# jdwhite48/groth-sahai-rs

Measured on AMD Instinct MI355X. Metric: GS proofs+verifies/sec (BLS12-381 PPE batch), higher is better.
Workload: dtype u32 limbs (381-bit Montgomery); 1 GPU; 2^16 independent PPE equations per GPU, m=4 n=4, BLS12-381, commit_and_prove+verify(exact); curve=BLS12-381, equations_per_gpu=65536, total_equations=65536, rccl_ranks=0, distinct_devices=1, parallelism=equation-sharded x1

## Files before the change

groth_sahai_rs_amd/csrc/gen_params.py:

```python
#!/usr/bin/env python3
import os
import sys


def limbs32(v, n):
    return [(v >> (32 * i)) & 0xFFFFFFFF for i in range(n)]


def carr(v, n):
    return "{" + ",".join("0x%08xu" % x for x in limbs32(v, n)) + "}"


class F2:

    def __init__(self, p):
        self.p = p

    def mul(self, a, b):
        p = self.p
        return ((a[0] * b[0] - a[1] * b[1]) % p, (a[0] * b[1] + a[1] * b[0]) % p)

    def pow(self, a, e):
        r = (1, 0)
        while e:
            if e & 1:
                r = self.mul(r, a)
            a = self.mul(a, a)
            e >>= 1
        return r

    def inv(self, a):
        p = self.p
        n = pow(a[0] * a[0] + a[1] * a[1], -1, p)
        return (a[0] * n % p, (-a[1]) * n % p)


def naf(k):
    d = []
    while k:
        if k & 1:
            z = 2 - (k % 4)
            k -= z
        else:
            z = 0
        d.append(z)
        k >>= 1
    return d


def emit(name, S, p, r, x, b, xi, twist, loop_count, loop_neg, bn, g1, g2):
    n = (p.bit_length() + 31) // 32
    nr = (r.bit_length() + 31) // 32
    Rp = 1 << (32 * n)
    Rr = 1 << (32 * nr)
    f2 = F2(p)

    def m(v):
        return v * Rp % p

    def m2(a):
        return "{%s,%s}" % (carr(m(a[0]), n), carr(m(a[1]), n))

    L = (p.bit_length() + 27) // 28
    if L * 28 - p.bit_length() < 8:
        L += 1
    R28 = 1 << (28 * L)
    Rb = 1 << (32 * n)

    def l28(v):
        ls = []
        for i in range(L - 1):
            ls.append(v & 0xFFFFFFF)
            v >>= 28
        ls.append(v)
        return "{" + ",".join(str(x) for x in ls) + "}"

    def i28(v):
        return l28(v * R28 % p)

    def i28_2(a):
        return "{%s,%s}" % (i28(a[0]), i28(a[1]))

    out = []
    w = out.append
    w("// GENERATED by gen_params.py -- do not edit.")
    w("#pragma once")
    w("#include <stdint.h>")
    w("#ifndef GS_DEVCONST")
    w("#if defined(__HIPCC__)")
    w("#define GS_DEVCONST __device__")
    w("#else")
    w("#define GS_DEVCONST")
    w("#endif")
    w("#endif")
    w("namespace gs {")
    w("struct %s {" % S)
    w("  static constexpr int N = %d;      // u32 limbs of Fq" % n)
    w("  static constexpr int NR = %d;     // u32 limbs of Fr" % nr)
    w("  static constexpr int CURVE_ID = %d;" % (0 if name == "bls12_381" else 1))
    w("  static constexpr bool TWIST_M = %s;" % ("true" if twist == "M" else "false"))
    w("  static constexpr bool IS_BN = %s;" % ("true" if bn else "false"))
    w("  static constexpr int XI_A = %d;   // xi = XI_A + u" % xi[0])
    w("  GS_DEVCONST static constexpr uint32_t P[%d] = %s;" % (n, carr(p, n)))
    w("  GS_DEVCONST static constexpr uint32_t P_INV = 0x%08xu;   // -p^-1 mod 2^32" % ((-pow(p, -1, 1 << 32)) % (1 << 32)))
    w("  GS_DEVCONST static constexpr uint32_t P_ONE[%d] = %s;   // R mod p" % (n, carr(Rp % p, n)))
    w("  GS_DEVCONST static constexpr uint32_t P_R2[%d] = %s;    // R^2 mod p" % (n, carr(Rp * Rp % p, n)))
    w("  GS_DEVCONST static constexpr uint32_t P_M2[%d] = %s;    // p - 2 (inversion exponent)" % (n, carr(p - 2, n)))
    w("  static constexpr int P_BITS = %d;" % p.bit_length())
    w("  GS_DEVCONST static constexpr uint32_t Q[%d] = %s;   // scalar field modulus r" % (nr, carr(r, nr)))
    w("  GS_DEVCONST static constexpr uint32_t Q_INV = 0x%08xu;" % ((-pow(r, -1, 1 << 32)) % (1 << 32)))
    w("  GS_DEVCONST static constexpr uint32_t Q_ONE[%d] = %s;" % (nr, carr(Rr % r, nr)))
    w("  GS_DEVCONST static constexpr uint32_t Q_R2[%d] = %s;" % (nr, carr(Rr * Rr % r, nr)))
    w("  static constexpr int Q_BITS = %d;" % r.bit_length())
    w("  GS_DEVCONST static constexpr uint32_t TWO_INV[%d] = %s;" % (n, carr(m(pow(2, -1, p)), n)))
    w("  GS_DEVCONST static constexpr uint32_t B1[%d] = %s;       // G1: y^2 = x^3 + b" % (n, carr(m(b), n)))
    b2 = f2.mul((b, 0), xi) if twist == "M" else f2.mul((b, 0), f2.inv(xi))
    w("  GS_DEVCONST static constexpr uint32_t B2[2][%d] = %s;   // twist coefficient b'" % (n, m2(b2)))
    b2x3 = ((3 * b2[0]) % p, (3 * b2[1]) % p)
    w("  GS_DEVCONST static constexpr uint32_t B2X3[2][%d] = %s;" % (n, m2(b2x3)))
    k = 3 * b if twist == "M" and 3 * b < 16 else 0
    assert k == 0 or b2x3 == f2.mul((k, 0), xi)
    w("  static constexpr int B2X3_XI_K = %d;   // 3 b' = B2X3_XI_K * xi when non-zero" % k)
    for j in (1, 2, 3):
        e = (p**j - 1) // 6
        assert (p**j - 1) % 6 == 0
        g = [f2.pow(xi, k * e) for k in range(6)]
        w("  GS_DEVCONST static constexpr uint32_t FROB%d[6][2][%d] = {%s};" % (j, n, ",".join(m2(v) for v in g)))
    ax = abs(x)
    w("  static constexpr uint64_t X_ABS = 0x%xull;" % ax)
    w("  static constexpr bool X_NEG = %s;" % ("true" if x < 0 else "false"))
    d = naf(loop_count) if bn else [(loop_count >> i) & 1 for i in range(loop_count.bit_length())]
    w("  static constexpr int LOOP_LEN = %d;   // digits of the Miller loop count, LSB first" % len(d))
    w("  GS_DEVCONST static constexpr int8_t LOOP[%d] = {%s};" % (len(d), ",".join(str(v) for v in d)))
    w("  static constexpr bool LOOP_NEG = %s;" % ("true" if loop_neg else "false"))
    w("  GS_DEVCONST static constexpr uint32_t G1_GEN[2][%d] = {%s,%s};" % (n, carr(m(g1[0]), n), carr(m(g1[1]), n)))
    w("  GS_DEVCONST static constexpr uint32_t G2_GEN[2][2][%d] = {%s,%s};" % (n, m2(g2[0]), m2(g2[1])))
    w("  static constexpr int L = %d;      // 28-bit limbs of Fq (internal form a*2^(28L) mod p, lazily reduced)" % L)
    w("  GS_DEVCONST static constexpr int32_t P28[%d] = %s;" % (L, l28(p)))
    w("  static constexpr uint32_t P28_INV = %du;   // -p^-1 mod 2^28" % ((-pow(p, -1, 1 << 28)) % (1 << 28)))
    w("  static constexpr float INV_PTOP2 = %.9ef;   // 2^(28(L-2)) / p  (value-reduction quotient estimate)" % ((1 << (28 * (L - 2))) / p))
    w("  GS_DEVCONST static constexpr int32_t ONE28[%d] = %s;" % (L, i28(1)))
    w("  GS_DEVCONST static constexpr int32_t K_IN28[%d] = %s;   // boundary -> internal: R28^2/Rb mod p" % (L, l28(R28 * R28 * pow(Rb, -1, p) % p)))
    w("  GS_DEVCONST static constexpr int32_t K_OUT28[%d] = %s;  // internal -> boundary: Rb mod p" % (L, l28(Rb % p)))
    assert p % 4 == 3
    w("  GS_DEVCONST static constexpr int32_t RR28[%d] = %s;    // canonical -> internal: R28^2 mod p" % (L, l28(R28 * R28 % p)))
    w("  GS_DEVCONST static constexpr int32_t RRR28[%d] = %s;   // R28^3 mod p: plain inverse of an internal value -> internal inverse" % (L, l28(pow(R28, 3, p))))
    w("  static constexpr int INV_DIVSTEPS = %d;" % ((45907 * p.bit_length() + 26313) // 19929))
    w("  GS_DEVCONST static constexpr uint32_t SQRT_EXP[%d] = %s;  // (p+1)/4" % (n, carr((p + 1) // 4, n)))
    w("  GS_DEVCONST static constexpr uint32_t HALF_P[%d] = %s;    // (p-1)/2" % (n, carr((p - 1) // 2, n)))
    w("  GS_DEVCONST static constexpr uint32_t P_WORDS[%d] = %s;" % (n, carr(p, n)))
    w("  GS_DEVCONST static constexpr uint32_t R_WORDS[%d] = %s;" % (nr, carr(r, nr)))
    w("  GS_DEVCONST static constexpr int32_t B2_28[2][%d] = %s;   // b of the twist" % (L, i28_2(b2)))
    w("  GS_DEVCONST static constexpr int32_t B1_28[%d] = %s;" % (L, i28(b)))
    w("  GS_DEVCONST static constexpr int32_t B2X3_28[2][%d] = %s;" % (L, i28_2(b2x3)))
    for j in (1, 2, 3):
        e = (p**j - 1) // 6
        g = [f2.pow(xi, k * e) for k in range(6)]
        w("  GS_DEVCONST static constexpr int32_t FROB%d_28[6][2][%d] = {%s};" % (j, L, ",".join(i28_2(v) for v in g)))
    if not bn:
        lam = x * x - 1
        assert (lam * lam + lam + 1) % r == 0 and lam.bit_length() <= 128
        def f2add(a, b2_): return ((a[0] + b2_[0]) % p, (a[1] + b2_[1]) % p)
        def f2sub(a, b2_): return ((a[0] - b2_[0]) % p, (a[1] - b2_[1]) % p)
        def ec_add(P1, P2, mul_, sub_, add_, inv_, zero):
            if P1 is None: return P2
            if P2 is None: return P1
            (x1, y1), (x2, y2) = P1, P2
            if x1 == x2:
                if y1 != y2 or y1 == zero: return None
                l_ = mul_(mul_(add_(add_(x1, x1), x1), x1), inv_(add_(y1, y1)))
            else:
                l_ = mul_(sub_(y2, y1), inv_(sub_(x2, x1)))
            x3 = sub_(sub_(mul_(l_, l_), x1), x2)
            return (x3, sub_(mul_(l_, sub_(x1, x3)), y1))
        def ec_mul(k, P_, *ops):
            acc = None
            for bit in bin(k)[2:]:
                acc = ec_add(acc, acc, *ops)
                if bit == "1": acc = ec_add(acc, P_, *ops)
            return acc
        ops1 = (lambda a, b_: a * b_ % p, lambda a, b_: (a - b_) % p, lambda a, b_: (a + b_) % p, lambda a: pow(a, -1, p), 0)
        ops2 = (f2.mul, f2sub, f2add, f2.inv, (0, 0))
        lamG = ec_mul(lam, g1, *ops1)
        beta = None
        for cand in range(2, 50):
            bcand = pow(cand, (p - 1) // 3, p)
            if bcand != 1 and (bcand * g1[0]) % p == lamG[0]:
                beta = bcand
                break
        assert beta is not None and lamG[1] == g1[1]
        G2 = ((g2[0][0], g2[0][1]), (g2[1][0], g2[1][1]))
        xG2 = ec_mul(abs(x), G2, *ops2)
        xG2 = (xG2[0], ((-xG2[1][0]) % p, (-xG2[1][1]) % p))
        conj_ = lambda a: (a[0], (-a[1]) % p)
        e3, e2 = (p - 1) // 3, (p - 1) // 2
        found = None
        for sx in (1, -1):
            for sy in (1, -1):
                cx = f2.pow(xi, e3) if sx == 1 else f2.inv(f2.pow(xi, e3))
                cy = f2.pow(xi, e2) if sy == 1 else f2.inv(f2.pow(xi, e2))
                if (f2.mul(conj_(G2[0]), cx), f2.mul(conj_(G2[1]), cy)) == xG2:
                    found = (cx, cy)
        assert found, "psi constants"
        cx, cy = found
        nx, ny = f2.mul(cx, conj_(cx)), f2.mul(cy, conj_(cy))
        assert nx[1] == 0 and ny[1] == 0
        c3x, c3y = f2.mul(cx, nx), f2.mul(cy, ny)
        out.insert(out.index("};"), "") if False else None
        w2 = lambda line: out.insert(len(out), line)
        endo = []
        endo.append("  static constexpr bool HAS_ENDO = true;")
        endo.append("  GS_DEVCONST static constexpr uint32_t LAMBDA[4] = %s;   // x^2 - 1: phi(P) = (beta x, y) = lambda P" % carr(lam, 4))
        endo.append("  GS_DEVCONST static constexpr int32_t BETA_28[%d] = %s;" % (L, i28(beta)))
        endo.append("  GS_DEVCONST static constexpr uint32_t XABS_LIMBS[2] = %s;" % carr(abs(x), 2))
        endo.append("  GS_DEVCONST static constexpr int32_t PSI_X_28[2][%d] = %s;   // psi(x,y) = (conj(x) cx, conj(y) cy) = [x]Q" % (L, i28_2(cx)))
        endo.append("  GS_DEVCONST static constexpr int32_t PSI_Y_28[2][%d] = %s;" % (L, i28_2(cy)))
        endo.append("  GS_DEVCONST static constexpr int32_t PSI2_X_28[%d] = %s;     // psi^2(x,y) = (x nx, y ny)" % (L, i28(nx[0])))
        endo.append("  GS_DEVCONST static constexpr int32_t PSI2_Y_28[%d] = %s;" % (L, i28(ny[0])))
        endo.append("  GS_DEVCONST static constexpr int32_t PSI3_X_28[2][%d] = %s;" % (L, i28_2(c3x)))
        endo.append("  GS_DEVCONST static constexpr int32_t PSI3_Y_28[2][%d] = %s;" % (L, i28_2(c3y)))
    else:
        from fractions import Fraction
        def ec_add1(P1, P2):
            if P1 is None: return P2
            if P2 is None: return P1
            (x1, y1), (x2, y2) = P1, P2
            if x1 == x2:
                if (y1 + y2) % p == 0: return None
                l_ = 3 * x1 * x1 * pow(2 * y1, -1, p) % p
            else:
                l_ = (y2 - y1) * pow(x2 - x1, -1, p) % p
            x3 = (l_ * l_ - x1 - x2) % p
            return (x3, (l_ * (x1 - x3) - y1) % p)
        def ec_mul1(k, P_):
            acc = None
            for bit in bin(k)[2:]:
                acc = ec_add1(acc, acc)
                if bit == "1": acc = ec_add1(acc, P_)
            return acc
        lam = beta = None
        for gcand in range(2, 12):
            z = pow(gcand, (r - 1) // 3, r)
            if z == 1: continue
            for zz in (z, (-z - 1) % r):
                lg = ec_mul1(zz, g1)
                for cand in range(2, 50):
                    bc = pow(cand, (p - 1) // 3, p)
                    if bc != 1 and bc * g1[0] % p == lg[0] and lg[1] == g1[1]:
                        lam, beta = zz, bc
            if lam: break
        assert lam and (lam * lam + lam + 1) % r == 0
        def lagrange(u, v):
            dot = lambda a, b_: a[0] * b_[0] + a[1] * b_[1]
            if dot(u, u) < dot(v, v): u, v = v, u
            while True:
                q = round(Fraction(dot(u, v), dot(v, v)))
                u = (u[0] - q * v[0], u[1] - q * v[1])
                if dot(u, u) >= dot(v, v): return [list(v), list(u)]
                u, v = v, u
        def lll(B_):
            n_ = len(B_)
            B_ = [list(map(Fraction, b_)) for b_ in B_]
            def gso():
                Bs, m_ = [], [[Fraction(0)] * n_ for _ in range(n_)]
                for i in range(n_):
                    v = B_[i][:]
                    for j in range(i):
                        m_[i][j] = sum(a * b_ for a, b_ in zip(B_[i], Bs[j])) / sum(a * a for a in Bs[j])
                        v = [a - m_[i][j] * b_ for a, b_ in zip(v, Bs[j])]
                    Bs.append(v)
                return Bs, m_
            k_ = 1
            while k_ < n_:
                Bs, m_ = gso()
                for j in range(k_ - 1, -1, -1):
                    q = round(m_[k_][j])
                    if q:
                        B_[k_] = [a - q * b_ for a, b_ in zip(B_[k_], B_[j])]
                        Bs, m_ = gso()
                if sum(a * a for a in Bs[k_]) >= (Fraction(3, 4) - m_[k_][k_ - 1] ** 2) * sum(a * a for a in Bs[k_ - 1]):
                    k_ += 1
                else:
                    B_[k_], B_[k_ - 1] = B_[k_ - 1], B_[k_]
                    k_ = max(k_ - 1, 1)
            return [[int(a) for a in b_] for b_ in B_]
        def inv_first_row(B_):
            n_ = len(B_)
            A_ = [list(map(Fraction, row)) + [Fraction(int(i == j)) for j in range(n_)] for i, row in enumerate(B_)]
            for i in range(n_):
                piv = next(j for j in range(i, n_) if A_[j][i] != 0)
                A_[i], A_[piv] = A_[piv], A_[i]
                f_ = A_[i][i]
                A_[i] = [a / f_ for a in A_[i]]
                for j in range(n_):
                    if j != i:
                        f_ = A_[j][i]
                        A_[j] = [a - f_ * b_ for a, b_ in zip(A_[j], A_[i])]
            return [A_[0][n_ + i] for i in range(n_)]
        def lattice_consts(tag, B_, eig, gw, bw):
            n_ = len(B_)
            for b_ in B_:
                assert sum(b_[j] * eig ** j for j in range(n_)) % r == 0
            row = inv_first_row(B_)
            G_ = [abs(int(v * (1 << 256))) for v in row]
            sg = [1 if v < 0 else 0 for v in row]
            import random as _rnd
            rr_ = _rnd.Random(7)
            worst = 0
            for _ in range(4000):
                k_ = rr_.randrange(r)
                cs = [(k_ * G_[i] >> 256) * (-1 if sg[i] else 1) for i in range(n_)]
                ks = [(k_ if j == 0 else 0) - sum(cs[i] * B_[i][j] for i in range(n_)) for j in range(n_)]
                assert (sum(ks[j] * eig ** j for j in range(n_)) - k_) % r == 0
                worst = max(worst, max(abs(v).bit_length() for v in ks))
            lines = ["  static constexpr int %s_SUBBITS = %d;   // measured bound on the sub-scalars (4000 samples) + slack below" % (tag, worst),
                     "  GS_DEVCONST static constexpr uint32_t %s_G[%d][%d] = {%s};" % (tag, n_, gw, ",".join(carr(v, gw) for v in G_)),
                     "  GS_DEVCONST static constexpr uint8_t %s_GS[%d] = {%s};" % (tag, n_, ",".join(str(v) for v in sg)),
                     "  GS_DEVCONST static constexpr uint32_t %s_B[%d][%d][%d] = {%s};" % (tag, n_, n_, bw, ",".join("{" + ",".join(carr(abs(v), bw) for v in b_) + "}" for b_ in B_)),
                     "  GS_DEVCONST static constexpr uint8_t %s_BS[%d][%d] = {%s};" % (tag, n_, n_, ",".join("{" + ",".join("1" if v < 0 else "0" for v in b_) + "}" for b_ in B_))]
            for v in G_: assert v.bit_length() <= 32 * gw
            for b_ in B_:
                for v in b_: assert abs(v).bit_length() <= 32 * bw
            return lines, worst
        B1 = lagrange((r, 0), (-lam, 1))
        mu = p % r
        B2l = lll([[r, 0, 0, 0], [-mu, 1, 0, 0], [-(mu * mu) % r, 0, 1, 0], [-(mu ** 3) % r, 0, 0, 1]])
        l1, w1 = lattice_consts("GLV1", B1, lam, 5, 4)
        l2, w2 = lattice_consts("GLS2", B2l, mu, 7, 2)
        assert w1 <= 130 and w2 <= 68
        f2add = lambda a, b2_: ((a[0] + b2_[0]) % p, (a[1] + b2_[1]) % p)
        f2sub = lambda a, b2_: ((a[0] - b2_[0]) % p, (a[1] - b2_[1]) % p)
        def ec_add2(P1, P2):
            if P1 is None: return P2
            if P2 is None: return P1
            (x1, y1), (x2, y2) = P1, P2
            if x1 == x2:
                if f2add(y1, y2) == (0, 0): return None
                l_ = f2.mul(f2.mul((3, 0), f2.mul(x1, x1)), f2.inv(f2add(y1, y1)))
            else:
                l_ = f2.mul(f2sub(y2, y1), f2.inv(f2sub(x2, x1)))
            x3 = f2sub(f2sub(f2.mul(l_, l_), x1), x2)
            return (x3, f2sub(f2.mul(l_, f2sub(x1, x3)), y1))
        def ec_mul2(k, P_):
            acc = None
            for bit in bin(k)[2:]:
                acc = ec_add2(acc, acc)
                if bit == "1": acc = ec_add2(acc, P_)
            return acc
        G2p = ((g2[0][0], g2[0][1]), (g2[1][0], g2[1][1]))
        cxp, cyp = f2.pow(xi, 2 * (p - 1) // 6), f2.pow(xi, 3 * (p - 1) // 6)
        psiQ = (f2.mul((G2p[0][0], (-G2p[0][1]) % p), cxp), f2.mul((G2p[1][0], (-G2p[1][1]) % p), cyp))
        assert psiQ == ec_mul2(mu, G2p), "psi eigenvalue"
        endo = ["  static constexpr bool HAS_ENDO = true;",
                "  GS_DEVCONST static constexpr int32_t BETA_28[%d] = %s;   // phi(x,y) = (beta x, y) = [lambda](x,y)" % (L, i28(beta))]
        endo += l1 + l2
    for line in endo:
        w(line)
    w("};")
    w("}  // namespace gs")
    return "\n".join(out) + "\n"


def main():
    here = os.path.dirname(os.path.abspath(__file__))
    p = 0x1A0111EA397FE69A4B1BA7B6434BACD764774B84F38512BF6730D2A0F6B0F6241EABFFFEB153FFFFB9FEFFFFFFFFAAAB
    r = 0x73EDA753299D7D483339D80809A1D80553BDA402FFFE5BFEFFFFFFFF00000001
    x = -0xD201000000010000
    g1 = (
        0x17F1D3A73197D7942695638C4FA9AC0FC3688C4F9774B905A14E3A3F171BAC586C55E83FF97A1AEFFB3AF00ADB22C6BB,
        0x08B3F481E3AAA0F1A09E30ED741D8AE4FCF5E095D5D00AF600DB18CB2C04B3EDD03CC744A2888AE40CAA232946C5E7E1,
    )
    g2 = (
        (
# ... 32 lines not shown
```

groth_sahai_rs_amd/csrc/gs_amd.hip:

```cpp
#include "../../include/gs_amd.h"

#include <hip/hip_runtime.h>
#include <stdio.h>
#include <stdlib.h>
#include <string.h>

#include <dlfcn.h>
#include <sys/mman.h>

#include <algorithm>
#include <atomic>
#include <chrono>
#include <condition_variable>
#include <deque>
#include <map>
#include <memory>
#include <mutex>
#include <queue>
#include <string>
#include <thread>
#include <type_traits>
#include <unordered_map>
#include <vector>

// ... 318 lines not shown
    hipError_t e = hipHostMalloc(&c->pin, bytes, hipHostMallocDefault);
    if (e != hipSuccess) return fail(c, GS_ERR_ALLOC, "hipHostMalloc (pinned staging)", e);
    c->pin_cap = bytes;
    return GS_OK;
  }
  int begin(const int* order, int norder, size_t base = 0, bool reserve = true) {
    begun = true;
    t0 = std::chrono::steady_clock::now();
    trace = getenv("GS_PIPE_TRACE") != nullptr;
    if (const char* e = getenv("GS_COPY_SPLIT")) split = std::max(1, std::min(2, atoi(e)));
    int prio_least = 0, prio_greatest = 0;
    (void)hipDeviceGetStreamPriorityRange(&prio_least, &prio_greatest);
    for (hipStream_t* st : {&c->copy_stream, &c->copy_stream2, &c->copy_out_stream, &c->copy_out_stream2})
      if (!*st && hipStreamCreateWithPriority(st, hipStreamNonBlocking, prio_greatest) != hipSuccess) {
        (void)hipGetLastError();
        *st = nullptr;
        HIPCHK(c, hipStreamCreateWithFlags(st, hipStreamNonBlocking));
      }
    if (!c->pev_ready) HIPCHK(c, hipEventCreateWithFlags(&c->pev_ready, hipEventDisableTiming));
    if (!c->pool) {
      int nt = 4;
      if (const char* e = getenv("GS_COPY_THREADS")) nt = std::max(1, std::min(32, atoi(e)));
      c->pool = new CopyPool(nt);
    }
    const size_t total = layout();
    if (reserve) RC(pin_reserve(c, base + total));
    for (int i = 0; i < n; i++) {
      if (!arr[i].bytes) continue;
      char name[32];
      snprintf(name, sizeof name, "stage.%d", i);
      RC(scratch(c, name, arr[i].bytes, &arr[i].d));
      arr[i].off += base;
      for (hipEvent_t* ev : {&ev1[i], &ev2[i]}) HIPCHK(c, hipEventCreateWithFlags(ev, hipEventDisableTiming));
    }
    for (int k = 0; k < norder; k++) {
      Arr& a = arr[order[k]];
      if (a.hin && !a.direct) c->pool->submit((uint8_t*)c->pin + a.off, a.hin, a.bytes, &a.left);
    }
    for (int k = 0; k < norder; k++) {
      Arr& a = arr[order[k]];
      if (!a.hin || !a.direct || a.enq) continue;
      RC(xfer(a.d, a.hin, a.bytes, hipMemcpyHostToDevice, c->copy_stream, c->copy_stream2, ev1[order[k]], ev2[order[k]]));
      a.enq = true;
    }
    c->pipe = this;
    if (trace) fprintf(stderr, "[pipe] %7.2f ms begin done (%zu bytes of staging)\n", ms(), total);
    return GS_OK;
  }
  int xfer(void* dst, const void* src, size_t bytes, hipMemcpyKind kind, hipStream_t s0, hipStream_t s1, hipEvent_t ev,
           hipEvent_t ev_b) {
    if (split < 2 || bytes < ((size_t)4 << 20)) {
      HIPCHK(c, hipMemcpyAsync(dst, src, bytes, kind, s0));
    } else {
      size_t h = (bytes / 2 + 255) & ~(size_t)255;
      HIPCHK(c, hipMemcpyAsync(dst, src, h, kind, s0));
      HIPCHK(c, hipMemcpyAsync((uint8_t*)dst + h, (const uint8_t*)src + h, bytes - h, kind, s1));
      HIPCHK(c, hipEventRecord(ev_b, s1));
      HIPCHK(c, hipStreamWaitEvent(s0, ev_b, 0));
    }
    HIPCHK(c, hipEventRecord(ev, s0));
    return GS_OK;
  }
  int need(unsigned mask) {
    hipStream_t tgt = c->cur ? c->cur : c->stream;
    for (int i = 0; i < n; i++) {
      Arr& a = arr[i];
      if (!((mask >> i) & 1) || !a.hin) continue;
      if (!a.enq) {
        double w0 = trace ? ms() : 0;
        CopyPool::wait(&a.left);
        double w1 = trace ? ms() : 0;
        RC(xfer(a.d, a.direct ? a.hin : (uint8_t*)c->pin + a.off, a.bytes, hipMemcpyHostToDevice, c->copy_stream, c->copy_stream2, ev1[i],
                ev2[i]));
        a.enq = true;
        if (trace)
          fprintf(stderr, "[pipe] %7.2f ms H2D of array %d enqueued (%.1f MB, waited %.2f ms for its staging, %.2f ms in the enqueue)\n",
                  ms(), i, a.bytes / 1e6, w1 - w0, ms() - w1);
      }
      HIPCHK(c, hipStreamWaitEvent(tgt, ev1[i], 0));
    }
    return GS_OK;
  }
  int out_ready(unsigned mask) {
    if (c->rec) return GS_OK;
    hipStream_t src = c->cur ? c->cur : c->stream;
    bool first = true;
    for (int i = 0; i < n; i++) {
      Arr& a = arr[i];
      if (!((mask >> i) & 1) || !a.hout || a.enq) continue;
      if (first) {
        HIPCHK(c, hipEventRecord(c->pev_ready, src));
        HIPCHK(c, hipStreamWaitEvent(c->copy_out_stream, c->pev_ready, 0));
        HIPCHK(c, hipStreamWaitEvent(c->copy_out_stream2, c->pev_ready, 0));
        first = false;
      }
      RC(xfer(a.direct ? a.hout : (uint8_t*)c->pin + a.off, a.d, a.bytes, hipMemcpyDeviceToHost, c->copy_out_stream, c->copy_out_stream2,
              ev1[i], ev2[i]));
      a.enq = true;
      out_order[n_out++] = i;
      if (trace) fprintf(stderr, "[pipe] %7.2f ms D2H of array %d enqueued (%.1f MB)\n", ms(), i, a.bytes / 1e6);
    }
    return GS_OK;
  }
  int finish() {
    c->pipe = nullptr;
    if (trace) fprintf(stderr, "[pipe] %7.2f ms kernels enqueued\n", ms());
    hipStream_t keep = c->cur;
    c->cur = nullptr;
    int rc = out_ready(0xFFFFu);
    c->cur = keep;
    RC(rc);
    for (int k = 0; k < n_out; k++) {
      const int i = out_order[k];
      Arr& a = arr[i];
      HIPCHK(c, hipEventSynchronize(ev1[i]));
      if (trace) fprintf(stderr, "[pipe] %7.2f ms array %d arrived\n", ms(), i);
      if (!a.direct) c->pool->submit(a.hout, (uint8_t*)c->pin + a.off, a.bytes, &a.left);
    }
    HIPCHK(c, hipStreamSynchronize(c->stream));
    for (int i = 0; i < n; i++) CopyPool::wait(&arr[i].left);
    finished = true;
    if (trace) fprintf(stderr, "[pipe] %7.2f ms done\n", ms());
    return GS_OK;
  }
};
bool HostPipe::host_pinned(const void* p, size_t bytes) {
  static const bool off = getenv("GS_PIPE_NO_DIRECT") != nullptr;
  if (off || !p || !bytes) return false;
  std::lock_guard<std::mutex> lk(g_reg_mu);
  auto it = g_reg.upper_bound((const uint8_t*)p);
  if (it == g_reg.begin()) return false;
  --it;
  return (const uint8_t*)p + bytes <= it->first + it->second;
}
static inline int need(gs_ctx* c, unsigned mask) { return c->pipe ? c->pipe->need(mask) : GS_OK; }
static inline int out_ready(gs_ctx* c, unsigned mask) { return c->pipe ? c->pipe->out_ready(mask) : GS_OK; }
enum { PI_X = 0, PI_Y, PI_A, PI_B, PI_G, PI_R, PI_S, PI_T, PO_XC, PO_YC, PO_PI, PO_TH };
enum { VI_A = 0, VI_B, VI_G, VI_TG, VI_XC, VI_YC, VI_PI, VI_TH, VO_OK };
enum { RI_A = 0, RI_B, RI_G, RI_R, RI_S, RI_T, RI_XC, RI_YC, RI_PI, RI_TH, RO_XC, RO_YC, RO_PI, RO_TH };
#define BIT(i) (1u << (i))

static inline size_t fillN(const gs_ctx* c, size_t N) { return c->fill_n > N ? c->fill_n : N; }

struct MCost {
  double base, var, fix;
};
#ifndef GS_PLAN_PAIR
#define GS_PLAN_PAIR 1
#endif
static inline MCost mcost(int curve, bool twin) {
#if defined(GS_LINES_GENERAL)
  if (curve == 0) return twin ? MCost{4536.0, 7764.0, 6256.0} : MCost{2268.0, 4636.0, 3128.0};
  return twin ? MCost{4680.0, 10519.0, 8096.0} : MCost{2340.0, 6471.0, 4048.0};
#else
  if (curve == 0) return twin ? MCost{4536.0, 7356.0, 5304.0} : MCost{2268.0, 4636.0, 2652.0};
  return twin ? MCost{4680.0, 9991.0, 6864.0} : MCost{2340.0, 6471.0, 3432.0};
#endif
}
static inline bool pair_fixed(bool lt, const PairRef& r) { return lt && r.q_arr == 2; }
static void chunk_tasks(std::vector<MillerTask>& mt, const std::vector<PairRef>& pr, double budget, int b, bool single,
                        const MCost& mc, bool lt) {
  size_t P = pr.size();
  if (P == 0) return;
  std::vector<size_t> order;
  double total = 0;
  for (size_t i = 0; i < P; i++)
    if (!pair_fixed(lt, pr[i])) order.push_back(i);
  for (size_t i = 0; i < P; i++)
    if (pair_fixed(lt, pr[i])) order.push_back(i);
  for (size_t i = 0; i < P; i++) total += pair_fixed(lt, pr[i]) ? mc.fix : mc.var;
  size_t nt0 = (P + MILLER_CH - 1) / MILLER_CH;
  if (budget > 0) nt0 = std::max(nt0, (size_t)(total / budget));
  nt0 = std::min(std::max(nt0, (size_t)1), P);
  for (size_t nt = nt0; nt <= P; nt++) {
    std::vector<double> load(nt, 0.0);
    std::vector<std::vector<size_t>> members(nt);
    typedef std::pair<double, size_t> Slot;
    std::priority_queue<Slot, std::vector<Slot>, std::greater<Slot>> heap;
    for (size_t t = 0; t < nt; t++) heap.push(Slot(0.0, t));
    for (size_t idx : order) {
      Slot sl = heap.top();
      heap.pop();
      size_t best = sl.second;
      members[best].push_back(idx);
      load[best] += pair_fixed(lt, pr[idx]) ? mc.fix : mc.var;
      if (members[best].size() < (size_t)MILLER_CH) heap.push(Slot(load[best], best));
    }
    double mx = 0;
    for (double l : load) mx = l > mx ? l : mx;
    if (mx > budget && nt < P) continue;
    for (size_t t = 0; t < nt; t++) {
      MillerTask mtk;
      memset(&mtk, 0, sizeof mtk);
      mtk.b = (uint8_t)b;
      mtk.single = single ? 1 : 0;
      mtk.np = (uint8_t)members[t].size();
      for (int q = 0; q < mtk.np; q++) mtk.pr[q] = pr[members[t][q]];
      mt.push_back(mtk);
    }
    return;
  }
}
static double fold_cost(double n, double unit) {
  double c = 0;
  while (n > 16.0) {
    c += 8.0 * unit;
    n = (double)(size_t)((n + 7.0) / 8.0);
  }
  return c + n * unit;
}
static inline double pair_lane_cost(const gs_ctx* c, const MillerTask& t) {
  const MCost mc = mcost(c->curve, true);
  int nv = 0, nf = 0;
  for (int q = 0; q < t.np; q++) (pair_fixed(c->line_tables, t.pr[q]) ? nf : nv)++;
  return mc.base / 2 + ((nv + 1) / 2) * (mc.var - mc.fix) + (nv + nf) * mc.fix / 2;
}
static double miller_cost(const gs_ctx* c, size_t N, const std::vector<MillerTask>& mt, bool twin, bool pair = false) {
  MCost mc = mcost(c->curve, twin);
  double longest = 0, all = 0;
  const size_t NL = pair ? 2 * N : N;
  const double wpt = NL >= 64 ? (double)(size_t)((NL + 63) / 64) : (double)NL / 64.0;
  for (const MillerTask& t : mt) {
    double l = mc.base;
    for (int q = 0; q < t.np; q++) l += pair_fixed(c->line_tables, t.pr[q]) ? mc.fix : mc.var;
    if (pair) l = pair_lane_cost(c, t);
    longest = l > longest ? l : longest;
    all += l * wpt;
  }
  double rounds = (double)mt.size() * wpt / (double)c->simd_slots;
  double fill = all / (double)c->simd_slots;
  if (rounds > 1.0 && rounds < 4.0) fill *= (double)(size_t)(rounds + 0.999) / rounds;
  double lane = rounds <= 1.0 ? longest : (fill > longest ? fill : longest);
  double per_cell = (double)mt.size() * (twin ? 2.0 : 1.0) / 4.0;
  return lane + fold_cost(per_cell, 54.0);
}
static std::vector<double> miller_budgets(const gs_ctx* c, bool twin) {
  const MCost mc = mcost(c->curve, twin);
  std::vector<double> out;
  for (int a = 1; a <= MILLER_CH; a++)
    for (int f = 0; f <= 2 && a + f <= MILLER_CH; f++) {
      if (c->miller_ch > 0 && a + f != c->miller_ch) continue;
      out.push_back(a * mc.var + f * mc.fix);
    }
  return out;
}
static std::vector<MillerTask> plan_miller_single(const gs_ctx* c, size_t N, const std::vector<PairRef>& pr) {
  std::vector<MillerTask> mt;
  double best = -1;
  for (double cand : miller_budgets(c, false)) {
    std::vector<MillerTask> tmp;
    chunk_tasks(tmp, pr, cand, 0, true, mcost(c->curve, false), c->line_tables);
    double cost = miller_cost(c, N, tmp, false);
    if (best < 0 || cost < best) {
      best = cost;
      mt = tmp;
    }
  }
  return mt;
}
static void miller_work_hint(gs_ctx* c, size_t N, const std::vector<MillerTask>& mt, bool twin) {
  const MCost mc = mcost(c->curve, twin);
  double pairs = 0;
  for (const MillerTask& t : mt)
    for (int q = 0; q < t.np; q++) pairs += pair_fixed(c->line_tables, t.pr[q]) ? mc.fix / mc.var : 1.0;
  c->work_hint = (uint64_t)((double)N * pairs);
}

static inline size_t var_ws_default(const gs_ctx* c) { return 2 * c->simd_slots * 64; }
static size_t var_ws_auto(const gs_ctx* c, size_t tot, size_t bytes_per_lane) {
  const size_t round = c->simd_slots * 64, base = var_ws_default(c);
  if (tot <= base) return tot;
  size_t free_b = 0, total_b = 0;
  if (hipMemGetInfo(&free_b, &total_b) != hipSuccess) {
    (void)hipGetLastError();
    return base;
  }
  size_t budget = std::min(free_b / 4, (size_t)32 << 30);
  size_t lanes = budget / std::max(bytes_per_lane, (size_t)1) / round * round;
  return std::min(tot, std::max(lanes, base));
}
template <class K, class... Args>
static int launch(gs_ctx* c, const char* name, K kern, size_t total, int block, Args... args) {
  if (c->rec) return fail(c, GS_ERR_ARG, "internal: this kernel cannot be part of a merged launch");
  if (total == 0) return GS_OK;
  unsigned grid = (unsigned)((total + block - 1) / block);
  hipStream_t st = c->cur ? c->cur : c->stream;
  if (c->prof) hipEventRecord(c->ev0, st);
  hipLaunchKernelGGL(kern, dim3(grid), dim3(block), 0, st, args...);
  hipError_t e = hipGetLastError();
  if (e != hipSuccess) return fail(c, GS_ERR_DEVICE, name, e);
  if (c->prof) {
    hipEventRecord(c->ev1, st);
    hipEventSynchronize(c->ev1);
    float ms = 0;
    hipEventElapsedTime(&ms, c->ev0, c->ev1);
    if (!c->prof_map.count(name)) c->prof_order.push_back(name);
    ProfEntry& p = c->prof_map[name];
    p.ms += ms;
    p.n += 1;
    p.lanes += total;
    p.work += c->work_hint ? c->work_hint : total;
  }
  c->work_hint = 0;
  return GS_OK;
}

// ... 169 lines not shown
      if (e.host.size() != nb || (nb && memcmp(e.host.data(), b, nb) != 0)) continue;
      if (!e.dev.p) {
        c->plans.erase(it);
        continue;
      }
      e.last_use = ++c->plan_clock;
      *out = (const T*)e.dev.p;
      return GS_OK;
    }
    RC(plan_evict(c));
    PlanEntry e;
    RC(ensure(c, e.dev, nb + 16));
    if (nb) {
      hipError_t ce = hipMemcpy(e.dev.p, b, nb, hipMemcpyHostToDevice);
      if (ce != hipSuccess) {
        hipFree(e.dev.p);
        return fail(c, GS_ERR_DEVICE, "task table upload", ce);
      }
    }
    e.host.assign(b, b + nb);
    e.last_use = ++c->plan_clock;
    *out = (const T*)e.dev.p;
    c->plans.emplace(key, std::move(e));
    return GS_OK;
  }
}

struct SidePlan {
  std::vector<GrpTask> grp;
  int tm = 1;
  int mo = 1, w = 4;
  bool shared_done = false;
  std::vector<VarTask> var;
  std::vector<FixTask> fix;
  std::vector<RedTask> red;
  int nslots = 0;
  int ncom = 0;
  int tab_bases = 0;
};

static FixTask mkfix(int s0, int t0, int s1, int t1, int a_arr, int a_idx, int slot, int a_neg = 0) {
  FixTask f;
  f.s0 = (uint32_t)s0;
  f.s1 = (uint32_t)s1;
  f.t0 = (uint8_t)t0;
  f.t1 = (uint8_t)t1;
  f.a_arr = (uint8_t)a_arr;
  f.a_idx = (uint32_t)a_idx;
  f.a_neg = (uint8_t)a_neg;
  f.slot = (uint32_t)slot;
  return f;
}
static VarTask mkvar(int s, int arr, int idx, int slot) {
  VarTask v;
  v.s_idx = (uint32_t)s;
  v.p_arr = (uint8_t)arr;
  v.p_idx = (uint32_t)idx;
  v.slot = (uint32_t)slot;
  v.neg = 0;
  v.pad0 = v.pad1 = 0;
  return v;
}
static RedTask mkred(int b0, int e0, int b1, int e1, int out_arr, int out_idx) {
  RedTask r;
  r.b0 = (uint32_t)b0;
  r.e0 = (uint32_t)e0;
  r.b1 = (uint32_t)b1;
  r.e1 = (uint32_t)e1;
  r.out_arr = (uint8_t)out_arr;
  r.out_idx = (uint32_t)out_idx;
  r.pad = r.pad1 = r.pad2 = 0;
  return r;
}
static void add_pair(std::vector<PairRef>& v, int p_arr, int p_idx, int neg, int q_arr, int q_idx) {
  PairRef r;
  r.p_arr = (uint8_t)p_arr;
  r.p_idx = (uint32_t)p_idx;
  r.neg = (uint8_t)neg;
  r.q_arr = (uint8_t)q_arr;
  r.q_idx = (uint32_t)q_idx;
  r.pad = 0;
  v.push_back(r);
}
struct ArrEnt {
  int i;
  const void* base;
  uint32_t stride;
  bool present = true;
};
static ArrTab arr_tab(std::initializer_list<ArrEnt> ents) {
  ArrTab t;
  memset(&t, 0, sizeof t);
  for (const ArrEnt& e : ents)
    if (e.present) {
      t.base[e.i] = (const uint8_t*)e.base;
      t.stride[e.i] = e.stride;
    }
  return t;
}
static OutTab out_tab(void* base0, uint32_t stride0, void* base1 = nullptr, uint32_t stride1 = 0) {
  OutTab t;
  memset(&t, 0, sizeof t);
  t.base[0] = (uint8_t*)base0;
  t.stride[0] = stride0;
  t.base[1] = (uint8_t*)base1;
  t.stride[1] = stride1;
  return t;
}

static void add_var_terms(SidePlan& sp, const std::vector<VarTask>& terms, int& slot) {
  size_t T = terms.size();
  if (T == 0) return;
  size_t tm = sp.tm < 1 ? 1 : (size_t)sp.tm, ng = (T + tm - 1) / tm, base = T / ng, rem = T % ng, s0 = 0;
  for (size_t k = 0; k < ng; k++) {
    size_t n = base + (k < rem ? 1 : 0);
    GrpTask g;
    memset(&g, 0, sizeof g);
    g.first[0] = (uint32_t)sp.var.size();
    g.nt = (uint32_t)n;
    g.no = 1;
    g.slot[0] = (uint32_t)slot;
    for (size_t i = 0; i < n; i++) {
      VarTask v = terms[s0 + i];
      v.slot = (uint32_t)slot;
      sp.var.push_back(v);
    }
    s0 += n;
    sp.grp.push_back(g);
    slot++;
  }
}
struct ComOutputs {
  SidePlan& sp;
  int slot = 0;
  void fix(int s0, int t0, int s1, int t1, int a_arr, int a_idx, int a_neg = 0) {
    sp.fix.push_back(mkfix(s0, t0, s1, t1, a_arr, a_idx, slot, a_neg));
    slot++;
  }
  void terms(const std::vector<VarTask>& t) { add_var_terms(sp, t, slot); }
  template <class Emit> void add(int count, int out_arr, int out0, Emit emit) {
    for (int q = 0; q < count; q++) {
      int b[2], e[2];
      for (int comp = 0; comp < 2; comp++) {
        b[comp] = slot;
        emit(q, comp, *this);
        e[comp] = slot;
      }
      sp.red.push_back(mkred(b[0], e[0], b[1], e[1], out_arr, out0 + q));
    }
    sp.nslots = slot;
  }
};
static double straus_lane_cost(bool g2, bool bn, int nt, int no, int w) {
  const double madd = g2 ? 29.0 : 11.0, dbl = g2 ? 16.0 : 8.0, gz = g2 ? 21.0 : 7.0, endo = g2 ? 4.0 : 0.5;
  const int ns = g2 ? 4 : 2, nl = g2 ? (bn ? 3 : 2) : (bn ? 5 : 4), nd = (32 * nl + w - 1) / w + 1, ne = 1 << (w - 1);
  double build = nt * (ne / 2 * dbl + (ne / 2 - 1) * madd + ne * gz);
  double run = (nd - 1) * w * dbl + (double)nt * ns * (nd - 0.5) * (1.0 - 1.0 / (2 * ne)) * (madd + endo);
  return build + no * run;
}
static double wave_rounds(const gs_ctx* c, double waves, bool g2) {
  double r = waves / (double)c->simd_slots;
  if (g2 || c->curve != 1) {
    if (r <= 1.0) return 1.0;
    return r < 4.0 ? (double)(size_t)(r + 0.999) : r;
  }
  const double gain = 1.55;
  return r <= gain ? 1.0 : r / gain;
}
static int pick_tm(const gs_ctx* c, size_t N, int T, int outputs, bool g2, int share) {
  if (T < 2 || !c->endo) return 1;
  if (c->var_tm > 0) {
    int ng = (T + c->var_tm - 1) / c->var_tm;
    return (T + ng - 1) / ng;
  }
  int best_tm = 1;
  double best = -1;
  for (int tm = 1; tm <= 8; tm++) {
    int ng = (T + tm - 1) / tm, eff = (T + ng - 1) / ng;
    if (eff != tm) continue;
    for (int mo : {1, 2, 4}) {
      if (mo > 1 && (eff < 2 || mo > share)) continue;
      if (c->var_mo > 0 && mo != c->var_mo && !(eff < 2 && mo == 1)) continue;
      for (int w : {4, 5}) {
        if (w == 5 && eff < 2) continue;
        if (c->var_w > 0 && w != c->var_w && eff >= 2) continue;
        double lanes = (double)N * ((double)outputs / mo) * ng;
        double rounds = wave_rounds(c, lanes / 64.0, g2);
        double cost = rounds * straus_lane_cost(g2, c->curve == 1, eff, mo, w) +
                      fold_cost((double)ng, g2 ? 29.0 + 14.0 : 16.0);
        if (best < 0 || cost < best) {
          best = cost;
          best_tm = eff;
        }
      }
    }
  }
  return best_tm;
}

static void share_tables(const gs_ctx* c, size_t N, SidePlan& sp, bool g2) {
  if (sp.shared_done) return;
  sp.shared_done = true;
  sp.mo = 1;
  sp.w = 4;
  if (sp.tab_bases > 0) return;
  if (sp.tm <= 1 || sp.grp.empty()) return;
  auto same = [&](const GrpTask& a, const GrpTask& b) {
    if (a.nt != b.nt) return false;
    for (uint32_t i = 0; i < a.nt; i++) {
      const VarTask &x = sp.var[a.first[0] + i], &y = sp.var[b.first[0] + i];
      if (x.p_idx != y.p_idx || x.p_arr != y.p_arr || x.neg != y.neg) return false;
    }
    return true;
  };
  std::vector<std::vector<size_t>> fam;
  std::unordered_map<uint64_t, std::vector<size_t>> by_hash;
  int ntmax = 1;
  for (size_t i = 0; i < sp.grp.size(); i++) {
    const GrpTask& g = sp.grp[i];
    uint64_t h = 1469598103934665603ull ^ g.nt;
    for (uint32_t k = 0; k < g.nt; k++) {
      const VarTask& v = sp.var[g.first[0] + k];
      h = (h ^ (((uint64_t)v.p_idx << 16) | ((uint64_t)v.p_arr << 8) | v.neg)) * 1099511628211ull;
    }
    std::vector<size_t>& cand = by_hash[h];
    size_t f = (size_t)-1;
    for (size_t c2 : cand)
      if (same(sp.grp[fam[c2][0]], g)) {
        f = c2;
        break;
      }
    if (f == (size_t)-1) {
      f = fam.size();
      fam.emplace_back();
      cand.push_back(f);
    }
    fam[f].push_back(i);
    ntmax = std::max(ntmax, (int)g.nt);
  }
  size_t share = 1;
  for (auto& f : fam) share = std::max(share, f.size());
  int best_mo = 1, best_w = 4;
  double best = -1;
  for (int mo : {1, 2, 4}) {
    if (c->var_mo > 0 && mo != c->var_mo) continue;
    if (c->var_mo <= 0 && (size_t)mo > share) continue;
    size_t lanes = 0;
    for (auto& f : fam) lanes += (f.size() + mo - 1) / mo;
    for (int w : {4, 5}) {
      if (c->var_w > 0 && w != c->var_w) continue;
      if (c->var_w <= 0 && c->rec && w != 4) continue;
      double rounds = wave_rounds(c, (double)N * lanes / 64.0, g2);
      int eff_mo = (int)std::min((size_t)mo, share);
      double cost = rounds * straus_lane_cost(g2, c->curve == 1, ntmax, eff_mo, w);
      if (best < 0 || cost < best) {
        best = cost;
        best_mo = mo;
        best_w = w;
      }
    }
  }
  sp.mo = best_mo;
  sp.w = best_w;
  if (getenv("GS_PLAN_TRACE")) {
    size_t lanes = 0;
    for (auto& f : fam) lanes += (f.size() + best_mo - 1) / best_mo;
    fprintf(stderr, "[plan] straus %s fill %zu: %zu groups in %zu families (largest %zu), <= %d terms; outputs per build %d, window %d, "
            "%zu lanes per equation\n", g2 ? "G2" : "G1", N, sp.grp.size(), fam.size(), share, ntmax, best_mo, best_w, lanes);
  }
  if (best_mo == 1) return;
  std::vector<GrpTask> merged;
  for (const std::vector<size_t>& f : fam) {
    for (size_t b = 0; b < f.size(); b += best_mo) {
      GrpTask g = sp.grp[f[b]];
      g.no = (uint32_t)std::min((size_t)best_mo, f.size() - b);
      for (uint32_t o = 1; o < g.no; o++) {
        g.first[o] = sp.grp[f[b + o]].first[0];
        g.slot[o] = sp.grp[f[b + o]].slot[0];
      }
      merged.push_back(g);
    }
  }
  sp.grp.swap(merged);
}

static void build_side(SidePlan& sp, bool want_coms, int nv, int nc, bool group, int kc, int npf, int rc, int vc,
                       int cs, int ph, int f0, int sg) {
  ComOutputs out{sp};
  if (want_coms) {
    out.add(nv, 0, 0, [&](int i, int c, ComOutputs& o) {
      if (group)
        o.fix(rc + 2 * i, tb_u(0, c), rc + 2 * i + 1, tb_u(1, c), c ? 0 : 0xFF, i);
      else
        o.fix(vc + i, tb_w(c), rc + i, tb_u(0, c), 0xFF, 0);
    });
    sp.ncom = nv;
  }
  out.add(npf, 1, 0, [&](int l, int c, ComOutputs& o) {
    if (!group) return o.fix(sg + l, tb_w(c), f0 + l, tb_u(0, c), 0xFF, 0);
    o.fix(f0 + l * 2, tb_u(0, c), f0 + l * 2 + 1, tb_u(1, c), 0xFF, 0);
    if (c == 0) return;
    std::vector<VarTask> terms;
    for (int j = 0; j < nc; j++) terms.push_back(mkvar(cs + j * npf + l, 1, j, 0));
    for (int i = 0; i < nv; i++) terms.push_back(mkvar(ph + l * nv + i, 0, i, 0));
    o.terms(terms);
  });
}
// ... 2594 lines not shown
```

groth_sahai_rs_amd/csrc/gs_curve.cuh:

```cuda
#pragma once
#include "gs_tower.cuh"

#if defined(GS_JAC_INLINE)
#define GS_JAC GS_HD
#else
#define GS_JAC GS_HD_NOINLINE
#endif

namespace gs {

template <class F> struct Aff {
  F x, y;
};
template <class F> struct Jac {
  F x, y, z;
};

template <class F> GS_HD bool aff_is_inf(const Aff<F>& p) { return is_zero_limbs(p.x) && is_zero_limbs(p.y); }
template <class F> GS_HD void jac_set_inf(Jac<F>& r) {
  r.x = one_of<F>();
  r.y = one_of<F>();
  r.z = zero_of<F>();
}
template <class F> GS_HD void jac_from_aff(Jac<F>& r, const Aff<F>& p) {
// ... 434 lines not shown
    v += carry;
    if (v >= (1u << (W - 1))) {
      dg[i] = (int8_t)((int)v - (1 << W));
      carry = 1;
    } else {
      dg[i] = (int8_t)v;
      carry = 0;
    }
  }
}
template <class F> GS_HD_NOINLINE void smul_build_table_n(Jac<F>* tab, const Aff<F>& p, int ne) {
  Jac<F> cur;
  jac_from_aff(cur, p);
  tab[0] = cur;
#pragma unroll 1
  for (int k = 2; k <= ne; k++) {
    if (k & 1) {
      jac_madd_ip(cur, p);
    } else {
      Jac<F> t = tab[k / 2 - 1];
      cur = t;
      jac_dbl_ip(cur);
    }
    tab[k - 1] = cur;
  }
}

template <class F> GS_HD_NOINLINE void smul_affine_table(Aff<F>* out, Jac<F>* stage, const Aff<F>& p, int ne) {
  if (aff_is_inf(p)) {
    for (int i = 0; i < ne; i++) out[i].x = zero_of<F>(), out[i].y = zero_of<F>();
    return;
  }
  smul_build_table_n(stage, p, ne);
  F acc = one_of<F>();
  for (int i = 0; i < ne; i++) {
    out[i].x = acc;
    if (!is_zero_limbs(stage[i].z)) acc = mul(acc, stage[i].z);
  }
  F iv = inv(acc);
  for (int i = ne - 1; i >= 0; i--) {
    if (is_zero_limbs(stage[i].z)) {
      out[i].x = zero_of<F>();
      out[i].y = zero_of<F>();
      continue;
    }
    F zi = mul(out[i].x, iv);
    iv = mul(iv, stage[i].z);
    F z2 = sqr(zi);
    out[i].x = mul(stage[i].x, z2);
    out[i].y = mul(stage[i].y, mul(z2, zi));
  }
}

template <int NA, int NB> GS_HD void mp_mul(uint32_t* out, const uint32_t* a, const uint32_t* b) {
  for (int i = 0; i < NA + NB; i++) out[i] = 0;
  for (int i = 0; i < NA; i++) {
    uint64_t carry = 0;
    for (int j = 0; j < NB; j++) {
      uint64_t t = (uint64_t)a[i] * b[j] + out[i + j] + carry;
      out[i + j] = (uint32_t)t;
      carry = t >> 32;
    }
    out[i + NB] = (uint32_t)carry;
  }
}
template <int W, int NA> GS_HD void mp_acc(uint32_t* acc, const uint32_t* a, bool add) {
  uint64_t c = add ? 0 : 1;
  for (int i = 0; i < W; i++) {
    uint32_t w = i < NA ? a[i] : 0u;
    if (!add) w = ~w;
    uint64_t t = (uint64_t)acc[i] + w + c;
    acc[i] = (uint32_t)t;
    c = t >> 32;
  }
}
template <int D, int GW, int BW, int NL>
GS_HD void endo_lattice(uint32_t (*mag)[NL], uint8_t* sgn, const uint32_t* k, const uint32_t (*G)[GW], const uint8_t* GS,
                        const uint32_t (*B)[D][BW], const uint8_t (*BS)[D]) {
  constexpr int W = 10;
  static_assert(GW + BW < W && NL <= W, "decomposition width");
  uint32_t c[D][GW];
  for (int i = 0; i < D; i++) {
    uint32_t t[8 + GW], g[GW];
    for (int w = 0; w < GW; w++) g[w] = G[i][w];
    mp_mul<8, GW>(t, k, g);
    for (int w = 0; w < GW; w++) c[i][w] = t[8 + w];
  }
  for (int j = 0; j < D; j++) {
    uint32_t acc[W];
    for (int w = 0; w < W; w++) acc[w] = (j == 0 && w < 8) ? k[w] : 0u;
    for (int i = 0; i < D; i++) {
      uint32_t t[GW + BW], b[BW];
      for (int w = 0; w < BW; w++) b[w] = B[i][j][w];
      mp_mul<GW, BW>(t, c[i], b);
      bool neg_prod = (GS[i] != 0) != (BS[i][j] != 0);
      mp_acc<W, GW + BW>(acc, t, neg_prod);
    }
    bool negative = (acc[W - 1] >> 31) != 0;
    if (negative) {
      uint64_t cy = 1;
      for (int w = 0; w < W; w++) {
        uint64_t t = (uint64_t)(~acc[w]) + cy;
        acc[w] = (uint32_t)t;
        cy = t >> 32;
      }
    }
    sgn[j] = negative ? 1 : 0;
    for (int w = 0; w < NL; w++) mag[j][w] = acc[w];
  }
}

template <class C> GS_HD_NOINLINE void jac_smul_endo(Jac<Fq<C>>& rout, const Aff<Fq<C>>& p, const Fr<C>& k) {
  Jac<Fq<C>> r;
  uint32_t kk[8], q[8], k1[4], k2[4], lam[4];
  for (int i = 0; i < 8; i++) kk[i] = k.v[i];
  for (int i = 0; i < 4; i++) lam[i] = C::LAMBDA[i];
  limb_divmod_const<8, 4, DivLambda<C>>(q, k1, kk);
  (void)lam;
  for (int i = 0; i < 4; i++) k2[i] = q[i];
  Jac<Fq<C>> tab[8];
  Aff<Fq<C>> at[8];
  Fq<C> zback;
  int8_t d1[33], d2[33];
  smul_build_table(tab, p);
  table_global_z<C>(at, tab, 8, zback);
  recode_w4_limbs<4>(d1, k1);
  recode_w4_limbs<4>(d2, k2);
  Fq<C> beta;
  for (int i = 0; i < C::L; i++) beta.v[i] = C::BETA_28[i];
  jac_set_inf(r);
  for (int i = 32; i >= 0; i--) {
    if (i != 32) {
#pragma unroll 1
      for (int d4 = 0; d4 < 4; d4++) jac_dbl(r, r);
    }
    int a = d1[i];
    if (a != 0) {
      Aff<Fq<C>> t = at[(a < 0 ? -a : a) - 1];
      if (a < 0) t.y = neg(t.y);
      jac_madd(r, r, t);
    }
    int b = d2[i];
    if (b != 0) {
      Aff<Fq<C>> t = at[(b < 0 ? -b : b) - 1];
      t.x = mul(t.x, beta);
      if (b < 0) t.y = neg(t.y);
      jac_madd(r, r, t);
    }
  }
  r.z = mul(r.z, zback);
  rout = r;
}

template <class C> GS_HD Fp2<C> fp2_const28(const int32_t (*c)[C::L]) {
  Fp2<C> r;
  for (int i = 0; i < C::L; i++) {
    r.c0.v[i] = c[0][i];
    r.c1.v[i] = c[1][i];
  }
  return r;
}
template <class C> GS_HD void endo_apply(Aff<Fq<C>>& t, int s) {
  if (s == 1) {
    Fq<C> beta;
    for (int i = 0; i < C::L; i++) beta.v[i] = C::BETA_28[i];
    t.x = mul(t.x, beta);
  }
}
template <class C> GS_HD void endo_apply(Aff<Fp2<C>>& t, int s) {
  if (aff_is_inf(t)) return;
  if constexpr (C::IS_BN) {
    if (s == 0) return;
    Fp2<C> x = (s & 1) ? conj(t.x) : t.x, y = (s & 1) ? conj(t.y) : t.y;
    t.x = mul(x, frob_coeff<C>(s, 2));
    t.y = mul(y, frob_coeff<C>(s, 3));
    return;
  } else if (s == 1) {
    t.x = mul(conj(t.x), fp2_const28<C>(C::PSI_X_28));
    t.y = mul(conj(t.y), fp2_const28<C>(C::PSI_Y_28));
  } else if (s == 2) {
    Fq<C> nx, ny;
    for (int l = 0; l < C::L; l++) {
      nx.v[l] = C::PSI2_X_28[l];
      ny.v[l] = C::PSI2_Y_28[l];
    }
    t.x = mul_fp(t.x, nx);
    t.y = mul_fp(t.y, ny);
  } else if (s == 3) {
    t.x = mul(conj(t.x), fp2_const28<C>(C::PSI3_X_28));
    t.y = mul(conj(t.y), fp2_const28<C>(C::PSI3_Y_28));
  }
}
template <class C> GS_HD_NOINLINE void jac_smul_endo(Jac<Fp2<C>>& rout, const Aff<Fp2<C>>& p, const Fr<C>& k) {
  Jac<Fp2<C>> r;
  uint32_t n[8], q[8], xa[2], d[4][2];
  for (int i = 0; i < 8; i++) n[i] = k.v[i];
  xa[0] = C::XABS_LIMBS[0];
  xa[1] = C::XABS_LIMBS[1];
  for (int j = 0; j < 3; j++) {
    limb_divmod_const<8, 2, DivXabs<C>>(q, d[j], n);
    for (int i = 0; i < 8; i++) n[i] = q[i];
  }
  (void)xa;
  d[3][0] = n[0];
  d[3][1] = n[1];
  Jac<Fp2<C>> tab[8];
  Aff<Fp2<C>> at[8];
  Fp2<C> zback;
  int8_t dg[4][17];
  smul_build_table(tab, p);
  table_global_z<C>(at, tab, 8, zback);
  for (int j = 0; j < 4; j++) recode_w4_limbs<2>(dg[j], d[j]);
  jac_set_inf(r);
  for (int i = 16; i >= 0; i--) {
    if (i != 16) {
#pragma unroll 1
      for (int d4 = 0; d4 < 4; d4++) jac_dbl_ip(r);
    }
    for (int j = 0; j < 4; j++) {
      int a = dg[j][i];
      if (a == 0) continue;
      Aff<Fp2<C>> t = at[(a < 0 ? -a : a) - 1];
      bool negate = (a < 0) != ((j & 1) != 0);
      endo_apply<C>(t, j);
      if (negate) t.y = neg(t.y);
      jac_madd_ip(r, t);
    }
  }
  r.z = mul(r.z, zback);
  rout = r;
}

template <class C, class F, int TMAX>
GS_HD void jac_msm_straus_at(Jac<F>& r, const Aff<F>* ps, const Fr<C>* ks, int nt, Aff<F>* at);
template <class C, class F, int TMAX> GS_HD void jac_msm_straus(Jac<F>& r, const Aff<F>* ps, const Fr<C>* ks, int nt) {
  Aff<F> at[TMAX * 8];
  jac_msm_straus_at<C, F, TMAX>(r, ps, ks, nt, at);
}
template <class C, class F, bool ENDO = true> GS_HD void jac_smul_any(Jac<F>& r, const Aff<F>& p, const Fr<C>& k) {
  if constexpr (!ENDO)
    jac_smul(r, p, k);
  else if constexpr (C::HAS_ENDO && C::IS_BN)
    jac_msm_straus<C, F, 1>(r, &p, &k, 1);
  else if constexpr (C::HAS_ENDO)
    jac_smul_endo<C>(r, p, k);
  else
    jac_smul(r, p, k);
}

template <class C, class F> struct EndoShape;
template <class C> struct EndoShape<C, Fq<C>> {
  static constexpr int NS = 2, NL = C::IS_BN ? 5 : 4, ND = 8 * NL + 1;
  static constexpr int nd(int w) { return (32 * NL + w - 1) / w + 1; }
};
template <class C> struct EndoShape<C, Fp2<C>> {
  static constexpr int NS = 4, NL = C::IS_BN ? 3 : 2, ND = 8 * NL + 1;
  static constexpr int nd(int w) { return (32 * NL + w - 1) / w + 1; }
};
template <class C, int W = 4> GS_HD void endo_digits(int8_t* dg, uint8_t* sgn, const Fr<C>& k, const Jac<Fq<C>>*) {
  typedef EndoShape<C, Fq<C>> E;
  constexpr int ND = E::nd(W);
  uint32_t kk[8];
  for (int i = 0; i < 8; i++) kk[i] = k.v[i];
  if constexpr (C::IS_BN) {
    uint32_t mag[2][E::NL];
    endo_lattice<2, 5, 4, E::NL>(mag, sgn, kk, C::GLV1_G, C::GLV1_GS, C::GLV1_B, C::GLV1_BS);
    for (int s = 0; s < 2; s++) recode_w_limbs<E::NL, W>(dg + ND * s, mag[s]);
  } else {
    uint32_t q[8], k1[4], k2[4], lam[4];
    for (int i = 0; i < 4; i++) lam[i] = C::LAMBDA[i];
    limb_divmod_const<8, 4, DivLambda<C>>(q, k1, kk);
    (void)lam;
    for (int i = 0; i < 4; i++) k2[i] = q[i];
    recode_w_limbs<4, W>(dg, k1);
    recode_w_limbs<4, W>(dg + ND, k2);
    sgn[0] = sgn[1] = 0;
  }
}
template <class C, int W = 4> GS_HD void endo_digits(int8_t* dg, uint8_t* sgn, const Fr<C>& k, const Jac<Fp2<C>>*) {
  typedef EndoShape<C, Fp2<C>> E;
  constexpr int ND = E::nd(W);
  uint32_t n[8];
  for (int i = 0; i < 8; i++) n[i] = k.v[i];
  if constexpr (C::IS_BN) {
    uint32_t mag[4][E::NL];
    endo_lattice<4, 7, 2, E::NL>(mag, sgn, n, C::GLS2_G, C::GLS2_GS, C::GLS2_B, C::GLS2_BS);
    for (int s = 0; s < 4; s++) recode_w_limbs<E::NL, W>(dg + ND * s, mag[s]);
  } else {
    uint32_t q[8], xa[2], d[4][2];
    xa[0] = C::XABS_LIMBS[0];
    xa[1] = C::XABS_LIMBS[1];
    for (int j = 0; j < 3; j++) {
      limb_divmod_const<8, 2, DivXabs<C>>(q, d[j], n);
      for (int i = 0; i < 8; i++) n[i] = q[i];
    }
    (void)xa;
    d[3][0] = n[0];
    d[3][1] = n[1];
    for (int j = 0; j < 4; j++) {
      recode_w_limbs<2, W>(dg + ND * j, d[j]);
      sgn[j] = (uint8_t)(j & 1);
    }
  }
}

#if defined(GS_DEBUG_STAMPS) && defined(__HIPCC__)
__device__ unsigned long long gs_dbg[16];
#endif
#if defined(GS_DEBUG_STAMPS) && defined(__HIP_DEVICE_COMPILE__)
#define GS_STAMP_T() __builtin_amdgcn_s_memtime()
#define GS_STAMP_ADD(i, t) do { if ((threadIdx.x & 63) == 0) atomicAdd(&gs_dbg[i], (unsigned long long)(t)); } while (0)
#else
#define GS_STAMP_T() 0ull
#define GS_STAMP_ADD(i, t) do { } while (0)
#endif
#if defined(GS_STRAUS_INLINE)
#define GS_STRAUS GS_HD
#else
#define GS_STRAUS GS_HD_NOINLINE
#endif
template <class C, class F, int TMAX, int W>
GS_STRAUS void jac_straus_build(Aff<F>* at, F& zback, const Aff<F>* ps, int nt, Jac<F>* tab) {
  constexpr int NE = 1 << (W - 1);
  for (int t = 0; t < nt; t++) smul_build_table_n(tab + t * NE, ps[t], NE);
  table_global_z<C>(at, tab, NE * nt, zback);
}
template <class C, class F, int TMAX, int W, bool GTAB = false, int LDSKB = 36>
GS_STRAUS void jac_straus_run(Jac<F>& rout, const Fr<C>* ks, int nt, const Aff<F>* at, const F& zback,
                                   const Aff<F>* const* tabs = nullptr, uint32_t negm = 0) {
  constexpr int NE = 1 << (W - 1);
  Jac<F> r;
  if constexpr (C::HAS_ENDO) {
    typedef EndoShape<C, F> E;
    constexpr int ND = E::nd(W);
#if defined(__HIP_DEVICE_COMPILE__) && !defined(GS_STRAUS_OLD_LOOP)
    unsigned long long st0 = GS_STAMP_T(), st_dbl = 0, st_add = 0;
    constexpr int NSL = E::NS * ND;
    constexpr int ROWB = ((TMAX * NSL + 3) / 4 * 4);
    constexpr int ROW = ((ROWB / 4) % 2 == 0) ? ROWB + 4 : ROWB;
    constexpr bool LDS_DG = (size_t)ROW * 64 <= (size_t)LDSKB * 1024;
    __shared__ int8_t sdg[LDS_DG ? ROW * 64 : 4];
    int8_t ldg[LDS_DG ? 1 : TMAX * NSL];
    int8_t* const dgp = LDS_DG ? &sdg[(threadIdx.x & 63) * ROW] : ldg;
    uint32_t sgm = 0;
    for (int t = 0; t < nt; t++) {
      uint8_t sg1[E::NS];
      endo_digits<C, W>(dgp + t * NSL, sg1, ks[t], (const Jac<F>*)nullptr);
      for (int s2 = 0; s2 < E::NS; s2++) sgm |= (uint32_t)(sg1[s2] != 0) << (t * E::NS + s2);
    }
    auto digit = [&](int i, int k) -> int {
      const int idx = (k / E::NS) * NSL + (k % E::NS) * ND + i;
      if constexpr (LDS_DG) return (int)sdg[(threadIdx.x & 63) * ROW + idx];
      return (int)ldg[idx];
    };
    jac_set_inf(r);
    const int nk = nt * E::NS;
    int top = 0;
    for (int k = 0; k < nk; k++)
      for (int i = ND - 1; i > top; i--)
        if (digit(i, k) != 0) top = i;
    auto entry = [&](int i, int k) -> const Aff<F>* {
      int a = digit(i, k);
      a = a < 0 ? -a : a;
      const int idx = a ? a - 1 : 0, t = k / E::NS;
      return tabs ? tabs[t] + idx : at + t * NE + idx;
    };
    auto ldaff = [](const Aff<F>* p) -> Aff<F> {
      Aff<F> v;
      constexpr int NWD = (int)(sizeof(Aff<F>) / sizeof(limb_t));
      if constexpr (GTAB) {
        typedef const __attribute__((address_space(1))) limb_t* gptr;
        gptr w = (gptr) reinterpret_cast<const limb_t*>(p);
#pragma unroll
        for (int q = 0; q < NWD; q++) reinterpret_cast<limb_t*>(&v)[q] = w[q];
      } else {
        const limb_t* w = reinterpret_cast<const limb_t*>(p);
#pragma unroll
        for (int q = 0; q < NWD; q++) reinterpret_cast<limb_t*>(&v)[q] = w[q];
      }
      return v;
    };
    Aff<F> e = ldaff(entry(top, 0));
    unsigned long long st1 = GS_STAMP_T();
    for (int i = top; i >= 0; i--) {
      if (i != top) {
        unsigned long long sa = GS_STAMP_T();
#pragma unroll 1
        for (int d4 = 0; d4 < W; d4++) jac_dbl_ip(r);
        st_dbl += GS_STAMP_T() - sa;
      }
#pragma unroll 1
      for (int k = 0; k < nk; k++) {
        Aff<F> en = e;
        {
          int ni = i, k2 = k + 1;
          if (k2 == nk) ni = i - 1, k2 = 0;
          if (ni >= 0) en = ldaff(entry(ni, k2));
        }
        const int a = digit(i, k);
        unsigned long long sb = GS_STAMP_T();
        if (a != 0) {
          const int t = k / E::NS, s2 = k % E::NS;
          Aff<F> u = e;
          endo_apply<C>(u, s2);
          if (((a < 0) != (((sgm >> k) & 1) != 0)) != (((negm >> t) & 1) != 0)) u.y = neg(u.y);
          jac_madd_ip(r, u);
        }
        st_add += GS_STAMP_T() - sb;
        e = en;
      }
    }
    {
      unsigned long long st2 = GS_STAMP_T();
      GS_STAMP_ADD(0, st1 - st0);
      GS_STAMP_ADD(1, st2 - st1);
      GS_STAMP_ADD(2, st_dbl);
      GS_STAMP_ADD(3, st_add);
      GS_STAMP_ADD(4, 1);
    }
#else
    int8_t dg[TMAX][E::NS * ND];
    uint8_t sg[TMAX][E::NS];
    for (int t = 0; t < nt; t++) endo_digits<C, W>(dg[t], sg[t], ks[t], (const Jac<F>*)nullptr);
    jac_set_inf(r);
    int top = 0;
    for (int t = 0; t < nt; t++)
      for (int s = 0; s < E::NS; s++)
        for (int i = ND - 1; i > top; i--)
          if (dg[t][s * ND + i] != 0) top = i;
    for (int i = top; i >= 0; i--) {
      if (i != top) {
#pragma unroll 1
        for (int d4 = 0; d4 < W; d4++) jac_dbl_ip(r);
      }
      for (int t = 0; t < nt; t++)
        for (int s = 0; s < E::NS; s++) {
          int a = dg[t][s * ND + i];
          if (a == 0) continue;
          Aff<F> e = tabs ? tabs[t][(a < 0 ? -a : a) - 1] : at[t * NE + (a < 0 ? -a : a) - 1];
          endo_apply<C>(e, s);
          if (((a < 0) != (sg[t][s] != 0)) != (((negm >> t) & 1) != 0)) e.y = neg(e.y);
          jac_madd_ip(r, e);
        }
    }
#endif
  } else {
    static_assert(C::HAS_ENDO || W == 4, "plain curves: width 4 only");
    constexpr int ND = (FrM<C>::BITS + 3) / 4 + 1;
    int8_t dg[TMAX][ND];
    for (int t = 0; t < nt; t++) recode_w4<FrM<C>>(dg[t], ND, ks[t]);
    jac_set_inf(r);
    int top = 0;
    for (int t = 0; t < nt; t++)
      for (int i = ND - 1; i > top; i--)
        if (dg[t][i] != 0) top = i;
    for (int i = top; i >= 0; i--) {
      if (i != top) {
#pragma unroll 1
        for (int d4 = 0; d4 < 4; d4++) jac_dbl(r, r);
      }
      for (int t = 0; t < nt; t++) {
        int a = dg[t][i];
        if (a == 0) continue;
        Aff<F> e = at[t * NE + (a < 0 ? -a : a) - 1];
        if (a < 0) e.y = neg(e.y);
        jac_madd(r, r, e);
      }
    }
  }
  r.z = mul(r.z, zback);
  rout = r;
}
template <class C, class F, int TMAX>
GS_HD void jac_msm_straus_at(Jac<F>& rout, const Aff<F>* ps, const Fr<C>* ks, int nt, Aff<F>* at) {
  F zback;
  Jac<F> tab[TMAX * 8];
  jac_straus_build<C, F, TMAX, 4>(at, zback, ps, nt, tab);
  jac_straus_run<C, F, TMAX, 4>(rout, ks, nt, at, zback);
}

constexpr int SHARED_MAXD = 104;
struct SharedDigits {
  int32_t top;
  uint32_t sgm;
  int8_t d[SHARED_MAXD];
};
template <class C, class F, bool ENDO> struct SharedShape {
  static constexpr bool E = ENDO && C::HAS_ENDO;
  static constexpr int NS = E ? EndoShape<C, F>::NS : 1;
  static constexpr int ND = E ? EndoShape<C, F>::nd(4) : (FrM<C>::BITS + 3) / 4 + 1;
  static_assert(NS * ND <= SHARED_MAXD, "digit streams of a launch-wide scalar");
};
template <class C, class F, bool ENDO> GS_HD void shared_digits(SharedDigits& o, const Fr<C>& k) {
  typedef SharedShape<C, F, ENDO> S;
  for (int i = 0; i < SHARED_MAXD; i++) o.d[i] = 0;
  o.sgm = 0;
  if constexpr (S::E) {
    uint8_t sg[S::NS];
    endo_digits<C, 4>(o.d, sg, k, (const Jac<F>*)nullptr);
    for (int s = 0; s < S::NS; s++) o.sgm |= (uint32_t)(sg[s] != 0) << s;
  } else {
    recode_w4<FrM<C>>(o.d, S::ND, k);
  }
  int top = 0;
  for (int s = 0; s < S::NS; s++)
    for (int i = S::ND - 1; i > top; i--)
      if (o.d[s * S::ND + i] != 0) top = i;
  o.top = top;
}
GS_HD int wave_uniform(int v) {
#if defined(__HIP_DEVICE_COMPILE__)
  return __builtin_amdgcn_readfirstlane(v);
#else
  return v;
#endif
}
template <class C, class F, bool ENDO>
GS_HD_NOINLINE void jac_smul_shared(Jac<F>& rout, const Aff<F>& p, const SharedDigits* sd) {
  typedef SharedShape<C, F, ENDO> S;
  constexpr bool IP = S::E && (C::IS_BN || sizeof(F) != sizeof(Fq<C>));
  Jac<F> r;
  Jac<F> tab[8];
  Aff<F> at[8];
  F zback;
  smul_build_table(tab, p);
  table_global_z<C>(at, tab, 8, zback);
  const int top = wave_uniform(sd->top);
  const uint32_t sgm = (uint32_t)wave_uniform((int)sd->sgm);
  jac_set_inf(r);
  for (int i = top; i >= 0; i--) {
    if (i != top) {
#pragma unroll 1
      for (int d4 = 0; d4 < 4; d4++) {
        if constexpr (IP)
          jac_dbl_ip(r);
        else
          jac_dbl(r, r);
      }
    }
#pragma unroll 1
    for (int s = 0; s < S::NS; s++) {
      const int a = wave_uniform((int)sd->d[s * S::ND + i]);
      if (a == 0) continue;
      Aff<F> t = at[(a < 0 ? -a : a) - 1];
      if constexpr (S::E) endo_apply<C>(t, s);
      if ((a < 0) != (((sgm >> s) & 1u) != 0)) t.y = neg(t.y);
      if constexpr (IP)
        jac_madd_ip(r, t);
      else
        jac_madd(r, r, t);
    }
  }
  r.z = mul(r.z, zback);
  rout = r;
}

}
```

groth_sahai_rs_amd/csrc/gs_pairing.cuh:

```cuda
#pragma once
#include "gs_curve.cuh"

namespace gs {

template <class C> struct Proj2 {
  Fp2<C> x, y, z;
};
template <class C> struct GLine {
  Fp2<C> l0, lx, ly;
};
#if defined(GS_LINES_GENERAL)
template <class C> using Line = GLine<C>;
template <class C> GS_HD Line<C> line_real(const GLine<C>& l) { return l; }
template <class C> GS_HD Line<C> line_unit(const GLine<C>& l) { return l; }
#else
template <class C> struct Line {
  Fp2<C> l0, lx;
  Fq<C> ly;
};
template <class C> GS_HD Line<C> line_real(const GLine<C>& l) {
  const bool z = is_zero(l.ly);
  const Fp2<C> cj = conj(l.ly);
  Line<C> r;
  r.l0 = select(z, l.l0, mul(l.l0, cj));
  r.lx = select(z, l.lx, mul(l.lx, cj));
  r.ly = add(sqr(l.ly.c0), sqr(l.ly.c1));
  return r;
}
template <class C> GS_HD Line<C> line_unit(const GLine<C>& l) {
  Line<C> r;
  if (is_zero(l.ly)) {
    r.l0 = l.l0;
    r.lx = l.lx;
    r.ly = fq_zero<C>();
    return r;
  }
  const Fp2<C> i = inv(l.ly);
  r.l0 = mul(l.l0, i);
  r.lx = mul(l.lx, i);
  r.ly = fq_one<C>();
  return r;
}
#endif

template <class C> GS_HD Fp2<C> twist_b3() {
  Fp2<C> r;
#pragma unroll
  for (int i = 0; i < C::L; i++) {
    r.c0.v[i] = C::B2X3_28[0][i];
    r.c1.v[i] = C::B2X3_28[1][i];
  }
  return r;
}

template <class C> GS_ML void miller_dbl(Proj2<C>& t, GLine<C>& l) {
  Fp2<C> xy = mul(t.x, t.y);
  Fp2<C> b = sqr(t.y);
  Fp2<C> c = sqr(t.z);
  Fp2<C> e;
  if constexpr (C::B2X3_XI_K != 0) {
    static_assert(C::B2X3_XI_K % 4 == 0 && C::B2X3_XI_K <= 12, "limb growth below: 2 x 3, then x 4");
    Fp2<C> x = norm(mul_small(norm(mul_small(mul_xi(c), C::B2X3_XI_K / 4)), 4));
    e.c0 = vreduce(x.c0);
    e.c1 = vreduce(x.c1);
  } else {
    e = mul(twist_b3<C>(), c);
  }
  Fp2<C> f = norm(add(dbl(e), e));
  Fp2<C> h = norm(sub(sub(sqr_l2(add(t.y, t.z)), b), c));
  Fp2<C> j = sqr(t.x);
  Fp2<C> e2 = sqr(e);
  l.l0 = norm(sub(b, e));
  l.lx = norm(neg(add(dbl(j), j)));
  l.ly = h;
  Fp2<C> e2x4 = norm(dbl(dbl(e2)));
  t.x = mul(norm(dbl(xy)), norm(sub(b, f)));
  t.y = norm(sub(sqr(norm(add(b, f))), add(dbl(e2x4), e2x4)));
  t.z = mul(b, norm(dbl(dbl(h))));
}

template <class C> GS_ML void miller_add(Proj2<C>& t, GLine<C>& l, const Aff<Fp2<C>>& q) {
  Fp2<C> theta = norm(sub(t.y, mul(q.y, t.z)));
  Fp2<C> lambda = norm(sub(t.x, mul(q.x, t.z)));
  Fp2<C> c = sqr(theta);
  Fp2<C> d = sqr(lambda);
  Fp2<C> e = mul(lambda, d);
  Fp2<C> f = mul(t.z, c);
  Fp2<C> g = mul(t.x, d);
  Fp2<C> h = norm(sub(add(e, f), dbl(g)));
  l.l0 = norm(sub(mul(theta, q.x), mul(lambda, q.y)));
  l.lx = neg(theta);
  l.ly = lambda;
  t.x = mul(lambda, h);
  t.y = norm(sub(mul(theta, norm(sub(g, h))), mul(e, t.y)));
  t.z = mul(t.z, e);
}

template <class C> struct LineAcc {
  ELine<C> pend;
  bool has = false;
#if !defined(GS_LINES_GENERAL)
  GS_HD void add(Fp12<C>& f, const Line<C>& l, const Aff<Fq<C>>& p) {
    const Fp2<C> cx = mul_fp(l.lx, p.x);
    const Fq<C> cy = mul(l.ly, p.y);
#if defined(GS_LINES2_ALL)
    GLine<C> g;
    g.l0 = l.l0, g.lx = cx, g.ly = Fp2<C>{cy, fq_zero<C>()};
    add_evaluated(f, g);
#else
    if (C::TWIST_M)
      f12_mul_by_014r(f, l.l0, cx, cy);
    else
      f12_mul_by_034r(f, cy, cx, l.l0);
#endif
  }
#endif
  GS_HD void add(Fp12<C>& f, const GLine<C>& l, const Aff<Fq<C>>& p) {
    GLine<C> g;
    g.l0 = l.l0, g.lx = mul_fp(l.lx, p.x), g.ly = mul_fp(l.ly, p.y);
    add_evaluated(f, g);
  }
  GS_HD void add_evaluated(Fp12<C>& f, const GLine<C>& l) {
    const Fp2<C>&cx = l.lx, &cy = l.ly;
#if defined(GS_LINES2_ALL)
    constexpr bool pair_lines = true;
#elif defined(GS_LINES2_NONE)
    constexpr bool pair_lines = false;
#else
    constexpr bool pair_lines = false;
#endif
    if (!pair_lines) {
      if (C::TWIST_M)
        f12_mul_by_014(f, l.l0, cx, cy);
      else
        f12_mul_by_034(f, cy, cx, l.l0);
      return;
    }
    ELine<C> e;
    if (C::TWIST_M) {
      e.a = l.l0;
      e.b = cx;
      e.c = cy;
    } else {
      e.a = cy;
      e.b = cx;
      e.c = l.l0;
    }
    if (has) {
      f12_mul_by_lines2(f, pend, e);
      has = false;
    } else {
      pend = e;
      has = true;
    }
  }
  GS_HD void flush(Fp12<C>& f) {
    if (has) {
      f12_mul_by_line(f, pend);
      has = false;
    }
  }
};

template <class C> constexpr int miller_line_count() {
  int n = 0;
  for (int i = C::LOOP_LEN - 2; i >= 0; i--) n += 1 + (C::LOOP[i] != 0 ? 1 : 0);
  return n + (C::IS_BN ? 2 : 0);
}
template <class C> GS_HD_NOINLINE void miller_line_table(Line<C>* out, const Aff<Fp2<C>>& q) {
  Proj2<C> t;
  t.x = q.x;
  t.y = q.y;
  t.z = one_of<Fp2<C>>();
  int n = 0;
  GLine<C> l;
  for (int i = C::LOOP_LEN - 2; i >= 0; i--) {
    miller_dbl(t, l);
    out[n++] = line_unit(l);
    int d = C::LOOP[i];
    if (d != 0) {
      Aff<Fp2<C>> qq = q;
      if (d < 0) qq.y = neg(qq.y);
      miller_add(t, l, qq);
      out[n++] = line_unit(l);
    }
  }
  if (C::IS_BN) {
    Aff<Fp2<C>> q1, q2;
    q1.x = mul(conj(q.x), frob_coeff<C>(1, 2));
    q1.y = mul(conj(q.y), frob_coeff<C>(1, 3));
    q2.x = mul(q.x, frob_coeff<C>(2, 2));
    q2.y = neg(mul(q.y, frob_coeff<C>(2, 3)));
    miller_add(t, l, q1);
    out[n++] = line_unit(l);
    miller_add(t, l, q2);
    out[n++] = line_unit(l);
  }
}

template <class C>
GS_HD_NOINLINE void multi_miller(Fp12<C>& fout, const Aff<Fq<C>>* ps, const Aff<Fp2<C>>* qs, int np, Proj2<C>* ts,
                                 bool* live, const Line<C>* const* fixed = nullptr) {
  Fp12<C> f;
  f12_one(f);
  bool any = false;
  for (int k = 0; k < np; k++) {
    live[k] = !(aff_is_inf(ps[k]) || aff_is_inf(qs[k]));
    any |= live[k];
    ts[k].x = qs[k].x;
    ts[k].y = qs[k].y;
    ts[k].z = one_of<Fp2<C>>();
  }
  if (!any) {
    fout = f;
    return;
  }
  GLine<C> l;
  LineAcc<C> acc;
  int li = 0;
  for (int i = C::LOOP_LEN - 2; i >= 0; i--) {
    acc.flush(f);
    f12_sqr(f, f);
    for (int k = 0; k < np; k++) {
      if (!live[k]) continue;
      if (fixed && fixed[k]) {
        acc.add(f, fixed[k][li], ps[k]);
        continue;
      }
      miller_dbl(ts[k], l);
      acc.add(f, l, ps[k]);
    }
    li++;
    int d = C::LOOP[i];
    if (d != 0) {
      for (int k = 0; k < np; k++) {
        if (!live[k]) continue;
        if (fixed && fixed[k]) {
          acc.add(f, fixed[k][li], ps[k]);
          continue;
        }
        Aff<Fp2<C>> q = qs[k];
        if (d < 0) q.y = neg(q.y);
        miller_add(ts[k], l, q);
        acc.add(f, l, ps[k]);
      }
      li++;
    }
  }
  if (C::IS_BN) {
    for (int k = 0; k < np; k++) {
      if (!live[k]) continue;
      if (fixed && fixed[k]) {
        acc.add(f, fixed[k][li], ps[k]);
        acc.add(f, fixed[k][li + 1], ps[k]);
        continue;
      }
      Aff<Fp2<C>> q1, q2;
      q1.x = mul(conj(qs[k].x), frob_coeff<C>(1, 2));
      q1.y = mul(conj(qs[k].y), frob_coeff<C>(1, 3));
      q2.x = mul(qs[k].x, frob_coeff<C>(2, 2));
      q2.y = neg(mul(qs[k].y, frob_coeff<C>(2, 3)));
      miller_add(ts[k], l, q1);
      acc.add(f, l, ps[k]);
      miller_add(ts[k], l, q2);
      acc.add(f, l, ps[k]);
    }
  }
  acc.flush(f);
  if (C::LOOP_NEG) f12_conj(f, f);
  fout = f;
}

template <class C>
GS_HD_NOINLINE void multi_miller2(Fp12<C>& f0out, Fp12<C>& f1out, const Aff<Fq<C>>* p0, const Aff<Fq<C>>* p1,
                                  const Aff<Fp2<C>>* qs, int np, Proj2<C>* ts, uint8_t* live,
                                  const Line<C>* const* fixed = nullptr) {
  Fp12<C>&f0 = f0out, &f1 = f1out;
  f12_one(f0);
  f12_one(f1);
  bool any = false;
  for (int k = 0; k < np; k++) {
    bool q_ok = !aff_is_inf(qs[k]);
    uint8_t l = 0;
    if (q_ok && !aff_is_inf(p0[k])) l |= 1;
    if (q_ok && !aff_is_inf(p1[k])) l |= 2;
    live[k] = l;
    any |= (l != 0);
    ts[k].x = qs[k].x;
    ts[k].y = qs[k].y;
    ts[k].z = one_of<Fp2<C>>();
  }
  if (!any) return;
  GLine<C> g;
  Line<C> l;
  LineAcc<C> acc0, acc1;
  int li = 0;
  for (int i = C::LOOP_LEN - 2; i >= 0; i--) {
    acc0.flush(f0);
    acc1.flush(f1);
    f12_sqr(f0, f0);
    f12_sqr(f1, f1);
    for (int k = 0; k < np; k++) {
      if (!live[k]) continue;
      const Line<C>* lp = &l;
      if (fixed && fixed[k])
        lp = &fixed[k][li];
      else {
        miller_dbl(ts[k], g);
        l = line_real(g);
      }
      if (live[k] & 1) acc0.add(f0, *lp, p0[k]);
      if (live[k] & 2) acc1.add(f1, *lp, p1[k]);
    }
    li++;
    int d = C::LOOP[i];
    if (d != 0) {
      for (int k = 0; k < np; k++) {
        if (!live[k]) continue;
        const Line<C>* lp = &l;
        if (fixed && fixed[k]) {
          lp = &fixed[k][li];
        } else {
          Aff<Fp2<C>> q = qs[k];
          if (d < 0) q.y = neg(q.y);
          miller_add(ts[k], g, q);
          l = line_real(g);
        }
        if (live[k] & 1) acc0.add(f0, *lp, p0[k]);
        if (live[k] & 2) acc1.add(f1, *lp, p1[k]);
      }
      li++;
    }
  }
  if (C::IS_BN) {
    for (int k = 0; k < np; k++) {
      if (!live[k]) continue;
      if (fixed && fixed[k]) {
        for (int e = 0; e < 2; e++) {
          if (live[k] & 1) acc0.add(f0, fixed[k][li + e], p0[k]);
          if (live[k] & 2) acc1.add(f1, fixed[k][li + e], p1[k]);
        }
        continue;
      }
      Aff<Fp2<C>> q1, q2;
      q1.x = mul(conj(qs[k].x), frob_coeff<C>(1, 2));
      q1.y = mul(conj(qs[k].y), frob_coeff<C>(1, 3));
      q2.x = mul(qs[k].x, frob_coeff<C>(2, 2));
      q2.y = neg(mul(qs[k].y, frob_coeff<C>(2, 3)));
      miller_add(ts[k], g, q1);
      l = line_real(g);
      if (live[k] & 1) acc0.add(f0, l, p0[k]);
      if (live[k] & 2) acc1.add(f1, l, p1[k]);
      miller_add(ts[k], g, q2);
      l = line_real(g);
      if (live[k] & 1) acc0.add(f0, l, p0[k]);
      if (live[k] & 2) acc1.add(f1, l, p1[k]);
    }
  }
  acc0.flush(f0);
  acc1.flush(f1);
  if (C::LOOP_NEG) {
    f12_conj(f0, f0);
    f12_conj(f1, f1);
  }
}

template <class C, class X>
GS_HD void multi_miller_pair(Fp12<C>& fout, int a, const Aff<Fq<C>>* ps, const Aff<Fp2<C>>* qown, uint32_t qok,
                                      int nstep, int np, Proj2<C>* ts, const Line<C>* const* fixed, X& xch) {
  Fp12<C> f;
  f12_one(f);
  uint32_t live = 0;
  for (int k = 0; k < np; k++)
    if (((qok >> k) & 1) && !aff_is_inf(ps[k])) live |= 1u << k;
  const int rounds = (nstep + 1) / 2;
  for (int r = 0; r < rounds; r++) {
    const Aff<Fp2<C>>& q = qown[r];
    ts[r].x = q.x;
    ts[r].y = q.y;
    ts[r].z = one_of<Fp2<C>>();
  }
  GLine<C> l;
  Line<C> lp;
  LineAcc<C> acc;
  int li = 0;
  auto products = [&](const GLine<C>& stepped, int ko, int kp) {
    const Line<C> mine = line_real(stepped);
    const bool own_ok = ko < nstep && ((live >> ko) & 1), par_ok = kp < nstep && ((live >> kp) & 1);
    xch.put(mine);
    if (own_ok && par_ok) {
      acc.add(f, mine, ps[ko]);
      lp = xch.get();
      acc.add(f, lp, ps[kp]);
    } else {
      lp = xch.get();
      if (own_ok || par_ok) {
        Line<C> use;
        use.l0 = select(own_ok, mine.l0, lp.l0);
        use.lx = select(own_ok, mine.lx, lp.lx);
        use.ly = select(own_ok, mine.ly, lp.ly);
        acc.add(f, use, ps[own_ok ? ko : kp]);
      }
    }
  };
  for (int i = C::LOOP_LEN - 2; i >= 0; i--) {
    acc.flush(f);
    f12_sqr(f, f);
    for (int r = 0; r < rounds; r++) {
      const int ko = 2 * r + a, kp = 2 * r + 1 - a;
      miller_dbl(ts[r], l);
      products(l, ko, kp);
    }
    for (int k = nstep; k < np; k++)
      if ((live >> k) & 1) acc.add(f, fixed[k][li], ps[k]);
    li++;
    int d = C::LOOP[i];
    if (d != 0) {
      for (int r = 0; r < rounds; r++) {
        const int ko = 2 * r + a, kp = 2 * r + 1 - a;
        Aff<Fp2<C>> q = qown[r];
        if (d < 0) q.y = neg(q.y);
        miller_add(ts[r], l, q);
        products(l, ko, kp);
      }
      for (int k = nstep; k < np; k++)
        if ((live >> k) & 1) acc.add(f, fixed[k][li], ps[k]);
      li++;
    }
  }
  if (C::IS_BN) {
    for (int e = 0; e < 2; e++) {
      for (int r = 0; r < rounds; r++) {
        const int ko = 2 * r + a, kp = 2 * r + 1 - a;
        const Aff<Fp2<C>>& q = qown[r];
        Aff<Fp2<C>> qf;
        if (e == 0) {
          qf.x = mul(conj(q.x), frob_coeff<C>(1, 2));
          qf.y = mul(conj(q.y), frob_coeff<C>(1, 3));
        } else {
          qf.x = mul(q.x, frob_coeff<C>(2, 2));
          qf.y = neg(mul(q.y, frob_coeff<C>(2, 3)));
        }
        miller_add(ts[r], l, qf);
        products(l, ko, kp);
      }
      for (int k = nstep; k < np; k++)
        if ((live >> k) & 1) acc.add(f, fixed[k][li + e], ps[k]);
    }
  }
  acc.flush(f);
  if (C::LOOP_NEG) f12_conj(f, f);
  fout = f;
}

template <class C> GS_HD_NOINLINE void f12_exp_by_x_gs(Fp12<C>& r, const Fp12<C>& f) {
  Fp12<C> acc = f;
  int top = 63;
  while (!((C::X_ABS >> top) & 1)) top--;
  int since = 0;
  for (int i = top - 1; i >= 0; i--) {
#if defined(GS_FE_INLINE)
    f12_cyclo_sqr_inl(acc, acc);
#else
    f12_cyclo_sqr(acc, acc);
#endif
    if ((C::X_ABS >> i) & 1) {
      Fp12<C> t = acc;
      f12_mul(t, t, f);
      acc = t;
      since = 0;
    } else if (++since == 3) {
      f12_vreduce_inl(acc);
      since = 0;
    }
  }
  if (C::X_NEG) f12_conj(acc, acc);
  r = acc;
}

template <class C> GS_HD void cyclo_sqr_compressed(Fp2<C>& g2, Fp2<C>& g3, Fp2<C>& g4, Fp2<C>& g5) {
  Fp2<C> t2, t3, t4, t5;
  fp4_sqr(t2, t3, g2, g3);
  fp4_sqr(t4, t5, g4, g5);
  Fp2<C> x5 = norm(mul_xi(t5));
  Fp2<C> z = add(x5, g2);
  g2 = norm(add(dbl(z), x5));
  z = sub(t4, g3);
  g3 = norm(add(dbl(z), t4));
  z = sub(t2, g4);
  g4 = norm(add(dbl(z), t2));
  z = add(t3, g5);
  g5 = norm(add(dbl(z), t3));
}
template <class C> constexpr int x_popcount() {
  int n = 0;
  for (int i = 0; i < 64; i++) n += (int)((C::X_ABS >> i) & 1);
  return n;
}
template <class C> GS_HD_NOINLINE void f12_exp_by_x_karabina(Fp12<C>& r, const Fp12<C>& f) {
  constexpr int NS = x_popcount<C>() - (int)(C::X_ABS & 1);
  Fp2<C> sv[NS][4];
  Fp2<C> g2 = f.c1.c0, g3 = f.c0.c2, g4 = f.c0.c1, g5 = f.c1.c2;
  int top = 63;
  while (!((C::X_ABS >> top) & 1)) top--;
  int ns = 0, since = 0;
  unsigned long long sk0 = GS_STAMP_T();
#pragma unroll 1
  for (int i = 1; i <= top; i++) {
    cyclo_sqr_compressed<C>(g2, g3, g4, g5);
    if (++since == 3) {
#define GS_VR2(x) x.c0 = vreduce(x.c0), x.c1 = vreduce(x.c1)
      GS_VR2(g2);
      GS_VR2(g3);
      GS_VR2(g4);
      GS_VR2(g5);
#undef GS_VR2
      since = 0;
    }
    if ((C::X_ABS >> i) & 1) {
      sv[ns][0] = g2, sv[ns][1] = g3, sv[ns][2] = g4, sv[ns][3] = g5;
      ns++;
    }
  }
  unsigned long long sk1 = GS_STAMP_T();
  GS_STAMP_ADD(10, sk1 - sk0);
  Fp2<C> den[NS], pre[NS];
  Fp2<C> acc = one_of<Fp2<C>>();
  bool degenerate = false;
  for (int k = 0; k < NS; k++) {
    den[k] = norm(dbl(dbl(sv[k][0])));
    degenerate |= is_zero(den[k]);
    pre[k] = acc;
    acc = mul(acc, den[k]);
  }
  if (degenerate) {
    f12_exp_by_x_gs(r, f);
    return;
  }
  Fp2<C> suf = inv(acc);
  GS_STAMP_ADD(11, GS_STAMP_T() - sk1);
  Fp12<C> out;
  bool have = false;
  if (C::X_ABS & 1) {
    out = f;
    have = true;
  }
  for (int k = NS - 1; k >= 0; k--) {
    Fp2<C> i4z2 = mul(suf, pre[k]);
    suf = mul(suf, den[k]);
    const Fp2<C>&z2 = sv[k][0], &z3 = sv[k][1], &z4 = sv[k][2], &z5 = sv[k][3];
    Fp2<C> s4 = sqr(z4);
    Fp2<C> num = norm(sub(add(mul_xi(sqr(z5)), add(dbl(s4), s4)), dbl(z3)));
    Fp2<C> z1 = mul(num, i4z2);
    Fp2<C> b = mul(z3, z4);
    Fp2<C> t = norm(sub(add(dbl(sqr(z1)), mul(z2, z5)), add(dbl(b), b)));
    Fp2<C> z0 = norm(add(mul_xi(t), one_of<Fp2<C>>()));
    Fp12<C> v;
    v.c0.c0 = z0, v.c1.c1 = z1, v.c1.c0 = z2, v.c0.c2 = z3, v.c0.c1 = z4, v.c1.c2 = z5;
    if (have) {
      f12_mul_inl(out, out, v);
    } else {
      out = v;
      have = true;
    }
  }
  if (C::X_NEG) f12_conj(out, out);
  r = out;
  GS_STAMP_ADD(12, GS_STAMP_T() - sk0);
}
template <class C> GS_HD void f12_exp_by_x(Fp12<C>& r, const Fp12<C>& f) {
#if !defined(GS_NO_KARABINA)
  if constexpr (x_popcount<C>() <= 8) {
    f12_exp_by_x_karabina(r, f);
    return;
  }
#endif
  f12_exp_by_x_gs(r, f);
}

template <class C> struct ExpXLane {
  GS_HD void operator()(Fp12<C>& r, const Fp12<C>& f) const { f12_exp_by_x(r, f); }
};
template <class C, class EX> GS_HD_NOINLINE void final_exp_with(Fp12<C>& out, const Fp12<C>& f, EX& ex) {
  Fp12<C> r, t, y0, y1, y2;
  unsigned long long se0 = GS_STAMP_T();
  if (!C::IS_BN) {
#pragma unroll 1
    for (int step = 0; step < 9; step++) {
      Fp12<C>*pd, *pb;
      const Fp12<C>* pa;
      switch (step) {
        case 0:
          f12_inv(t, f);
          f12_conj(r, f);
          pd = &r, pa = &r, pb = &t;
          break;
        case 1:
          f12_frob(t, r, 2);
          pd = &r, pa = &r, pb = &t;
          break;
// ... 78 lines not shown
```

groth_sahai_rs_amd/csrc/gs_params_bls12_381.h:

```cpp
#pragma once
#include <stdint.h>
#ifndef GS_DEVCONST
#if defined(__HIPCC__)
#define GS_DEVCONST __device__
#else
#define GS_DEVCONST
#endif
#endif
namespace gs {
struct Bls12_381 {
  static constexpr int N = 12;
  static constexpr int NR = 8;
  static constexpr int CURVE_ID = 0;
  static constexpr bool TWIST_M = true;
  static constexpr bool IS_BN = false;
  static constexpr int XI_A = 1;
  GS_DEVCONST static constexpr uint32_t P[12] = {0xffffaaabu,0xb9feffffu,0xb153ffffu,0x1eabfffeu,0xf6b0f624u,0x6730d2a0u,0xf38512bfu,0x64774b84u,0x434bacd7u,0x4b1ba7b6u,0x397fe69au,0x1a0111eau};
  GS_DEVCONST static constexpr uint32_t P_INV = 0xfffcfffdu;
  GS_DEVCONST static constexpr uint32_t P_ONE[12] = {0x0002fffdu,0x76090000u,0xc40c0002u,0xebf4000bu,0x53c758bau,0x5f489857u,0x70525745u,0x77ce5853u,0xa256ec6du,0x5c071a97u,0xfa80e493u,0x15f65ec3u};
  GS_DEVCONST static constexpr uint32_t P_R2[12] = {0x1c341746u,0xf4df1f34u,0x09d104f1u,0x0a76e6a6u,0x4c95b6d5u,0x8de5476cu,0x939d83c0u,0x67eb88a9u,0xb519952du,0x9a793e85u,0x92cae3aau,0x11988fe5u};
  GS_DEVCONST static constexpr uint32_t P_M2[12] = {0xffffaaa9u,0xb9feffffu,0xb153ffffu,0x1eabfffeu,0xf6b0f624u,0x6730d2a0u,0xf38512bfu,0x64774b84u,0x434bacd7u,0x4b1ba7b6u,0x397fe69au,0x1a0111eau};
  static constexpr int P_BITS = 381;
  GS_DEVCONST static constexpr uint32_t Q[8] = {0x00000001u,0xffffffffu,0xfffe5bfeu,0x53bda402u,0x09a1d805u,0x3339d808u,0x299d7d48u,0x73eda753u};
  GS_DEVCONST static constexpr uint32_t Q_INV = 0xffffffffu;
  GS_DEVCONST static constexpr uint32_t Q_ONE[8] = {0xfffffffeu,0x00000001u,0x00034802u,0x5884b7fau,0xecbc4ff5u,0x998c4fefu,0xacc5056fu,0x1824b159u};
  GS_DEVCONST static constexpr uint32_t Q_R2[8] = {0xf3f29c6du,0xc999e990u,0x87925c23u,0x2b6cedcbu,0x7254398fu,0x05d31496u,0x9f59ff11u,0x0748d9d9u};
  static constexpr int Q_BITS = 255;
  GS_DEVCONST static constexpr uint32_t TWO_INV[12] = {0x00015554u,0x18040000u,0x3ab00001u,0x85500005u,0x253c276fu,0x633cb57cu,0x31ebb502u,0x6e22d1ecu,0xf2d14ca2u,0xd3916126u,0x1a006596u,0x17fbb857u};
  GS_DEVCONST static constexpr uint32_t B1[12] = {0x000cfff3u,0xaa270000u,0xfc34000au,0x53cc0032u,0x6b0a807fu,0x478fe97au,0xe6ba24d7u,0xb1d37ebeu,0xbf78ab2fu,0x8ec9733bu,0x3d83de7eu,0x09d64551u};
  GS_DEVCONST static constexpr uint32_t B2[2][12] = {{0x000cfff3u,0xaa270000u,0xfc34000au,0x53cc0032u,0x6b0a807fu,0x478fe97au,0xe6ba24d7u,0xb1d37ebeu,0xbf78ab2fu,0x8ec9733bu,0x3d83de7eu,0x09d64551u},{0x000cfff3u,0xaa270000u,0xfc34000au,0x53cc0032u,0x6b0a807fu,0x478fe97au,0xe6ba24d7u,0xb1d37ebeu,0xbf78ab2fu,0x8ec9733bu,0x3d83de7eu,0x09d64551u}};
  GS_DEVCONST static constexpr uint32_t B2X3[2][12] = {{0x0027552eu,0x44760000u,0x43480020u,0xdcb8009au,0x4a6e8b59u,0x6f7ee9ceu,0xc0a95bc6u,0xb10330b7u,0xfb1e54b7u,0x6140b1fcu,0x7f0bb4e1u,0x0381be09u},{0x0027552eu,0x44760000u,0x43480020u,0xdcb8009au,0x4a6e8b59u,0x6f7ee9ceu,0xc0a95bc6u,0xb10330b7u,0xfb1e54b7u,0x6140b1fcu,0x7f0bb4e1u,0x0381be09u}};
  static constexpr int B2X3_XI_K = 12;
  GS_DEVCONST static constexpr uint32_t FROB1[6][2][12] = {{{0x0002fffdu,0x76090000u,0xc40c0002u,0xebf4000bu,0x53c758bau,0x5f489857u,0x70525745u,0x77ce5853u,0xa256ec6du,0x5c071a97u,0xfa80e493u,0x15f65ec3u},{0x00000000u,0x00000000u,0x00000000u,0x00000000u,0x00000000u,0x00000000u,0x00000000u,0x00000000u,0x00000000u,0x00000000u,0x00000000u,0x00000000u}},{{0xb319d465u,0x07089552u,0xb50a8313u,0xc6695f92u,0xd117228fu,0x97e83cccu,0xb2dc29eeu,0xa35baecau,0x5daace4du,0x1ce393eau,0xb0fb66ebu,0x08f2220fu},{0x4ce5d646u,0xb2f66aadu,0xfc497cecu,0x5842a06bu,0x2599d394u,0xcf4895d4u,0x40a8e8d0u,0xc11b9cbau,0xe5a0de89u,0x2e3813cbu,0x88847fafu,0x110eefdau}},{{0x00000000u,0x00000000u,0x00000000u,0x00000000u,0x00000000u,0x00000000u,0x00000000u,0x00000000u,0x00000000u,0x00000000u,0x00000000u,0x00000000u},{0x8671f071u,0xcd03c9e4u,0x1fcda5d2u,0x5dab2246u,0xd3851b95u,0x587042afu,0x01bacb9eu,0x8eb60ebeu,0x83d050d2u,0x03f97d6eu,0x54638741u,0x18f02065u}},{{0x5aa30fdau,0x7bcfa7a2u,0x2a927e7cu,0xdc17dec1u,0x6b4ebef1u,0x2f088dd8u,0xda74d4a7u,0xd1ca2087u,0x96cebc1du,0x2da25966u,0xbbfd87d2u,0x0e2b7eedu},{0x5aa30fdau,0x7bcfa7a2u,0x2a927e7cu,0xdc17dec1u,0x6b4ebef1u,0x2f088dd8u,0xda74d4a7u,0xd1ca2087u,0x96cebc1du,0x2da25966u,0xbbfd87d2u,0x0e2b7eedu}},{{0x867545c3u,0x890dc9e4u,0x3285a5d5u,0x2af32253u,0x309b7e2cu,0x50880866u,0x7e881024u,0xa20d1b8cu,0xe2db9068u,0x14e4f04fu,0x1564853au,0x14e56d3fu},{0x00000000u,0x00000000u,0x00000000u,0x00000000u,0x00000000u,0x00000000u,0x00000000u,0x00000000u,0x00000000u,0x00000000u,0x00000000u,0x00000000u}},{{0x0dbce43fu,0x82d83cf5u,0xdf9d018fu,0xa2813e53u,0x3c65e181u,0xc6f0caa5u,0x8d50fe95u,0x7525cf52u,0xf4798a6bu,0x4a85ed50u,0x6cf8eebdu,0x171da0fdu},{0xf242c66cu,0x3726c30au,0xd1b6fe70u,0x7c2ac1aau,0xba4b14a2u,0xa04007fbu,0x66341429u,0xef517c32u,0x4ed2226bu,0x0095ba65u,0xcc86f7ddu,0x02e370ecu}}};
  GS_DEVCONST static constexpr uint32_t FROB2[6][2][12] = {{{0x0002fffdu,0x76090000u,0xc40c0002u,0xebf4000bu,0x53c758bau,0x5f489857u,0x70525745u,0x77ce5853u,0xa256ec6du,0x5c071a97u,0xfa80e493u,0x15f65ec3u},{0x00000000u,0x00000000u,0x00000000u,0x00000000u,0x00000000u,0x00000000u,0x00000000u,0x00000000u,0x00000000u,0x00000000u,0x00000000u,0x00000000u}},{{0x798dba3au,0xecfb361bu,0x91865a2cu,0xc100ddb8u,0x232bda8eu,0x0ec08ff1u,0xf1ca4721u,0xd5c13cc6u,0xbf7b5c04u,0x47222a47u,0xe51c5f59u,0x0110f184u},{0x00000000u,0x00000000u,0x00000000u,0x00000000u,0x00000000u,0x00000000u,0x00000000u,0x00000000u,0x00000000u,0x00000000u,0x00000000u,0x00000000u}},{{0x798a64e8u,0x30f1361bu,0x7ece5a2au,0xf3b8ddabu,0xc61577f7u,0x16a8ca3au,0x74fd029bu,0xc26a2ff8u,0x60701c6eu,0x3636b766u,0x241b6160u,0x051ba4abu},{0x00000000u,0x00000000u,0x00000000u,0x00000000u,0x00000000u,0x00000000u,0x00000000u,0x00000000u,0x00000000u,0x00000000u,0x00000000u,0x00000000u}},{{0xfffcaaaeu,0x43f5ffffu,0xed47fffdu,0x32b7fff2u,0xa2e99d69u,0x07e83a49u,0x8332bb7au,0xeca8f331u,0xa0f4c069u,0xef148d1eu,0x3eff0206u,0x040ab326u},{0x00000000u,0x00000000u,0x00000000u,0x00000000u,0x00000000u,0x00000000u,0x00000000u,0x00000000u,0x00000000u,0x00000000u,0x00000000u,0x00000000u}},{{0x8671f071u,0xcd03c9e4u,0x1fcda5d2u,0x5dab2246u,0xd3851b95u,0x587042afu,0x01bacb9eu,0x8eb60ebeu,0x83d050d2u,0x03f97d6eu,0x54638741u,0x18f02065u},{0x00000000u,0x00000000u,0x00000000u,0x00000000u,0x00000000u,0x00000000u,0x00000000u,0x00000000u,0x00000000u,0x00000000u,0x00000000u,0x00000000u}},{{0x867545c3u,0x890dc9e4u,0x3285a5d5u,0x2af32253u,0x309b7e2cu,0x50880866u,0x7e881024u,0xa20d1b8cu,0xe2db9068u,0x14e4f04fu,0x1564853au,0x14e56d3fu},{0x00000000u,0x00000000u,0x00000000u,0x00000000u,0x00000000u,0x00000000u,0x00000000u,0x00000000u,0x00000000u,0x00000000u,0x00000000u,0x00000000u}}};
  GS_DEVCONST static constexpr uint32_t FROB3[6][2][12] = {{{0x0002fffdu,0x76090000u,0xc40c0002u,0xebf4000bu,0x53c758bau,0x5f489857u,0x70525745u,0x77ce5853u,0xa256ec6du,0x5c071a97u,0xfa80e493u,0x15f65ec3u},{0x00000000u,0x00000000u,0x00000000u,0x00000000u,0x00000000u,0x00000000u,0x00000000u,0x00000000u,0x00000000u,0x00000000u,0x00000000u,0x00000000u}},{{0xa55c9ad1u,0x3e2f585du,0x86c18183u,0x4294213du,0x8b623732u,0x382844c8u,0x19103e18u,0x92ad2afdu,0xac7cf0b9u,0x1d794e4fu,0x7d825ec8u,0x0bd592fcu},{0x5aa30fdau,0x7bcfa7a2u,0x2a927e7cu,0xdc17dec1u,0x6b4ebef1u,0x2f088dd8u,0xda74d4a7u,0xd1ca2087u,0x96cebc1du,0x2da25966u,0xbbfd87d2u,0x0e2b7eedu}},{{0x00000000u,0x00000000u,0x00000000u,0x00000000u,0x00000000u,0x00000000u,0x00000000u,0x00000000u,0x00000000u,0x00000000u,0x00000000u,0x00000000u},{0x0002fffdu,0x76090000u,0xc40c0002u,0xebf4000bu,0x53c758bau,0x5f489857u,0x70525745u,0x77ce5853u,0xa256ec6du,0x5c071a97u,0xfa80e493u,0x15f65ec3u}},{{0xa55c9ad1u,0x3e2f585du,0x86c18183u,0x4294213du,0x8b623732u,0x382844c8u,0x19103e18u,0x92ad2afdu,0xac7cf0b9u,0x1d794e4fu,0x7d825ec8u,0x0bd592fcu},{0xa55c9ad1u,0x3e2f585du,0x86c18183u,0x4294213du,0x8b623732u,0x382844c8u,0x19103e18u,0x92ad2afdu,0xac7cf0b9u,0x1d794e4fu,0x7d825ec8u,0x0bd592fcu}},{{0xfffcaaaeu,0x43f5ffffu,0xed47fffdu,0x32b7fff2u,0xa2e99d69u,0x07e83a49u,0x8332bb7au,0xeca8f331u,0xa0f4c069u,0xef148d1eu,0x3eff0206u,0x040ab326u},{0x00000000u,0x00000000u,0x00000000u,0x00000000u,0x00000000u,0x00000000u,0x00000000u,0x00000000u,0x00000000u,0x00000000u,0x00000000u,0x00000000u}},{{0x5aa30fdau,0x7bcfa7a2u,0x2a927e7cu,0xdc17dec1u,0x6b4ebef1u,0x2f088dd8u,0xda74d4a7u,0xd1ca2087u,0x96cebc1du,0x2da25966u,0xbbfd87d2u,0x0e2b7eedu},{0xa55c9ad1u,0x3e2f585du,0x86c18183u,0x4294213du,0x8b623732u,0x382844c8u,0x19103e18u,0x92ad2afdu,0xac7cf0b9u,0x1d794e4fu,0x7d825ec8u,0x0bd592fcu}}};
  static constexpr uint64_t X_ABS = 0xd201000000010000ull;
  static constexpr bool X_NEG = true;
  static constexpr int LOOP_LEN = 64;
  GS_DEVCONST static constexpr int8_t LOOP[64] = {0,0,0,0,0,0,0,0,0,0,0,0,0,0,0,0,1,0,0,0,0,0,0,0,0,0,0,0,0,0,0,0,0,0,0,0,0,0,0,0,0,0,0,0,0,0,0,0,1,0,0,0,0,0,0,0,0,1,0,0,1,0,1,1};
  static constexpr bool LOOP_NEG = true;
  GS_DEVCONST static constexpr uint32_t G1_GEN[2][12] = {{0xfd530c16u,0x5cb38790u,0x9976fff5u,0x7817fc67u,0x143ba1c1u,0x154f95c7u,0xf3d0e747u,0xf0ae6acdu,0x21dbf440u,0xedce6eccu,0x9e0bfb75u,0x12017741u},{0x0ce72271u,0xbaac93d5u,0x7918fd8eu,0x8c22631au,0x570725ceu,0xdd595f13u,0x50405194u,0x51ac5829u,0xad0059c0u,0x0e1c8c3fu,0x5008a26au,0x0bbc3efcu}};
  GS_DEVCONST static constexpr uint32_t G2_GEN[2][2][12] = {{{0x02940a10u,0xf5f28fa2u,0x87b4961au,0xb3f5fb26u,0x3e2ae580u,0xa1a893b5u,0x1a3caee9u,0x9894999du,0x1863366bu,0x6f67b763u,0x4350bcd7u,0x05819192u},{0x9e23f606u,0xa5a9c075u,0xbccd60c3u,0xaaa0c59du,0xe2867806u,0x3bb17e18u,0x8541b367u,0x1b1ab6ccu,0xf2158547u,0xc2b6ed0eu,0x7360edf3u,0x11922a09u}},{{0x60494c4au,0x4c730af8u,0x5e369c5au,0x597cfa1fu,0xaa0a635au,0xe7e6856cu,0x6e0d495fu,0xbbefb5e9u,0xf0ef25a2u,0x07d3a975u,0x7e80dae5u,0x0083fd8eu},{0xdf64b05du,0xadc0fc92u,0x2b1461dcu,0x18aa270au,0x3be4eba0u,0x86adac6au,0xc93da33au,0x79495c4eu,0xa43ccaedu,0xe7175850u,0x63de1bf2u,0x0b2bc2a1u}}};
  static constexpr int L = 14;
  GS_DEVCONST static constexpr int32_t P28[14] = {268413611,267386879,67108793,268430101,103030443,168782607,258420946,255349035,74926980,79351158,195540547,241804465,32127359,106513};
  static constexpr uint32_t P28_INV = 268238845u;
  static constexpr float INV_PTOP2 = 3.497494308e-14f;
  GS_DEVCONST static constexpr int32_t ONE28[14] = {55049400,226492416,176409,13493970,208802528,138027152,3630751,228652862,162569026,19495856,85318031,1231484,106560762,22394};
  GS_DEVCONST static constexpr int32_t K_IN28[14] = {135160473,55574580,246491222,233514649,211322480,82798231,118064104,172912617,65577043,248456990,203477795,116089733,75436678,87770};
  GS_DEVCONST static constexpr int32_t K_OUT28[14] = {196605,9437184,201327222,48192,146467828,91569269,90130584,117777780,130963539,91145943,119183266,239678912,247724672,89957};
  GS_DEVCONST static constexpr int32_t RR28[14] = {17002733,114410309,237256034,247749715,61986394,9646461,189740704,97992840,202435186,140890392,120719989,265669968,214476633,51412};
  GS_DEVCONST static constexpr int32_t RRR28[14] = {33011856,43306061,166965026,190555500,213237964,202217308,210348229,113862836,36074218,152955081,55988902,139032520,69516217,82347};
  static constexpr int INV_DIVSTEPS = 878;
  GS_DEVCONST static constexpr uint32_t SQRT_EXP[12] = {0xffffeaabu,0xee7fbfffu,0xac54ffffu,0x07aaffffu,0x3dac3d89u,0xd9cc34a8u,0x3ce144afu,0xd91dd2e1u,0x90d2eb35u,0x92c6e9edu,0x8e5ff9a6u,0x0680447au};
  GS_DEVCONST static constexpr uint32_t HALF_P[12] = {0xffffd555u,0xdcff7fffu,0x58a9ffffu,0x0f55ffffu,0x7b587b12u,0xb3986950u,0x79c2895fu,0xb23ba5c2u,0x21a5d66bu,0x258dd3dbu,0x1cbff34du,0x0d0088f5u};
  GS_DEVCONST static constexpr uint32_t P_WORDS[12] = {0xffffaaabu,0xb9feffffu,0xb153ffffu,0x1eabfffeu,0xf6b0f624u,0x6730d2a0u,0xf38512bfu,0x64774b84u,0x434bacd7u,0x4b1ba7b6u,0x397fe69au,0x1a0111eau};
  GS_DEVCONST static constexpr uint32_t R_WORDS[8] = {0x00000001u,0xffffffffu,0xfffe5bfeu,0x53bda402u,0x09a1d805u,0x3339d808u,0x299d7d48u,0x73eda753u};
  GS_DEVCONST static constexpr int32_t B2_28[2][14] = {{220197600,100663296,705639,53975880,29903744,15237699,14523006,109305080,113405195,77983426,72836668,4925937,157807592,89577},{220197600,100663296,705639,53975880,29903744,15237699,14523006,109305080,113405195,77983426,72836668,4925937,157807592,89577}};
  GS_DEVCONST static constexpr int32_t B1_28[14] = {220197600,100663296,705639,53975880,29903744,15237699,14523006,109305080,113405195,77983426,72836668,4925937,157807592,89577};
  GS_DEVCONST static constexpr int32_t B2X3_28[2][14] = {{123765578,35651586,136334786,161938349,152085800,245018794,63598036,85652624,190361624,75247962,95864366,68039792,140732600,55706},{123765578,35651586,136334786,161938349,152085800,245018794,63598036,85652624,190361624,75247962,95864366,68039792,140732600,55706}};
  GS_DEVCONST static constexpr int32_t FROB1_28[6][2][14] = {{{55049400,226492416,176409,13493970,208802528,138027152,3630751,228652862,162569026,19495856,85318031,1231484,106560762,22394},{0,0,0,0,0,0,0,0,0,0,0,0,0,0}},{{166836792,248851249,51584792,154304858,56352319,130327775,208630885,40286156,44881151,212744589,37992072,174141729,120403823,7230},{101576819,18535630,15524001,114125243,46678124,38454832,49790061,215062879,30045829,135042025,157548474,67662736,180158992,99282}},{{0,0,0,0,0,0,0,0,0,0,0,0,0,0},{37886809,200165479,30609410,74842500,80498822,209116160,179210523,180816594,266565572,239503032,99423592,150315392,2841631,53668}},{{54406951,53093802,41722322,203293854,205484154,5622420,33622907,62470036,224036522,173297123,89563204,163999141,59688213,52899},{54406951,53093802,41722322,203293854,205484154,5622420,33622907,62470036,224036522,173297123,89563204,163999141,59688213,52899}},{{92936209,158222439,30785820,88336470,20865894,78707857,182841275,141034000,160699143,258998889,184741623,151546876,109402393,76062},{0,0,0,0,0,0,0,0,0,0,0,0,0,0}},{{221243743,33509595,93307115,89163256,261836474,135950195,242253792,102756192,482217,117606257,127555277,69705414,180092037,60129},{47169868,233877284,242237134,179266844,109629425,32832411,16167154,152592843,74444763,230180357,67985269,172099051,120470778,46383}}};
  GS_DEVCONST static constexpr int32_t FROB2_28[6][2][14] = {{{55049400,226492416,176409,13493970,208802528,138027152,3630751,228652862,162569026,19495856,85318031,1231484,106560762,22394},{0,0,0,0,0,0,0,0,0,0,0,0,0,0}},{{230526802,67221400,36499383,193587601,22531621,228101903,79210422,74532441,76796864,108283581,96116954,91489073,29285728,52845},{0,0,0,0,0,0,0,0,0,0,0,0,0,0}},{{175477402,109164440,36322973,180093631,82164549,90074750,75579671,114315035,182663293,88787724,10798923,90257589,191160422,30450},{0,0,0,0,0,0,0,0,0,0,0,0,0,0}},{{213364211,40894463,66932384,254936131,162663371,30755454,254790195,26696173,180793410,59855301,110222516,240572981,194002053,84118},{0,0,0,0,0,0,0,0,0,0,0,0,0,0}},{{37886809,200165479,30609410,74842500,80498822,209116160,179210523,180816594,266565572,239503032,99423592,150315392,2841631,53668},{0,0,0,0,0,0,0,0,0,0,0,0,0,0}},{{92936209,158222439,30785820,88336470,20865894,78707857,182841275,141034000,160699143,258998889,184741623,151546876,109402393,76062},{0,0,0,0,0,0,0,0,0,0,0,0,0,0}}};
  GS_DEVCONST static constexpr int32_t FROB3_28[6][2][14] = {{{55049400,226492416,176409,13493970,208802528,138027152,3630751,228652862,162569026,19495856,85318031,1231484,106560762,22394},{0,0,0,0,0,0,0,0,0,0,0,0,0,0}},{{214006660,214293077,25386471,65136247,165981745,163160186,224798039,192878999,119325914,174489490,105977342,77805324,240874602,53613},{54406951,53093802,41722322,203293854,205484154,5622420,33622907,62470036,224036522,173297123,89563204,163999141,59688213,52899}},{{0,0,0,0,0,0,0,0,0,0,0,0,0,0},{55049400,226492416,176409,13493970,208802528,138027152,3630751,228652862,162569026,19495856,85318031,1231484,106560762,22394}},{{214006660,214293077,25386471,65136247,165981745,163160186,224798039,192878999,119325914,174489490,105977342,77805324,240874602,53613},{214006660,214293077,25386471,65136247,165981745,163160186,224798039,192878999,119325914,174489490,105977342,77805324,240874602,53613}},{{213364211,40894463,66932384,254936131,162663371,30755454,254790195,26696173,180793410,59855301,110222516,240572981,194002053,84118},{0,0,0,0,0,0,0,0,0,0,0,0,0,0}},{{54406951,53093802,41722322,203293854,205484154,5622420,33622907,62470036,224036522,173297123,89563204,163999141,59688213,52899},{214006660,214293077,25386471,65136247,165981745,163160186,224798039,192878999,119325914,174489490,105977342,77805324,240874602,53613}}};
  static constexpr bool HAS_ENDO = true;
  GS_DEVCONST static constexpr uint32_t LAMBDA[4] = {0xffffffffu,0x00000000u,0x0001a402u,0xac45a401u};
  GS_DEVCONST static constexpr int32_t BETA_28[14] = {37886809,200165479,30609410,74842500,80498822,209116160,179210523,180816594,266565572,239503032,99423592,150315392,2841631,53668};
  GS_DEVCONST static constexpr uint32_t XABS_LIMBS[2] = {0x00010000u,0xd2010000u};
  GS_DEVCONST static constexpr int32_t PSI_X_28[2][14] = {{0,0,0,0,0,0,0,0,0,0,0,0,0,0},{92936209,158222439,30785820,88336470,20865894,78707857,182841275,141034000,160699143,258998889,184741623,151546876,109402393,76062}};
  GS_DEVCONST static constexpr int32_t PSI_Y_28[2][14] = {{214006660,214293077,25386471,65136247,165981745,163160186,224798039,192878999,119325914,174489490,105977342,77805324,240874602,53613},{54406951,53093802,41722322,203293854,205484154,5622420,33622907,62470036,224036522,173297123,89563204,163999141,59688213,52899}};
  GS_DEVCONST static constexpr int32_t PSI2_X_28[14] = {37886809,200165479,30609410,74842500,80498822,209116160,179210523,180816594,266565572,239503032,99423592,150315392,2841631,53668};
  GS_DEVCONST static constexpr int32_t PSI2_Y_28[14] = {213364211,40894463,66932384,254936131,162663371,30755454,254790195,26696173,180793410,59855301,110222516,240572981,194002053,84118};
  GS_DEVCONST static constexpr int32_t PSI3_X_28[2][14] = {{0,0,0,0,0,0,0,0,0,0,0,0,0,0},{213364211,40894463,66932384,254936131,162663371,30755454,254790195,26696173,180793410,59855301,110222516,240572981,194002053,84118}};
  GS_DEVCONST static constexpr int32_t PSI3_Y_28[2][14] = {{54406951,53093802,41722322,203293854,205484154,5622420,33622907,62470036,224036522,173297123,89563204,163999141,59688213,52899},{214006660,214293077,25386471,65136247,165981745,163160186,224798039,192878999,119325914,174489490,105977342,77805324,240874602,53613}};
};
}
```

groth_sahai_rs_amd/csrc/gs_params_bn254.h:

```cpp
#pragma once
#include <stdint.h>
#ifndef GS_DEVCONST
#if defined(__HIPCC__)
#define GS_DEVCONST __device__
#else
#define GS_DEVCONST
#endif
#endif
namespace gs {
struct Bn254 {
  static constexpr int N = 8;
  static constexpr int NR = 8;
  static constexpr int CURVE_ID = 1;
  static constexpr bool TWIST_M = false;
  static constexpr bool IS_BN = true;
  static constexpr int XI_A = 9;
  GS_DEVCONST static constexpr uint32_t P[8] = {0xd87cfd47u,0x3c208c16u,0x6871ca8du,0x97816a91u,0x8181585du,0xb85045b6u,0xe131a029u,0x30644e72u};
  GS_DEVCONST static constexpr uint32_t P_INV = 0xe4866389u;
  GS_DEVCONST static constexpr uint32_t P_ONE[8] = {0xc58f0d9du,0xd35d438du,0xf5c70b3du,0x0a78eb28u,0x7879462cu,0x666ea36fu,0x9a07df2fu,0x0e0a77c1u};
  GS_DEVCONST static constexpr uint32_t P_R2[8] = {0x538afa89u,0xf32cfc5bu,0xd44501fbu,0xb5e71911u,0x0a417ff6u,0x47ab1effu,0xcab8351fu,0x06d89f71u};
  GS_DEVCONST static constexpr uint32_t P_M2[8] = {0xd87cfd45u,0x3c208c16u,0x6871ca8du,0x97816a91u,0x8181585du,0xb85045b6u,0xe131a029u,0x30644e72u};
  static constexpr int P_BITS = 254;
  GS_DEVCONST static constexpr uint32_t Q[8] = {0xf0000001u,0x43e1f593u,0x79b97091u,0x2833e848u,0x8181585du,0xb85045b6u,0xe131a029u,0x30644e72u};
  GS_DEVCONST static constexpr uint32_t Q_INV = 0xefffffffu;
  GS_DEVCONST static constexpr uint32_t Q_ONE[8] = {0x4ffffffbu,0xac96341cu,0x9f60cd29u,0x36fc7695u,0x7879462eu,0x666ea36fu,0x9a07df2fu,0x0e0a77c1u};
  GS_DEVCONST static constexpr uint32_t Q_R2[8] = {0xae216da7u,0x1bb8e645u,0xe35c59e3u,0x53fe3ab1u,0x53bb8085u,0x8c49833du,0x7f4e44a5u,0x0216d0b1u};
  static constexpr int Q_BITS = 254;
  GS_DEVCONST static constexpr uint32_t TWO_INV[8] = {0x4f060572u,0x87bee7d2u,0x2f1c6ae5u,0xd0fd2addu,0xfcfd4f44u,0x8f5f7492u,0x3d9cbfacu,0x1f37631au};
  GS_DEVCONST static constexpr uint32_t B1[8] = {0x50ad28d7u,0x7a17caa9u,0xe15521b9u,0x1f6ac17au,0x696bd284u,0x334bea4eu,0xce179d8eu,0x2a1f6744u};
  GS_DEVCONST static constexpr uint32_t B2[2][8] = {{0x77b802a8u,0x3bf938e3u,0x3633535du,0x020b1b27u,0x49755260u,0x26b7edf0u,0x4384a86du,0x2514c632u},{0xd1dcff67u,0x38e7ecccu,0x93ce0d3eu,0x65f0b37du,0x22ac00aau,0xd749d0ddu,0x4a688d4du,0x0141b9ceu}};
  GS_DEVCONST static constexpr uint32_t B2X3[2][8] = {{0xb62e0d6au,0x3baa927cu,0xd1b664fdu,0xd71e7c52u,0xd95d4664u,0x03873e63u,0x082ab8f4u,0x0e75b5b1u},{0x7596fe35u,0xaab7c666u,0xbb6a27bau,0x31d21a78u,0x680401ffu,0x85dd7297u,0xdf39a7e9u,0x03c52d6au}};
  static constexpr int B2X3_XI_K = 0;
  GS_DEVCONST static constexpr uint32_t FROB1[6][2][8] = {{{0xc58f0d9du,0xd35d438du,0xf5c70b3du,0x0a78eb28u,0x7879462cu,0x666ea36fu,0x9a07df2fu,0x0e0a77c1u},{0x00000000u,0x00000000u,0x00000000u,0x00000000u,0x00000000u,0x00000000u,0x00000000u,0x00000000u}},{{0x33144907u,0xaf9ba696u,0x87afb78au,0xca6b1d73u,0xf08a2087u,0x11bded5eu,0x1a1f3a7cu,0x02f34d75u},{0x4c492d72u,0xa222ae23u,0x565de15bu,0xd00f02a4u,0x53dfc926u,0xdc2ff3a2u,0xb3899551u,0x10a75716u}},{{0x4563ab30u,0xb5773b10u,0xa9aa6454u,0x347f91c8u,0x242e0991u,0x7a007127u,0x118214ecu,0x1956bcd8u},{0xa0aa4757u,0x6e849f1eu,0x89f89141u,0xaa1c7b6du,0xfae0ca3au,0xb6e713cdu,0x4e82ebc3u,0x26694fbbu}},{{0x2936b629u,0xe4bbdd0cu,0xe133bacbu,0xbb30f162u,0xf9645366u,0x31a9d1b6u,0xa500f8ddu,0x253570beu},{0x5ffe77c7u,0xa1d77ce4u,0x7826d1dbu,0x07affd11u,0xbb7edc6bu,0x6d16bd27u,0x85defeccu,0x2c872002u}},{{0x843abe92u,0x7361d77fu,0x273411fbu,0xa5bb2bd3u,0x4b3e2399u,0x9c941f31u,0xbb9fd3ecu,0x15df9cddu},{0x4bd8c949u,0x5dddfd15u,0xa4445b60u,0x62cb29a5u,0x0c7dd2b9u,0x37bc870au,0x3171f0fdu,0x24830a9du}},{{0x41690fe7u,0xc970692fu,0x27694b0bu,0xe2403421u,0x83c459e8u,0x32bee66bu,0x0ab08841u,0x12aabcedu},{0x40aebfa9u,0x0d485d23u,0xab2fcc57u,0x05193418u,0x8a4910f5u,0xd3b0a40bu,0x35d2925au,0x2f21ebb5u}}};
  GS_DEVCONST static constexpr uint32_t FROB2[6][2][8] = {{{0xc58f0d9du,0xd35d438du,0xf5c70b3du,0x0a78eb28u,0x7879462cu,0x666ea36fu,0x9a07df2fu,0x0e0a77c1u},{0x00000000u,0x00000000u,0x00000000u,0x00000000u,0x00000000u,0x00000000u,0x00000000u,0x00000000u}},{{0x00fa1bf2u,0xca8d8005u,0x68b39769u,0xf0c5d614u,0xad0d4418u,0x0e201271u,0xbad856e6u,0x04290f65u},{0x00000000u,0x00000000u,0x00000000u,0x00000000u,0x00000000u,0x00000000u,0x00000000u,0x00000000u}},{{0x13e80b9cu,0x3350c88eu,0xdb5e56b9u,0x7dce557cu,0xb615564au,0x6001b4b8u,0x020217e0u,0x2682e617u},{0x00000000u,0x00000000u,0x00000000u,0x00000000u,0x00000000u,0x00000000u,0x00000000u,0x00000000u}},{{0x12edefaau,0x68c34889u,0x72aabf4fu,0x8d087f68u,0x09081231u,0x51e1a247u,0x4729c0fau,0x2259d6b1u},{0x00000000u,0x00000000u,0x00000000u,0x00000000u,0x00000000u,0x00000000u,0x00000000u,0x00000000u}},{{0xd782e155u,0x71930c11u,0xffbe3323u,0xa6bb947cu,0xd4741444u,0xaa303344u,0x26594943u,0x2c3b3f0du},{0x00000000u,0x00000000u,0x00000000u,0x00000000u,0x00000000u,0x00000000u,0x00000000u,0x00000000u}},{{0xc494f1abu,0x08cfc388u,0x8d1373d4u,0x19b31514u,0xcb6c0213u,0x584e90fdu,0xdf2f8849u,0x09e1685bu},{0x00000000u,0x00000000u,0x00000000u,0x00000000u,0x00000000u,0x00000000u,0x00000000u,0x00000000u}}};
  GS_DEVCONST static constexpr uint32_t FROB3[6][2][8] = {{{0xc58f0d9du,0xd35d438du,0xf5c70b3du,0x0a78eb28u,0x7879462cu,0x666ea36fu,0x9a07df2fu,0x0e0a77c1u},{0x00000000u,0x00000000u,0x00000000u,0x00000000u,0x00000000u,0x00000000u,0x00000000u,0x00000000u}},{{0x4e46d97du,0x36531618u,0xd4c96d9fu,0x0af7129eu,0xca1009b5u,0x659da72fu,0x83a20d23u,0x08116d89u},{0xc39c1939u,0xb1df4af7u,0x8a73bf7fu,0x3d9f0287u,0x8caf0ae0u,0x9b222092u,0xeff054a6u,0x26684515u}},{{0x16ad6badu,0xc9af22f7u,0x4aa662b2u,0xb311782au,0xe248c7f4u,0x19eeaf64u,0xe3439f82u,0x20273e77u},{0xf7ce93acu,0xacc02860u,0x7ba76b4cu,0x3933d581u,0x446c8467u,0x69e6188bu,0x4417cc55u,0x0a46036du}},{{0xaf46471eu,0x5764af0au,0x873e0fc1u,0xdc50792eu,0x881d04f6u,0x86a673ffu,0x3c30a74cu,0x0b2eddb4u},{0x787e8580u,0x9a490f32u,0xf04af8b1u,0x8fd16d7fu,0xc6027bf2u,0x4b39888eu,0x5b52a15du,0x03dd2e70u}},{{0x7b6762dfu,0x448a93a5u,0x28fdeadfu,0xbfd62df5u,0x0e9bd47au,0xd858f5d0u,0x3476ec58u,0x06b03d4du},{0xbcc936d1u,0x2b19daf4u,0x56f4299fu,0xa1a54e7au,0x5adeaef1u,0xb533eee0u,0x84dda0b2u,0x170c812bu}},{{0x75cf559fu,0xe0bc4b22u,0xc154e60fu,0xc238b945u,0x929a7d5eu,0x803982a5u,0xf7e4a37eu,0x15ce052du},{0xbf3799a7u,0x2d28efbdu,0x1ad60773u,0x9b097e3cu,0xaf4a535bu,0x982d4113u,0xe3056063u,0x24e18991u}}};
  static constexpr uint64_t X_ABS = 0x44e992b44a6909f1ull;
  static constexpr bool X_NEG = false;
  static constexpr int LOOP_LEN = 66;
  GS_DEVCONST static constexpr int8_t LOOP[66] = {0,0,0,1,0,1,0,-1,0,0,-1,0,0,0,1,0,0,-1,0,-1,0,0,0,1,0,-1,0,0,0,0,-1,0,0,1,0,-1,0,0,1,0,0,0,0,0,-1,0,0,-1,0,1,0,-1,0,0,0,-1,0,-1,0,0,0,1,0,-1,0,1};
  static constexpr bool LOOP_NEG = false;
  GS_DEVCONST static constexpr uint32_t G1_GEN[2][8] = {{0xc58f0d9du,0xd35d438du,0xf5c70b3du,0x0a78eb28u,0x7879462cu,0x666ea36fu,0x9a07df2fu,0x0e0a77c1u},{0x8b1e1b3au,0xa6ba871bu,0xeb8e167bu,0x14f1d651u,0xf0f28c58u,0xccdd46deu,0x340fbe5eu,0x1c14ef83u}};
  GS_DEVCONST static constexpr uint32_t G2_GEN[2][2][8] = {{{0x02bc2026u,0x8e83b5d1u,0x497b0172u,0xdceb1935u,0x97811adfu,0xfbb82647u,0xaf96503bu,0x19573841u},{0xa84c6140u,0xafb4737du,0x5802d8c4u,0x6043dd5au,0x52a02f86u,0x09e950fcu,0x3aea7b6bu,0x14fef083u}},{{0x886be9f6u,0x619dfa9du,0xf59e9b78u,0xfe7fd297u,0x231b7dfeu,0xff9e1a62u,0xae9e4206u,0x28fd7eebu},{0xc71856eeu,0x64095b56u,0x327d3cbbu,0xdc57f922u,0x33351076u,0x55f935beu,0x93fd6482u,0x0da4a0e6u}}};
  static constexpr int L = 10;
  GS_DEVCONST static constexpr int32_t P28[10] = {142409031,34128237,30051644,111744647,140351361,191371285,163074117,236132866,6573682,3};
  static constexpr uint32_t P28_INV = 75916169u;
  static constexpr float INV_PTOP2 = 1.231709042e-09f;
  GS_DEVCONST static constexpr int32_t ONE28[10] = {168693142,111503912,91066263,31901995,249956604,17138120,144666204,147168414,120954792,0};
  GS_DEVCONST static constexpr int32_t K_IN28[10] = {146210464,175364601,9831375,193333901,145963144,157451143,193695069,162022466,236203989,0};
  GS_DEVCONST static constexpr int32_t K_OUT28[10] = {93261213,97794268,118177235,246583132,103549560,116885396,258371235,161512946,235567041,0};
  GS_DEVCONST static constexpr int32_t RR28[10] = {74005574,196643059,237682909,29670299,64610745,203061996,46675328,63655842,157167273,0};
  GS_DEVCONST static constexpr int32_t RRR28[10] = {266160126,186936205,33545765,190180742,21740766,181491448,75707147,94037804,31419118,0};
  static constexpr int INV_DIVSTEPS = 586;
  GS_DEVCONST static constexpr uint32_t SQRT_EXP[8] = {0xb61f3f52u,0x4f082305u,0x5a1c72a3u,0x65e05aa4u,0xa0605617u,0x6e14116du,0xb84c680au,0x0c19139cu};
  GS_DEVCONST static constexpr uint32_t HALF_P[8] = {0x6c3e7ea3u,0x9e10460bu,0xb438e546u,0xcbc0b548u,0x40c0ac2eu,0xdc2822dbu,0x7098d014u,0x18322739u};
  GS_DEVCONST static constexpr uint32_t P_WORDS[8] = {0xd87cfd47u,0x3c208c16u,0x6871ca8du,0x97816a91u,0x8181585du,0xb85045b6u,0xe131a029u,0x30644e72u};
  GS_DEVCONST static constexpr uint32_t R_WORDS[8] = {0xf0000001u,0x43e1f593u,0x79b97091u,0x2833e848u,0x8181585du,0xb85045b6u,0xe131a029u,0x30644e72u};
  GS_DEVCONST static constexpr int32_t B2_28[2][10] = {{187688155,136643569,57298256,39951603,109389214,184234337,195895417,213958046,158638292,0},{235398570,55845783,212433874,152113795,94281753,73146108,92244205,174242486,253000206,0}};
  GS_DEVCONST static constexpr int32_t B1_28[10] = {237643970,66076281,4763334,95705986,212998900,51414362,165563156,173069787,94428921,1};
  GS_DEVCONST static constexpr int32_t B2X3_28[2][10] = {{26193553,141495253,171894769,119854809,59732186,15832100,50815341,105003228,207479422,1},{169324798,167537351,100430710,187905931,14409804,219438325,8297159,254292003,222129707,2}};
  GS_DEVCONST static constexpr int32_t FROB1_28[6][2][10] = {{{168693142,111503912,91066263,31901995,249956604,17138120,144666204,147168414,120954792,0},{0,0,0,0,0,0,0,0,0,0}},{{133812001,148983001,115022330,46996794,168023309,175683240,100797293,104742705,245863714,2},{209518029,201944753,158778186,246160477,210649201,171526389,209979198,53258301,211906895,1}},{{140912976,227821077,257547131,43198697,4610002,129533238,192242920,264698265,118551830,2},{181583081,26829790,145239802,134208534,183985030,63805091,202956448,46570285,87740487,1}},{{83059826,204664921,41965564,76289372,115534858,28421534,226234731,215327779,360179,1},{194284916,163115080,49151338,194679599,222240089,141486694,99351608,123507005,258529708,2}},{{208317434,262351505,119736315,220162787,142173683,256650118,190801998,887777,20243402,2},{212065600,159522258,90307450,196404121,152942189,255877235,2933919,102716968,126783104,1}},{{236217877,184571513,20657105,262931563,12266425,58945376,245120179,17071039,39035204,2},{133272975,216598130,9045820,148217946,34804272,136589691,85149247,39083786,3724050,3}}};
  GS_DEVCONST static constexpr int32_t FROB2_28[6][2][10] = {{{168693142,111503912,91066263,31901995,249956604,17138120,144666204,147168414,120954792,0},{0,0,0,0,0,0,0,0,0,0}},{{56972283,105669712,228356411,10331154,254790175,259527765,85027812,197267587,247015697,2},{0,0,0,0,0,0,0,0,0,0}},{{156714597,262601255,137290147,246864615,4833570,242389645,208797064,50099172,126060905,2},{0,0,0,0,0,0,0,0,0,0}},{{242151345,191059780,207420836,79842651,158830213,174233164,18407913,88964452,154054346,2},{0,0,0,0,0,0,0,0,0,0}},{{85436748,196893981,70130688,101413492,153996642,200278975,78046304,38865279,27993441,0},{0,0,0,0,0,0,0,0,0,0}},{{254129890,39962437,161196952,133315487,135517790,217417096,222712508,186033693,148948233,0},{0,0,0,0,0,0,0,0,0,0}}};
  GS_DEVCONST static constexpr int32_t FROB3_28[6][2][10] = {{{168693142,111503912,91066263,31901995,249956604,17138120,144666204,147168414,120954792,0},{0,0,0,0,0,0,0,0,0,0}},{{108585996,163715322,218319775,231133125,123814385,214601971,191797595,34346809,50823778,1},{96123710,168468400,191581498,95021741,156797909,110407292,197124267,71121725,146317535,2}},{{61390692,566658,101912546,190896821,252781826,172357921,109691706,102543529,75923538,0},{108446554,28537652,196884390,157548044,92417415,71878819,229727544,94151635,21874737,1}},{{59349205,97898772,256521535,35455274,24816503,162949751,205274842,20805086,6213503,2},{216559571,139448612,249335761,185500503,186546727,49884590,63722509,112625861,16479430,0}},{{89510400,196146886,188816392,12978662,192731260,152969732,227371785,121455318,225948398,2},{169967077,207684762,231786589,189991190,180115521,168398853,147329430,222040410,252340873,2}},{{28985521,261494431,138392687,227950732,71822300,127002716,154818457,149123811,144316937,1},{145156726,198296246,124114604,33294981,84601829,13823162,170288652,195619255,221755845,0}}};
  static constexpr bool HAS_ENDO = true;
  GS_DEVCONST static constexpr int32_t BETA_28[10] = {156714597,262601255,137290147,246864615,4833570,242389645,208797064,50099172,126060905,2};
  static constexpr int GLV1_SUBBITS = 127;
  GS_DEVCONST static constexpr uint32_t GLV1_G[2][5] = {{0x00ff6565u,0x5398fd03u,0xa773d2d2u,0x4ccef014u,0x00000002u},{0xc7e0b3d7u,0xd91d232eu,0x00000002u,0x00000000u,0x00000000u}};
  GS_DEVCONST static constexpr uint8_t GLV1_GS[2] = {0,0};
  GS_DEVCONST static constexpr uint32_t GLV1_B[2][2][4] = {{{0x7d4f1128u,0x8211bbebu,0xeeb859fcu,0x6f4d8248u},{0x94d213e3u,0x89d32568u,0x00000000u,0x00000000u}},{{0x94d213e3u,0x89d32568u,0x00000000u,0x00000000u},{0x1221250bu,0x0be4e154u,0xeeb859fdu,0x6f4d8248u}}};
  GS_DEVCONST static constexpr uint8_t GLV1_BS[2][2] = {{0,1},{0,0}};
  static constexpr int GLS2_SUBBITS = 65;
  GS_DEVCONST static constexpr uint32_t GLS2_G[4][7] = {{0x32e42728u,0x2dff2915u,0xa3e5577fu,0x55b4ca7bu,0xb0d92b95u,0x9e80318au,0x00000000u},{0x95d51bb1u,0x46f4bda9u,0xfc7184aeu,0x08e5da66u,0xb0d92b93u,0x9e80318au,0x00000000u},{0xc7e0b3d7u,0xd91d232eu,0x00000002u,0x00000000u,0x00000000u,0x00000000u,0x00000000u},{0xcef3cd3fu,0xc170977du,0xa3e5577du,0x55b4ca7bu,0xb0d92b95u,0x9e80318au,0x00000000u}};
  GS_DEVCONST static constexpr uint8_t GLS2_GS[4] = {0,0,0,0};
  GS_DEVCONST static constexpr uint32_t GLS2_B[4][4][2] = {{{0x94d213e3u,0x89d32568u},{0x00000000u,0x00000000u},{0x94d213e2u,0x89d32568u},{0x00000001u,0x00000000u}},{{0x94d213e2u,0x89d32568u},{0x4a6909f2u,0x44e992b4u},{0x4a6909f1u,0x44e992b4u},{0x4a6909f1u,0x44e992b4u}},{{0x4a6909f2u,0x44e992b4u},{0x4a6909f1u,0x44e992b4u},{0x4a6909f1u,0x44e992b4u},{0x94d213e2u,0x89d32568u}},{{0x94d213e3u,0x89d32568u},{0x4a6909f1u,0x44e992b4u},{0x4a6909f2u,0x44e992b4u},{0x4a6909f1u,0x44e992b4u}}};
  GS_DEVCONST static constexpr uint8_t GLS2_BS[4][4] = {{0,0,0,0},{0,0,1,0},{0,0,0,1},{0,1,1,1}};
};
}
```

groth_sahai_rs_amd/csrc/gs_tower.cuh:

```cuda
#pragma once
#include "gs_fq28.cuh"

#if defined(GS_F6_INLINE)
#define GS_F6 GS_HD
#else
#define GS_F6 GS_HD_NOINLINE
#endif
#if (defined(GS_MILLER_INLINE) || defined(GS_FE_INLINE)) && !defined(GS_LONGBR_OK) && defined(__HIPCC__)
#error "GS_MILLER_INLINE / GS_FE_INLINE need -mllvm -amdgpu-long-branch-factor=0 (csrc/Makefile probes it and passes -DGS_LONGBR_OK): without it the reserved long-branch register aliases the return address and the kernels never return"
#endif
#if defined(GS_MILLER_INLINE)
#define GS_ML GS_HD
#else
#define GS_ML GS_HD_NOINLINE
#endif

namespace gs {

template <class C> using Fq = Fq28<C>;
template <class C> using Fr = Fe<FrM<C>>;

template <class C> struct Fp2 {
  Fq<C> c0, c1;
};

template <class C> GS_HD Fp2<C> add(const Fp2<C>& a, const Fp2<C>& b) { return {add(a.c0, b.c0), add(a.c1, b.c1)}; }
template <class C> GS_HD Fp2<C> sub(const Fp2<C>& a, const Fp2<C>& b) { return {sub(a.c0, b.c0), sub(a.c1, b.c1)}; }
template <class C> GS_HD Fp2<C> neg(const Fp2<C>& a) { return {neg(a.c0), neg(a.c1)}; }
template <class C> GS_HD Fp2<C> dbl(const Fp2<C>& a) { return {dbl(a.c0), dbl(a.c1)}; }
template <class C> GS_HD Fp2<C> conj(const Fp2<C>& a) { return {a.c0, neg(a.c1)}; }
template <class C> GS_HD Fp2<C> norm(const Fp2<C>& a) { return {norm(a.c0), norm(a.c1)}; }
template <class C> GS_HD Fp2<C> mul_small(const Fp2<C>& a, int k) { return {mul_small(a.c0, k), mul_small(a.c1, k)}; }
template <class C> GS_HD bool is_zero(const Fp2<C>& a) { return is_zero(a.c0) && is_zero(a.c1); }
template <class C> GS_HD bool is_zero_limbs(const Fp2<C>& a) { return is_zero_limbs(a.c0) && is_zero_limbs(a.c1); }
template <class C> GS_HD bool eq(const Fp2<C>& a, const Fp2<C>& b) { return is_zero(sub(a, b)); }
template <class C> GS_HD void zero_window_check(const Fp2<C>& a) {
  zero_window_check(a.c0);
  zero_window_check(a.c1);
}
template <class C> GS_HD Fp2<C> select(bool c, const Fp2<C>& a, const Fp2<C>& b) {
  return {select(c, a.c0, b.c0), select(c, a.c1, b.c1)};
}
#if !defined(GS_FP2_KARATSUBA)
template <class C> GS_HD Fp2<C> mul(const Fp2<C>& a, const Fp2<C>& b) {
  Fp2<C> r;
  fp2mul28<C>(r.c0, r.c1, a.c0, a.c1, b.c0, b.c1);
  return r;
}
template <class C> GS_HD Fp2<C> mul_l2(const Fp2<C>& a, const Fp2<C>& b) { return mul(a, b); }
#else
template <class C> GS_HD Fp2<C> mul(const Fp2<C>& a, const Fp2<C>& b) {
  Fq<C> v0 = mul(a.c0, b.c0), v1 = mul(a.c1, b.c1);
  Fq<C> s = mul(add(a.c0, a.c1), add(b.c0, b.c1));
  return {sub(v0, v1), norm(sub(sub(s, v0), v1))};
}
template <class C> GS_HD Fp2<C> mul_l2(const Fp2<C>& a, const Fp2<C>& b) {
  Fq<C> v0 = mul(a.c0, b.c0), v1 = mul(a.c1, b.c1);
  Fq<C> s = mul(add(a.c0, a.c1), norm(add(b.c0, b.c1)));
  return {sub(v0, v1), norm(sub(sub(s, v0), v1))};
}
#endif
#if !defined(GS_FP2_KARATSUBA)
template <class C> GS_HD Fp2<C> sqr(const Fp2<C>& a) {
  Fp2<C> r;
  fp2sqr28<C>(r.c0, r.c1, a.c0, a.c1);
  return r;
}
template <class C> GS_HD Fp2<C> sqr_l2(const Fp2<C>& a) { return sqr(a); }
#else
template <class C> GS_HD Fp2<C> sqr(const Fp2<C>& a) {
  Fq<C> t = mul(a.c0, a.c1);
  return {mul(add(a.c0, a.c1), sub(a.c0, a.c1)), norm(dbl(t))};
}
template <class C> GS_HD Fp2<C> sqr_l2(const Fp2<C>& a) {
  Fq<C> t = mul(a.c0, a.c1);
  return {mul(add(a.c0, a.c1), norm(sub(a.c0, a.c1))), norm(dbl(t))};
}
#endif
template <class C>
GS_HD Fp2<C> dot3(const Fp2<C>& a0, const Fp2<C>& b0, const Fp2<C>& a1, const Fp2<C>& b1, const Fp2<C>& a2,
                  const Fp2<C>& b2) {
  Fp2<C> r;
  fp2dot3_28<C>(r.c0, r.c1, a0.c0, a0.c1, b0.c0, b0.c1, a1.c0, a1.c1, b1.c0, b1.c1, a2.c0, a2.c1, b2.c0, b2.c1);
  return r;
}
template <class C>
GS_HD Fp2<C> dot3(const Fp2<C>& a0, const Fp2<C>& b0, const Fp2<C>& a1, const Fp2<C>& b1, const Fp2<C>& a2,
                  const Fq<C>& r) {
  Fp2<C> o;
  fp2dot3r_28<C>(o.c0, o.c1, a0.c0, a0.c1, b0.c0, b0.c1, a1.c0, a1.c1, b1.c0, b1.c1, a2.c0, a2.c1, r);
  return o;
}
template <class C> GS_HD Fp2<C> mul_fp(const Fp2<C>& a, const Fq<C>& k) { return {mul(a.c0, k), mul(a.c1, k)}; }
template <class C> GS_HD Fp2<C> mul_xi(const Fp2<C>& a) {
  if (C::XI_A == 1) return {sub(a.c0, a.c1), add(a.c0, a.c1)};
  Fq<C> e0 = norm(mul_small(a.c0, 4)), e1 = norm(mul_small(a.c1, 4));
  e0 = norm(dbl(e0));
  e1 = norm(dbl(e1));
  return {sub(add(e0, a.c0), a.c1), add(add(e1, a.c1), a.c0)};
}
template <class C> GS_HD Fp2<C> inv(const Fp2<C>& a) {
  Fq<C> n = inv(add(sqr(a.c0), sqr(a.c1)));
  return {mul(a.c0, n), neg(mul(a.c1, n))};
}

template <class C> GS_HD Fq<C> mul_l2(const Fq<C>& a, const Fq<C>& b) { return mul(a, b); }
template <class C> GS_HD Fq<C> sqr_l2(const Fq<C>& a) { return sqr(a); }

template <class F> GS_HD F zero_of();
template <class F> GS_HD F one_of();
#define GS_ZERO_ONE(CURVE)                                                                     \
  template <> GS_HD Fq<CURVE> zero_of<Fq<CURVE>>() { return fq_zero<CURVE>(); }                \
  template <> GS_HD Fq<CURVE> one_of<Fq<CURVE>>() { return fq_one<CURVE>(); }                  \
  template <> GS_HD Fp2<CURVE> zero_of<Fp2<CURVE>>() { return {fq_zero<CURVE>(), fq_zero<CURVE>()}; } \
  template <> GS_HD Fp2<CURVE> one_of<Fp2<CURVE>>() { return {fq_one<CURVE>(), fq_zero<CURVE>()}; }

template <class C> struct Fp6 {
  Fp2<C> c0, c1, c2;
};

template <class C> GS_HD void f6_add(Fp6<C>& r, const Fp6<C>& a, const Fp6<C>& b) {
  r.c0 = add(a.c0, b.c0);
  r.c1 = add(a.c1, b.c1);
  r.c2 = add(a.c2, b.c2);
}
template <class C> GS_HD void f6_sub(Fp6<C>& r, const Fp6<C>& a, const Fp6<C>& b) {
  r.c0 = sub(a.c0, b.c0);
  r.c1 = sub(a.c1, b.c1);
  r.c2 = sub(a.c2, b.c2);
}
template <class C> GS_HD void f6_neg(Fp6<C>& r, const Fp6<C>& a) {
  r.c0 = neg(a.c0);
  r.c1 = neg(a.c1);
  r.c2 = neg(a.c2);
}
template <class C> GS_HD void f6_norm(Fp6<C>& r, const Fp6<C>& a) {
  r.c0 = norm(a.c0);
  r.c1 = norm(a.c1);
  r.c2 = norm(a.c2);
}
template <class C> GS_HD void f6_addn(Fp6<C>& r, const Fp6<C>& a, const Fp6<C>& b) {
  r.c0 = norm(add(a.c0, b.c0));
  r.c1 = norm(add(a.c1, b.c1));
  r.c2 = norm(add(a.c2, b.c2));
}
template <class C> GS_HD void f6_mul_v(Fp6<C>& r, const Fp6<C>& a) {
  Fp2<C> t = norm(mul_xi(a.c2));
  r.c2 = a.c1;
  r.c1 = a.c0;
  r.c0 = t;
}
template <class C> GS_F6 void f6_mul(Fp6<C>& r, const Fp6<C>& a, const Fp6<C>& b) {
  Fp2<C> v0 = mul(a.c0, b.c0), v1 = mul(a.c1, b.c1), v2 = mul(a.c2, b.c2);
  Fp2<C> t0 = sub(sub(mul_l2(add(a.c1, a.c2), add(b.c1, b.c2)), v1), v2);
  Fp2<C> t1 = sub(sub(mul_l2(add(a.c0, a.c1), add(b.c0, b.c1)), v0), v1);
  Fp2<C> t2 = sub(sub(mul_l2(add(a.c0, a.c2), add(b.c0, b.c2)), v0), v2);
  r.c0 = norm(add(v0, mul_xi(C::XI_A == 1 ? t0 : norm(t0))));
  r.c1 = norm(add(t1, mul_xi(v2)));
  r.c2 = norm(add(t2, v1));
}
template <class C> GS_F6 void f6_mul_by_01(Fp6<C>& r, const Fp6<C>& a, const Fp2<C>& b0, const Fp2<C>& b1) {
  Fp2<C> v0 = mul(a.c0, b0), v1 = mul(a.c1, b1);
  Fp2<C> t0 = mul(a.c2, b1), t2 = mul(a.c2, b0);
  Fp2<C> t1 = sub(sub(mul_l2(add(a.c0, a.c1), add(b0, b1)), v0), v1);
  r.c0 = norm(add(v0, mul_xi(t0)));
  r.c1 = norm(t1);
  r.c2 = norm(add(t2, v1));
}
template <class C> GS_HD void f6_mul_by_1(Fp6<C>& r, const Fp6<C>& a, const Fp2<C>& b1) {
  Fp2<C> t0 = norm(mul_xi(mul(a.c2, b1)));
  Fp2<C> t1 = mul(a.c0, b1);
  Fp2<C> t2 = mul(a.c1, b1);
  r.c0 = t0;
  r.c1 = t1;
  r.c2 = t2;
}
template <class C> GS_HD void f6_mul_fp2(Fp6<C>& r, const Fp6<C>& a, const Fp2<C>& k) {
  r.c0 = mul(a.c0, k);
  r.c1 = mul(a.c1, k);
  r.c2 = mul(a.c2, k);
}
template <class C> GS_HD_NOINLINE void f6_inv(Fp6<C>& r, const Fp6<C>& a) {
  Fp2<C> t0 = norm(sub(sqr(a.c0), mul_xi(mul(a.c1, a.c2))));
  Fp2<C> t1 = norm(sub(norm(mul_xi(sqr(a.c2))), mul(a.c0, a.c1)));
  Fp2<C> t2 = norm(sub(sqr(a.c1), mul(a.c0, a.c2)));
  Fp2<C> s = norm(add(mul(a.c2, t1), mul(a.c1, t2)));
  Fp2<C> n = norm(add(mul(a.c0, t0), mul_xi(s)));
  Fp2<C> ni = inv(n);
  r.c0 = mul(t0, ni);
  r.c1 = mul(t1, ni);
  r.c2 = mul(t2, ni);
}

template <class C> struct Fp12 {
  Fp6<C> c0, c1;
};

template <class C> GS_HD void f12_one(Fp12<C>& r) {
  Fp2<C> z = zero_of<Fp2<C>>();
  r.c0.c0 = one_of<Fp2<C>>();
  r.c0.c1 = z;
  r.c0.c2 = z;
  r.c1.c0 = z;
  r.c1.c1 = z;
  r.c1.c2 = z;
}
template <class C> GS_HD void f12_mul_inl(Fp12<C>& r, const Fp12<C>& a, const Fp12<C>& b) {
  Fp6<C> t0, t1, sa, sb, m;
  f6_mul(t0, a.c0, b.c0);
  f6_mul(t1, a.c1, b.c1);
  f6_addn(sa, a.c0, a.c1);
  f6_addn(sb, b.c0, b.c1);
  f6_mul(m, sa, sb);
  f6_sub(m, m, t0);
  f6_sub(m, m, t1);
  f6_norm(r.c1, m);
  f6_mul_v(t1, t1);
  f6_addn(r.c0, t0, t1);
}
template <class C> GS_HD_NOINLINE void f12_mul(Fp12<C>& r, const Fp12<C>& a, const Fp12<C>& b) { f12_mul_inl(r, a, b); }
template <class C> GS_ML void f12_sqr(Fp12<C>& r, const Fp12<C>& a) {
  Fp6<C> v0, s0, s1, t;
  f6_mul(v0, a.c0, a.c1);
  f6_addn(s0, a.c0, a.c1);
  f6_mul_v(t, a.c1);
  f6_addn(s1, a.c0, t);
  f6_mul(s0, s0, s1);
  f6_mul_v(t, v0);
  f6_sub(s0, s0, v0);
  f6_sub(s0, s0, t);
  f6_norm(r.c0, s0);
  f6_addn(r.c1, v0, v0);
}
template <class C> GS_HD void f12_conj(Fp12<C>& r, const Fp12<C>& a) {
  r.c0 = a.c0;
  f6_neg(r.c1, a.c1);
}
template <class C> GS_HD_NOINLINE void f12_inv(Fp12<C>& r, const Fp12<C>& a) {
  Fp6<C> t0, t1;
  f6_mul(t0, a.c0, a.c0);
  f6_mul(t1, a.c1, a.c1);
  f6_mul_v(t1, t1);
  f6_sub(t0, t0, t1);
  f6_norm(t0, t0);
  f6_inv(t1, t0);
  f6_mul(r.c0, a.c0, t1);
  f6_mul(t0, a.c1, t1);
  f6_neg(r.c1, t0);
}

template <class C> GS_HD Fp2<C> frob_coeff(int j, int k) {
  Fp2<C> r;
#pragma unroll
  for (int i = 0; i < C::L; i++) {
    r.c0.v[i] = (j == 1) ? C::FROB1_28[k][0][i] : (j == 2) ? C::FROB2_28[k][0][i] : C::FROB3_28[k][0][i];
    r.c1.v[i] = (j == 1) ? C::FROB1_28[k][1][i] : (j == 2) ? C::FROB2_28[k][1][i] : C::FROB3_28[k][1][i];
  }
  return r;
}
template <class C> GS_HD_NOINLINE void f12_frob(Fp12<C>& r, const Fp12<C>& a, int j) {
  bool cj = (j & 1);
  Fp2<C> x;
  x = cj ? conj(a.c0.c0) : a.c0.c0;
  r.c0.c0 = x;
  x = cj ? conj(a.c0.c1) : a.c0.c1;
  r.c0.c1 = mul(x, frob_coeff<C>(j, 2));
  x = cj ? conj(a.c0.c2) : a.c0.c2;
  r.c0.c2 = mul(x, frob_coeff<C>(j, 4));
  x = cj ? conj(a.c1.c0) : a.c1.c0;
  r.c1.c0 = mul(x, frob_coeff<C>(j, 1));
  x = cj ? conj(a.c1.c1) : a.c1.c1;
  r.c1.c1 = mul(x, frob_coeff<C>(j, 3));
  x = cj ? conj(a.c1.c2) : a.c1.c2;
  r.c1.c2 = mul(x, frob_coeff<C>(j, 5));
}

template <class C>
GS_ML void f12_mul_by_014(Fp12<C>& f, const Fp2<C>& l0, const Fp2<C>& l1, const Fp2<C>& l4) {
#if !defined(GS_NO_SPARSE_DOT3)
  const Fp2<C> a0 = f.c0.c0, a1 = f.c0.c1, a2 = f.c0.c2, b0 = f.c1.c0, b1 = f.c1.c1, b2 = f.c1.c2;
  Fp2<C> n00, n01, n02, n10, n11, n12;
  {
    const Fp2<C> xa2 = norm(mul_xi(a2));
    {
      const Fp2<C> xb1 = norm(mul_xi(b1));
      n00 = dot3(a0, l0, xa2, l1, xb1, l4);
    }
    const Fp2<C> xb2 = norm(mul_xi(b2));
    n10 = dot3(b0, l0, xb2, l1, xa2, l4);
    n01 = dot3(a1, l0, a0, l1, xb2, l4);
  }
  n02 = dot3(a2, l0, a1, l1, b0, l4);
  n11 = dot3(b1, l0, b0, l1, a0, l4);
  n12 = dot3(b2, l0, b1, l1, a1, l4);
  f.c0.c0 = n00;
  f.c0.c1 = n01;
  f.c0.c2 = n02;
  f.c1.c0 = n10;
  f.c1.c1 = n11;
  f.c1.c2 = n12;
  return;
#endif
  Fp6<C> aa, bb, s, t;
  f6_mul_by_01(aa, f.c0, l0, l1);
  f6_mul_by_1(bb, f.c1, l4);
  f6_addn(s, f.c0, f.c1);
  f6_mul_by_01(t, s, l0, norm(add(l1, l4)));
  f6_sub(t, t, aa);
  f6_sub(t, t, bb);
  f6_norm(f.c1, t);
  f6_mul_v(bb, bb);
  f6_addn(f.c0, aa, bb);
}
template <class C>
GS_ML void f12_mul_by_034(Fp12<C>& f, const Fp2<C>& l0, const Fp2<C>& l3, const Fp2<C>& l4) {
#if !defined(GS_NO_SPARSE_DOT3)
  const Fp2<C> a0 = f.c0.c0, a1 = f.c0.c1, a2 = f.c0.c2, b0 = f.c1.c0, b1 = f.c1.c1, b2 = f.c1.c2;
  Fp2<C> n00, n01, n02, n10, n11, n12;
  {
    const Fp2<C> xb2 = norm(mul_xi(b2));
    {
      const Fp2<C> xb1 = norm(mul_xi(b1));
      n00 = dot3(a0, l0, xb2, l3, xb1, l4);
    }
    n01 = dot3(a1, l0, b0, l3, xb2, l4);
  }
  {
    const Fp2<C> xa2 = norm(mul_xi(a2));
    n10 = dot3(b0, l0, a0, l3, xa2, l4);
  }
  n02 = dot3(a2, l0, b1, l3, b0, l4);
  n11 = dot3(b1, l0, a1, l3, a0, l4);
  n12 = dot3(b2, l0, a2, l3, a1, l4);
  f.c0.c0 = n00;
  f.c0.c1 = n01;
  f.c0.c2 = n02;
  f.c1.c0 = n10;
  f.c1.c1 = n11;
  f.c1.c2 = n12;
  return;
#endif
  Fp6<C> aa, bb, s, t;
  f6_mul_fp2(aa, f.c0, l0);
  f6_mul_by_01(bb, f.c1, l3, l4);
  f6_addn(s, f.c0, f.c1);
  f6_mul_by_01(t, s, norm(add(l0, l3)), l4);
  f6_sub(t, t, aa);
  f6_sub(t, t, bb);
  f6_norm(f.c1, t);
  f6_mul_v(bb, bb);
  f6_addn(f.c0, aa, bb);
}

template <class C>
GS_ML void f12_mul_by_014r(Fp12<C>& f, const Fp2<C>& l0, const Fp2<C>& l1, const Fq<C>& l4) {
#if !defined(GS_NO_SPARSE_DOT3)
  const Fp2<C> a0 = f.c0.c0, a1 = f.c0.c1, a2 = f.c0.c2, b0 = f.c1.c0, b1 = f.c1.c1, b2 = f.c1.c2;
  Fp2<C> n00, n01, n02, n10, n11, n12;
  {
    const Fp2<C> xa2 = norm(mul_xi(a2));
    {
      const Fp2<C> xb1 = norm(mul_xi(b1));
      n00 = dot3(a0, l0, xa2, l1, xb1, l4);
    }
    const Fp2<C> xb2 = norm(mul_xi(b2));
    n10 = dot3(b0, l0, xb2, l1, xa2, l4);
    n01 = dot3(a1, l0, a0, l1, xb2, l4);
  }
  n02 = dot3(a2, l0, a1, l1, b0, l4);
  n11 = dot3(b1, l0, b0, l1, a0, l4);
  n12 = dot3(b2, l0, b1, l1, a1, l4);
  f.c0.c0 = n00;
  f.c0.c1 = n01;
  f.c0.c2 = n02;
  f.c1.c0 = n10;
  f.c1.c1 = n11;
  f.c1.c2 = n12;
#else
  f12_mul_by_014(f, l0, l1, Fp2<C>{l4, fq_zero<C>()});
#endif
}
template <class C>
GS_ML void f12_mul_by_034r(Fp12<C>& f, const Fq<C>& l0, const Fp2<C>& l3, const Fp2<C>& l4) {
#if !defined(GS_NO_SPARSE_DOT3)
  const Fp2<C> a0 = f.c0.c0, a1 = f.c0.c1, a2 = f.c0.c2, b0 = f.c1.c0, b1 = f.c1.c1, b2 = f.c1.c2;
  Fp2<C> n00, n01, n02, n10, n11, n12;
  {
    const Fp2<C> xb2 = norm(mul_xi(b2));
    {
      const Fp2<C> xb1 = norm(mul_xi(b1));
      n00 = dot3(xb2, l3, xb1, l4, a0, l0);
    }
    n01 = dot3(b0, l3, xb2, l4, a1, l0);
  }
  {
    const Fp2<C> xa2 = norm(mul_xi(a2));
    n10 = dot3(a0, l3, xa2, l4, b0, l0);
  }
  n02 = dot3(b1, l3, b0, l4, a2, l0);
  n11 = dot3(a1, l3, a0, l4, b1, l0);
  n12 = dot3(a2, l3, a1, l4, b2, l0);
  f.c0.c0 = n00;
  f.c0.c1 = n01;
  f.c0.c2 = n02;
  f.c1.c0 = n10;
  f.c1.c1 = n11;
  f.c1.c2 = n12;
#else
  f12_mul_by_034(f, Fp2<C>{l0, fq_zero<C>()}, l3, l4);
#endif
}

template <class C> struct ELine {
  Fp2<C> a, b, c;
};
template <class C> GS_HD void f12_mul_by_line(Fp12<C>& f, const ELine<C>& e) {
  if (C::TWIST_M)
    f12_mul_by_014(f, e.a, e.b, e.c);
  else
    f12_mul_by_034(f, e.a, e.b, e.c);
}
template <class C> GS_ML void f12_mul_by_lines2(Fp12<C>& f, const ELine<C>& u, const ELine<C>& v) {
  Fp2<C> aa = mul(u.a, v.a), bb = mul(u.b, v.b), cc = mul(u.c, v.c);
  Fp2<C> ab = norm(sub(sub(mul_l2(add(u.a, u.b), add(v.a, v.b)), aa), bb));
  Fp2<C> ac = norm(sub(sub(mul_l2(add(u.a, u.c), add(v.a, v.c)), aa), cc));
  Fp2<C> bc = norm(sub(sub(mul_l2(add(u.b, u.c), add(v.b, v.c)), bb), cc));
  Fp6<C> c0, s, t0, t1, sa, m;
  Fp2<C> y0, y1;
// ... 113 lines not shown
```

groth_sahai_rs_amd/csrc/gs_wire.cuh:

```cuda
#pragma once
#include "gs_pairing.cuh"

namespace gs {

template <class C> GS_HD Fq28<C> fq_from_canonical(const uint32_t* w) {
  Fq28<C> t;
#pragma unroll
  for (int i = 0; i < C::L; i++) {
    int bit = 28 * i;
    int lo = bit >> 5, sh = bit & 31;
    uint64_t x = 0;
    if (lo < C::N) x = w[lo];
    if (lo + 1 < C::N) x |= (uint64_t)w[lo + 1] << 32;
    t.v[i] = (limb_t)((uint32_t)(x >> sh) & (uint32_t)M28);
  }
  Fq28<C> k;
#pragma unroll
  for (int i = 0; i < C::L; i++) k.v[i] = C::RR28[i];
  return mul(t, k);
}
template <class C> GS_HD void fq_to_canonical(uint32_t* w, const Fq28<C>& a) {
  Fq28<C> k = fq_zero<C>();
  k.v[0] = 1;
  Fq28<C> t = norm_full(mul(norm(a), k));
// ... 54 lines not shown
    if (dgt) {
      r = started ? mul(r, tab[dgt]) : tab[dgt];
      started = true;
    }
  }
  out = r;
}
template <class C> GS_HD Fq28<C> fq_sqrt(const Fq28<C>& a, bool& ok) {
  uint32_t e[C::N];
  for (int i = 0; i < C::N; i++) e[i] = C::SQRT_EXP[i];
  Fq28<C> r;
  fq_pow_words<C>(r, a, e);
  ok = eq(sqr(r), a);
  return r;
}
template <class C> GS_HD_NOINLINE Fp2<C> fp2_sqrt(const Fp2<C>& a, bool& ok) {
  Fq28<C> a0 = norm(a.c0), a1 = norm(a.c1);
  Fp2<C> r = {fq_zero<C>(), fq_zero<C>()};
  if (is_zero(a1)) {
    bool sq;
    Fq28<C> s = fq_sqrt<C>(a0, sq);
    if (sq) {
      r.c0 = s;
    } else {
      s = fq_sqrt<C>(neg(a0), sq);
      r.c1 = s;
    }
    ok = sq;
    return r;
  }
  bool sq;
  Fq28<C> n = fq_sqrt<C>(norm(add(sqr(a0), sqr(a1))), sq);
  if (!sq) {
    ok = false;
    return r;
  }
  Fq28<C> two = norm(dbl(fq_one<C>())), half = inv(two);
  Fq28<C> d = mul(norm(add(a0, n)), half);
  Fq28<C> c0 = fq_sqrt<C>(d, sq);
  if (!sq) {
    d = mul(norm(sub(a0, n)), half);
    c0 = fq_sqrt<C>(d, sq);
  }
  if (!sq) {
    ok = false;
    return r;
  }
  Fq28<C> c1 = mul(a1, inv(norm(dbl(c0))));
  r.c0 = c0;
  r.c1 = c1;
  Fp2<C> chk = sqr(r);
  ok = eq(chk, Fp2<C>{a0, a1});
  return r;
}
template <class C> GS_HD Fq28<C> f_sqrt(const Fq28<C>& a, bool& ok) { return fq_sqrt<C>(a, ok); }
template <class C> GS_HD Fp2<C> f_sqrt(const Fp2<C>& a, bool& ok) { return fp2_sqrt<C>(a, ok); }

template <class C> GS_HD void coord_words(uint32_t w[][C::N], const Fq28<C>& a) { fq_to_canonical<C>(w[0], a); }
template <class C> GS_HD void coord_words(uint32_t w[][C::N], const Fp2<C>& a) {
  fq_to_canonical<C>(w[0], a.c0);
  fq_to_canonical<C>(w[1], a.c1);
}
template <class C> GS_HD void coord_from_words(Fq28<C>& a, const uint32_t w[][C::N]) { a = fq_from_canonical<C>(w[0]); }
template <class C> GS_HD void coord_from_words(Fp2<C>& a, const uint32_t w[][C::N]) {
  a.c0 = fq_from_canonical<C>(w[0]);
  a.c1 = fq_from_canonical<C>(w[1]);
}
template <class F> struct NCoord;
template <class C> struct NCoord<Fq28<C>> { static constexpr int V = 1; };
template <class C> struct NCoord<Fp2<C>> { static constexpr int V = 2; };

template <class C, int NC> GS_HD bool y_is_largest(const uint32_t w[][C::N]) {
  uint32_t h[C::N];
  for (int i = 0; i < C::N; i++) h[i] = C::HALF_P[i];
  if (NC == 2 && !words_zero<C::N>(w[1])) return words_gt<C::N>(w[1], h);
  return words_gt<C::N>(w[0], h);
}

constexpr int FQB(int n_words) { return n_words * 4; }
template <class C> GS_HD void fq_put_bytes(uint8_t* o, const uint32_t* w) {
  constexpr int B = C::N * 4;
  for (int i = 0; i < B; i++) {
    uint8_t b = (uint8_t)(w[i >> 2] >> ((i & 3) * 8));
    if (C::IS_BN) o[i] = b; else o[B - 1 - i] = b;
  }
}
template <class C> GS_HD void fq_get_bytes(uint32_t* w, const uint8_t* in, uint8_t clear_mask, int flag_byte) {
  constexpr int B = C::N * 4;
  for (int i = 0; i < C::N; i++) w[i] = 0;
  for (int i = 0; i < B; i++) {
    int src = C::IS_BN ? i : B - 1 - i;
    uint8_t b = in[src];
    if (src == flag_byte) b &= (uint8_t)~clear_mask;
    w[i >> 2] |= (uint32_t)b << ((i & 3) * 8);
  }
}

template <class C> GS_HD Fq28<C> curve_rhs(const Fq28<C>& x) {
  Fq28<C> b;
  for (int i = 0; i < C::L; i++) b.v[i] = C::B1_28[i];
  return norm(add(mul(sqr(x), x), b));
}
template <class C> GS_HD Fp2<C> curve_rhs(const Fp2<C>& x) {
  Fp2<C> b;
  for (int i = 0; i < C::L; i++) {
    b.c0.v[i] = C::B2_28[0][i];
    b.c1.v[i] = C::B2_28[1][i];
  }
  return norm(add(mul(sqr(x), x), b));
}

template <class F> GS_HD_NOINLINE void jac_mul_bits(Jac<F>& r, const Aff<F>& p, const uint32_t* k, int nbits) {
  jac_set_inf(r);
  for (int i = nbits - 1; i >= 0; i--) {
    jac_dbl(r, r);
    if ((k[i >> 5] >> (i & 31)) & 1) jac_madd(r, r, p);
  }
}
template <class F> GS_HD bool jac_eq_aff(const Jac<F>& j, const Aff<F>& a) {
  if (is_zero(j.z)) return false;
  F z2 = sqr(j.z);
  return eq(mul(a.x, z2), j.x) && eq(mul(a.y, mul(z2, j.z)), j.y);
}
template <class C> GS_HD_NOINLINE bool in_prime_subgroup(const Aff<Fq28<C>>& p) {
  if constexpr (C::IS_BN) {
    return true;
  } else {
    uint32_t x2[4];
    uint64_t cy = 1;
    for (int i = 0; i < 4; i++) {
      uint64_t t = (uint64_t)C::LAMBDA[i] + cy;
      x2[i] = (uint32_t)t;
      cy = t >> 32;
    }
    Jac<Fq28<C>> j;
    jac_mul_bits(j, p, x2, 128);
    Fq28<C> beta;
    for (int i = 0; i < C::L; i++) beta.v[i] = C::BETA_28[i];
    Aff<Fq28<C>> e = {mul(p.x, sqr(beta)), neg(p.y)};
    return jac_eq_aff(j, e);
  }
}
template <class C> GS_HD_NOINLINE bool in_prime_subgroup(const Aff<Fp2<C>>& q) {
  Jac<Fp2<C>> j;
  if constexpr (C::IS_BN) {
    uint32_t r[FrM<C>::N];
    for (int i = 0; i < FrM<C>::N; i++) r[i] = C::R_WORDS[i];
    jac_mul_bits(j, q, r, FrM<C>::BITS);
    return is_zero(j.z);
  } else {
    uint32_t xa[2] = {C::XABS_LIMBS[0], C::XABS_LIMBS[1]};
    jac_mul_bits(j, q, xa, 64);
    Aff<Fp2<C>> e = q;
    endo_apply<C>(e, 1);
    e.y = neg(e.y);
    return jac_eq_aff(j, e);
  }
}

template <class C, class F> GS_HD_NOINLINE void wire_encode_point(uint8_t* out, const Aff<F>& p, bool compressed) {
  constexpr int NC = NCoord<F>::V, B = C::N * 4;
  const int total = (compressed ? NC : 2 * NC) * B;
  bool inf = aff_is_inf(p);
  uint32_t xw[2][C::N], yw[2][C::N];
  coord_words<C>(xw, p.x);
  coord_words<C>(yw, p.y);
  bool largest = !inf && y_is_largest<C, NC>(yw);
  if (inf) {
    for (int i = 0; i < total; i++) out[i] = 0;
  } else if (!C::IS_BN) {
    for (int k = 0; k < NC; k++) fq_put_bytes<C>(out + k * B, xw[NC - 1 - k]);
    if (!compressed)
      for (int k = 0; k < NC; k++) fq_put_bytes<C>(out + (NC + k) * B, yw[NC - 1 - k]);
  } else {
    for (int k = 0; k < NC; k++) fq_put_bytes<C>(out + k * B, xw[k]);
    if (!compressed)
      for (int k = 0; k < NC; k++) fq_put_bytes<C>(out + (NC + k) * B, yw[k]);
  }
  if (!C::IS_BN) {
    uint8_t fl = (compressed ? 0x80 : 0) | (inf ? 0x40 : 0) | ((compressed && largest) ? 0x20 : 0);
    out[0] |= fl;
  } else {
    uint8_t fl = (inf ? 0x40 : 0) | (largest ? 0x80 : 0);
    out[total - 1] |= fl;
  }
}

template <class C, class F>
GS_HD_NOINLINE bool wire_decode_point(Aff<F>& p, const uint8_t* in, bool compressed, bool validate) {
  constexpr int NC = NCoord<F>::V, B = C::N * 4;
  const int total = (compressed ? NC : 2 * NC) * B;
  p.x = zero_of<F>();
  p.y = zero_of<F>();
  uint8_t fb = C::IS_BN ? in[total - 1] : in[0];
  bool inf, largest;
  uint8_t mask;
  if (!C::IS_BN) {
    mask = 0xE0;
    if (((fb & 0x80) != 0) != compressed) return false;
    inf = fb & 0x40;
    largest = fb & 0x20;
    if (!compressed && largest) return false;
    if (inf && largest) return false;
  } else {
    mask = 0xC0;
    inf = fb & 0x40;
    largest = fb & 0x80;
    if (inf && largest) return false;
  }
  const int flag_pos = C::IS_BN ? total - 1 : 0;
  uint32_t xw[2][C::N], yw[2][C::N];
  for (int k = 0; k < NC; k++) {
    int slot = C::IS_BN ? k : NC - 1 - k;
    fq_get_bytes<C>(xw[slot], in + k * B, mask, flag_pos - k * B);
    if (!compressed) fq_get_bytes<C>(yw[slot], in + (NC + k) * B, mask, flag_pos - (NC + k) * B);
  }
  bool canon = true, zero = true;
  for (int k = 0; k < NC; k++) {
    canon = canon && words_lt_p<C>(xw[k]);
    zero = zero && words_zero<C::N>(xw[k]);
    if (!compressed) {
      canon = canon && words_lt_p<C>(yw[k]);
      zero = zero && words_zero<C::N>(yw[k]);
    }
  }
  if (!canon) return false;
  if (inf) return zero;
  F x, y;
  coord_from_words<C>(x, xw);
  F rhs = curve_rhs<C>(x);
  if (compressed) {
    bool sq;
    y = f_sqrt<C>(rhs, sq);
    if (!sq) return false;
    uint32_t got[2][C::N];
    coord_words<C>(got, y);
    if (y_is_largest<C, NC>(got) != largest) y = neg(y);
  } else {
    if (C::IS_BN && y_is_largest<C, NC>(yw) != largest) return false;
    coord_from_words<C>(y, yw);
    if (!eq(sqr(y), rhs)) return false;
  }
  p.x = x;
  p.y = norm(y);
  if (validate && !in_prime_subgroup<C>(p)) {
    p.x = zero_of<F>();
    p.y = zero_of<F>();
    return false;
  }
  return true;
}

template <class C> GS_HD_NOINLINE bool f12_in_torsion(const Fp12<C>& f) {
  Fp12<C> acc;
  f12_one(acc);
  bool started = false;
  for (int i = FrM<C>::N * 32 - 1; i >= 0; i--) {
    if (started) f12_sqr(acc, acc);
    if ((C::R_WORDS[i >> 5] >> (i & 31)) & 1) {
      if (started) f12_mul(acc, acc, f); else acc = f;
      started = true;
    }
  }
  return f12_is_one(acc);
}

}
```

Before: 242,200 proofs+verifies/s.

## Specialize Fp2 constant multiplies by compile-time constant kind in Frobenius and endomorphisms

Tags each tabulated Fp2 constant (Frobenius coefficients, psi endomorphism constants) with a generated kind such as ONE, MINUS_ONE, REAL, IMAG or DIAG. Multiplies by these constants are then specialized at compile time into sign flips, single Fq multiplies or two Fq multiplies instead of a full Fp2 multiply. Frobenius is dispatched to per-j templates. Fixed-table line additions get a sparse add_table path that exploits the structure of real lines. Cost-model constants are updated to match. Static asserts check that the kinds agree with the tables, which adds template complexity and more code paths.

```diff
diff --git a/groth_sahai_rs_amd/csrc/gen_params.py b/groth_sahai_rs_amd/csrc/gen_params.py
--- a/groth_sahai_rs_amd/csrc/gen_params.py
+++ b/groth_sahai_rs_amd/csrc/gen_params.py
@@ -46,6 +46,23 @@
         d.append(z)
         k >>= 1
     return d
+
+
+KINDS = ["ZERO", "ONE", "MINUS_ONE", "U", "MINUS_U", "REAL", "IMAG", "DIAG_MINUS", "DIAG_PLUS", "GENERAL"]
+
+
+def const_kind(a, p):
+    c0, c1 = a[0] % p, a[1] % p
+    if (c0, c1) == (0, 0): return "ZERO"
+    if (c0, c1) == (1, 0): return "ONE"
+    if (c0, c1) == (p - 1, 0): return "MINUS_ONE"
+    if (c0, c1) == (0, 1): return "U"
+    if (c0, c1) == (0, p - 1): return "MINUS_U"
+    if c1 == 0: return "REAL"
+    if c0 == 0: return "IMAG"
+    if (c0 + c1) % p == 0: return "DIAG_MINUS"
+    if c0 == c1: return "DIAG_PLUS"
+    return "GENERAL"
 
 
 def emit(name, S, p, r, x, b, xi, twist, loop_count, loop_neg, bn, g1, g2):
@@ -94,6 +111,11 @@
     w("#endif")
     w("#endif")
     w("namespace gs {")
+    w("#ifndef GS_CONST_KINDS")
+    w("#define GS_CONST_KINDS")
+    w("// what a tabulated Fp2 constant c0 + c1 u is, for mul_const (gs_tower.cuh): DIAG_MINUS = c (1 - u), DIAG_PLUS = c (1 + u)")
+    w("enum ConstKind : int { %s };" % ", ".join("CK_" + k for k in KINDS))
+    w("#endif")
     w("struct %s {" % S)
     w("  static constexpr int N = %d;      // u32 limbs of Fq" % n)
     w("  static constexpr int NR = %d;     // u32 limbs of Fr" % nr)
@@ -157,6 +179,7 @@
         e = (p**j - 1) // 6
         g = [f2.pow(xi, k * e) for k in range(6)]
         w("  GS_DEVCONST static constexpr int32_t FROB%d_28[6][2][%d] = {%s};" % (j, L, ",".join(i28_2(v) for v in g)))
+        w("  static constexpr ConstKind FROB%d_KIND[6] = {%s};" % (j, ", ".join("CK_" + const_kind(v, p) for v in g)))
     if not bn:
         lam = x * x - 1
         assert (lam * lam + lam + 1) % r == 0 and lam.bit_length() <= 128
@@ -219,6 +242,8 @@
         endo.append("  GS_DEVCONST static constexpr int32_t PSI2_Y_28[%d] = %s;" % (L, i28(ny[0])))
         endo.append("  GS_DEVCONST static constexpr int32_t PSI3_X_28[2][%d] = %s;" % (L, i28_2(c3x)))
         endo.append("  GS_DEVCONST static constexpr int32_t PSI3_Y_28[2][%d] = %s;" % (L, i28_2(c3y)))
+        for nm, v in (("PSI_X", cx), ("PSI_Y", cy), ("PSI2_X", nx), ("PSI2_Y", ny), ("PSI3_X", c3x), ("PSI3_Y", c3y)):
+            endo.append("  static constexpr ConstKind %s_KIND = CK_%s;" % (nm, const_kind(v, p)))
     else:
         from fractions import Fraction
         def ec_add1(P1, P2):
diff --git a/groth_sahai_rs_amd/csrc/gs_amd.hip b/groth_sahai_rs_amd/csrc/gs_amd.hip
--- a/groth_sahai_rs_amd/csrc/gs_amd.hip
+++ b/groth_sahai_rs_amd/csrc/gs_amd.hip
@@ -494,6 +494,9 @@
 #if defined(GS_LINES_GENERAL)
   if (curve == 0) return twin ? MCost{4536.0, 7764.0, 6256.0} : MCost{2268.0, 4636.0, 3128.0};
   return twin ? MCost{4680.0, 10519.0, 8096.0} : MCost{2340.0, 6471.0, 4048.0};
+#elif !defined(GS_CONST_GENERAL)
+  if (curve == 0) return twin ? MCost{4536.0, 7356.0, 5168.0} : MCost{2268.0, 4636.0, 2584.0};
+  return twin ? MCost{4680.0, 9991.0, 6688.0} : MCost{2340.0, 6471.0, 3344.0};
 #else
   if (curve == 0) return twin ? MCost{4536.0, 7356.0, 5304.0} : MCost{2268.0, 4636.0, 2652.0};
   return twin ? MCost{4680.0, 9991.0, 6864.0} : MCost{2340.0, 6471.0, 3432.0};
@@ -969,7 +972,12 @@
   }
 };
 static double straus_lane_cost(bool g2, bool bn, int nt, int no, int w) {
-  const double madd = g2 ? 29.0 : 11.0, dbl = g2 ? 16.0 : 8.0, gz = g2 ? 21.0 : 7.0, endo = g2 ? 4.0 : 0.5;
+#if defined(GS_CONST_GENERAL)
+  const double endo2 = 4.0;
+#else
+  const double endo2 = bn ? 3.5 : 2.0;
+#endif
+  const double madd = g2 ? 29.0 : 11.0, dbl = g2 ? 16.0 : 8.0, gz = g2 ? 21.0 : 7.0, endo = g2 ? endo2 : 0.5;
   const int ns = g2 ? 4 : 2, nl = g2 ? (bn ? 3 : 2) : (bn ? 5 : 4), nd = (32 * nl + w - 1) / w + 1, ne = 1 << (w - 1);
   double build = nt * (ne / 2 * dbl + (ne / 2 - 1) * madd + ne * gz);
   double run = (nd - 1) * w * dbl + (double)nt * ns * (nd - 0.5) * (1.0 - 1.0 / (2 * ne)) * (madd + endo);
diff --git a/groth_sahai_rs_amd/csrc/gs_curve.cuh b/groth_sahai_rs_amd/csrc/gs_curve.cuh
--- a/groth_sahai_rs_amd/csrc/gs_curve.cuh
+++ b/groth_sahai_rs_amd/csrc/gs_curve.cuh
@@ -610,14 +610,6 @@
   rout = r;
 }
 
-template <class C> GS_HD Fp2<C> fp2_const28(const int32_t (*c)[C::L]) {
-  Fp2<C> r;
-  for (int i = 0; i < C::L; i++) {
-    r.c0.v[i] = c[0][i];
-    r.c1.v[i] = c[1][i];
-  }
-  return r;
-}
 template <class C> GS_HD void endo_apply(Aff<Fq<C>>& t, int s) {
   if (s == 1) {
     Fq<C> beta;
@@ -625,29 +617,53 @@
     t.x = mul(t.x, beta);
   }
 }
-template <class C> GS_HD void endo_apply(Aff<Fp2<C>>& t, int s) {
+template <class C> GS_HD void endo_apply(Aff<Fp2<C>>& t, int s, bool negy = false) {
   if (aff_is_inf(t)) return;
   if constexpr (C::IS_BN) {
-    if (s == 0) return;
-    Fp2<C> x = (s & 1) ? conj(t.x) : t.x, y = (s & 1) ? conj(t.y) : t.y;
-    t.x = mul(x, frob_coeff<C>(s, 2));
-    t.y = mul(y, frob_coeff<C>(s, 3));
-    return;
-  } else if (s == 1) {
-    t.x = mul(conj(t.x), fp2_const28<C>(C::PSI_X_28));
-    t.y = mul(conj(t.y), fp2_const28<C>(C::PSI_Y_28));
-  } else if (s == 2) {
-    Fq<C> nx, ny;
-    for (int l = 0; l < C::L; l++) {
-      nx.v[l] = C::PSI2_X_28[l];
-      ny.v[l] = C::PSI2_Y_28[l];
-    }
-    t.x = mul_fp(t.x, nx);
-    t.y = mul_fp(t.y, ny);
-  } else if (s == 3) {
-    t.x = mul(conj(t.x), fp2_const28<C>(C::PSI3_X_28));
-    t.y = mul(conj(t.y), fp2_const28<C>(C::PSI3_Y_28));
-  }
+    static_assert(frob_kinds_ok<C>(), "FROBj_KIND does not describe FROBj_28: regenerate the parameter headers");
+    if (s == 1) {
+      t.x = mul_const<C, C::FROB1_KIND[2], true>(t.x, C::FROB1_28[2]);
+      t.y = mul_const<C, C::FROB1_KIND[3], true>(t.y, C::FROB1_28[3]);
+    } else if (s == 2) {
+      t.x = mul_const<C, C::FROB2_KIND[2], false>(t.x, C::FROB2_28[2]);
+      if constexpr (const_is_minus_one<C::FROB2_KIND[3]>())
+        negy = !negy;
+      else
+        t.y = mul_const<C, C::FROB2_KIND[3], false>(t.y, C::FROB2_28[3]);
+    } else if (s == 3) {
+      t.x = mul_const<C, C::FROB3_KIND[2], true>(t.x, C::FROB3_28[2]);
+      t.y = mul_const<C, C::FROB3_KIND[3], true>(t.y, C::FROB3_28[3]);
+    }
+  } else {
+    static_assert(const_kind_ok<C>(C::PSI_X_KIND, C::PSI_X_28[0], C::PSI_X_28[1]) &&
+                      const_kind_ok<C>(C::PSI_Y_KIND, C::PSI_Y_28[0], C::PSI_Y_28[1]) &&
+                      const_kind_ok_fq<C>(C::PSI2_X_KIND, C::PSI2_X_28) &&
+                      const_kind_ok_fq<C>(C::PSI2_Y_KIND, C::PSI2_Y_28) &&
+                      const_kind_ok<C>(C::PSI3_X_KIND, C::PSI3_X_28[0], C::PSI3_X_28[1]) &&
+                      const_kind_ok<C>(C::PSI3_Y_KIND, C::PSI3_Y_28[0], C::PSI3_Y_28[1]),
+                  "PSI*_KIND does not describe PSI*_28: regenerate the parameter headers");
+    if (s == 1) {
+      t.x = mul_const<C, C::PSI_X_KIND, true>(t.x, C::PSI_X_28);
+      t.y = mul_const<C, C::PSI_Y_KIND, true>(t.y, C::PSI_Y_28);
+    } else if (s == 2) {
+      t.x = mul_const_fq<C, C::PSI2_X_KIND>(t.x, C::PSI2_X_28);
+      if constexpr (const_is_minus_one<C::PSI2_Y_KIND>())
+        negy = !negy;
+      else
+        t.y = mul_const_fq<C, C::PSI2_Y_KIND>(t.y, C::PSI2_Y_28);
+    } else if (s == 3) {
+      t.x = mul_const<C, C::PSI3_X_KIND, true>(t.x, C::PSI3_X_28);
+      t.y = mul_const<C, C::PSI3_Y_KIND, true>(t.y, C::PSI3_Y_28);
+    }
+  }
+  if (negy) t.y = neg(t.y);
+}
+template <class C, class NEGY> GS_HD void endo_apply_signed(Aff<Fq<C>>& t, int s, NEGY negy) {
+  endo_apply<C>(t, s);
+  if (negy()) t.y = neg(t.y);
+}
+template <class C, class NEGY> GS_HD void endo_apply_signed(Aff<Fp2<C>>& t, int s, NEGY negy) {
+  endo_apply<C>(t, s, negy());
 }
 template <class C> GS_HD_NOINLINE void jac_smul_endo(Jac<Fp2<C>>& rout, const Aff<Fp2<C>>& p, const Fr<C>& k) {
   Jac<Fp2<C>> r;
@@ -680,8 +696,7 @@
       if (a == 0) continue;
       Aff<Fp2<C>> t = at[(a < 0 ? -a : a) - 1];
       bool negate = (a < 0) != ((j & 1) != 0);
-      endo_apply<C>(t, j);
-      if (negate) t.y = neg(t.y);
+      endo_apply<C>(t, j, negate);
       jac_madd_ip(r, t);
     }
   }
@@ -860,8 +875,7 @@
         if (a != 0) {
           const int t = k / E::NS, s2 = k % E::NS;
           Aff<F> u = e;
-          endo_apply<C>(u, s2);
-          if (((a < 0) != (((sgm >> k) & 1) != 0)) != (((negm >> t) & 1) != 0)) u.y = neg(u.y);
+          endo_apply_signed<C>(u, s2, [&] { return ((a < 0) != (((sgm >> k) & 1) != 0)) != (((negm >> t) & 1) != 0); });
           jac_madd_ip(r, u);
         }
         st_add += GS_STAMP_T() - sb;
@@ -896,8 +910,7 @@
           int a = dg[t][s * ND + i];
           if (a == 0) continue;
           Aff<F> e = tabs ? tabs[t][(a < 0 ? -a : a) - 1] : at[t * NE + (a < 0 ? -a : a) - 1];
-          endo_apply<C>(e, s);
-          if (((a < 0) != (sg[t][s] != 0)) != (((negm >> t) & 1) != 0)) e.y = neg(e.y);
+          endo_apply_signed<C>(e, s, [&] { return ((a < 0) != (sg[t][s] != 0)) != (((negm >> t) & 1) != 0); });
           jac_madd_ip(r, e);
         }
     }
@@ -1001,8 +1014,11 @@
       const int a = wave_uniform((int)sd->d[s * S::ND + i]);
       if (a == 0) continue;
       Aff<F> t = at[(a < 0 ? -a : a) - 1];
-      if constexpr (S::E) endo_apply<C>(t, s);
-      if ((a < 0) != (((sgm >> s) & 1u) != 0)) t.y = neg(t.y);
+      auto negate = [&] { return (a < 0) != (((sgm >> s) & 1u) != 0); };
+      if constexpr (S::E)
+        endo_apply_signed<C>(t, s, negate);
+      else if (negate())
+        t.y = neg(t.y);
       if constexpr (IP)
         jac_madd_ip(r, t);
       else
diff --git a/groth_sahai_rs_amd/csrc/gs_pairing.cuh b/groth_sahai_rs_amd/csrc/gs_pairing.cuh
--- a/groth_sahai_rs_amd/csrc/gs_pairing.cuh
+++ b/groth_sahai_rs_amd/csrc/gs_pairing.cuh
@@ -114,6 +114,20 @@
       f12_mul_by_034r(f, cy, cx, l.l0);
 #endif
   }
+  GS_HD void add_table(Fp12<C>& f, const Line<C>& l, const Aff<Fq<C>>& p) {
+#if defined(GS_CONST_GENERAL) || defined(GS_LINES2_ALL)
+    add(f, l, p);
+#else
+    const Fp2<C> cx = mul_fp(l.lx, p.x);
+    const Fq<C> cy = select(is_zero_limbs(l.ly), fq_zero<C>(), p.y);
+    if (C::TWIST_M)
+      f12_mul_by_014r(f, l.l0, cx, cy);
+    else
+      f12_mul_by_034r(f, cy, cx, l.l0);
+#endif
+  }
+#else
+  GS_HD void add_table(Fp12<C>& f, const GLine<C>& l, const Aff<Fq<C>>& p) { add(f, l, p); }
 #endif
   GS_HD void add(Fp12<C>& f, const GLine<C>& l, const Aff<Fq<C>>& p) {
     GLine<C> g;
@@ -224,7 +238,7 @@
     for (int k = 0; k < np; k++) {
       if (!live[k]) continue;
       if (fixed && fixed[k]) {
-        acc.add(f, fixed[k][li], ps[k]);
+        acc.add_table(f, fixed[k][li], ps[k]);
         continue;
       }
       miller_dbl(ts[k], l);
@@ -236,7 +250,7 @@
       for (int k = 0; k < np; k++) {
         if (!live[k]) continue;
         if (fixed && fixed[k]) {
-          acc.add(f, fixed[k][li], ps[k]);
+          acc.add_table(f, fixed[k][li], ps[k]);
           continue;
         }
         Aff<Fp2<C>> q = qs[k];
@@ -251,8 +265,8 @@
     for (int k = 0; k < np; k++) {
       if (!live[k]) continue;
       if (fixed && fixed[k]) {
-        acc.add(f, fixed[k][li], ps[k]);
-        acc.add(f, fixed[k][li + 1], ps[k]);
+        acc.add_table(f, fixed[k][li], ps[k]);
+        acc.add_table(f, fixed[k][li + 1], ps[k]);
         continue;
       }
       Aff<Fp2<C>> q1, q2;
@@ -302,32 +316,32 @@
     f12_sqr(f1, f1);
     for (int k = 0; k < np; k++) {
       if (!live[k]) continue;
-      const Line<C>* lp = &l;
-      if (fixed && fixed[k])
-        lp = &fixed[k][li];
-      else {
-        miller_dbl(ts[k], g);
-        l = line_real(g);
-      }
-      if (live[k] & 1) acc0.add(f0, *lp, p0[k]);
-      if (live[k] & 2) acc1.add(f1, *lp, p1[k]);
+      if (fixed && fixed[k]) {
+        if (live[k] & 1) acc0.add_table(f0, fixed[k][li], p0[k]);
+        if (live[k] & 2) acc1.add_table(f1, fixed[k][li], p1[k]);
+        continue;
+      }
+      miller_dbl(ts[k], g);
+      l = line_real(g);
+      if (live[k] & 1) acc0.add(f0, l, p0[k]);
+      if (live[k] & 2) acc1.add(f1, l, p1[k]);
     }
     li++;
     int d = C::LOOP[i];
     if (d != 0) {
       for (int k = 0; k < np; k++) {
         if (!live[k]) continue;
-        const Line<C>* lp = &l;
         if (fixed && fixed[k]) {
-          lp = &fixed[k][li];
-        } else {
-          Aff<Fp2<C>> q = qs[k];
-          if (d < 0) q.y = neg(q.y);
-          miller_add(ts[k], g, q);
-          l = line_real(g);
+          if (live[k] & 1) acc0.add_table(f0, fixed[k][li], p0[k]);
+          if (live[k] & 2) acc1.add_table(f1, fixed[k][li], p1[k]);
+          continue;
         }
-        if (live[k] & 1) acc0.add(f0, *lp, p0[k]);
-        if (live[k] & 2) acc1.add(f1, *lp, p1[k]);
+        Aff<Fp2<C>> q = qs[k];
+        if (d < 0) q.y = neg(q.y);
+        miller_add(ts[k], g, q);
+        l = line_real(g);
+        if (live[k] & 1) acc0.add(f0, l, p0[k]);
+        if (live[k] & 2) acc1.add(f1, l, p1[k]);
       }
       li++;
     }
@@ -337,8 +351,8 @@
       if (!live[k]) continue;
       if (fixed && fixed[k]) {
         for (int e = 0; e < 2; e++) {
-          if (live[k] & 1) acc0.add(f0, fixed[k][li + e], p0[k]);
-          if (live[k] & 2) acc1.add(f1, fixed[k][li + e], p1[k]);
+          if (live[k] & 1) acc0.add_table(f0, fixed[k][li + e], p0[k]);
+          if (live[k] & 2) acc1.add_table(f1, fixed[k][li + e], p1[k]);
         }
         continue;
       }
@@ -412,7 +426,7 @@
       products(l, ko, kp);
     }
     for (int k = nstep; k < np; k++)
-      if ((live >> k) & 1) acc.add(f, fixed[k][li], ps[k]);
+      if ((live >> k) & 1) acc.add_table(f, fixed[k][li], ps[k]);
     li++;
     int d = C::LOOP[i];
     if (d != 0) {
@@ -424,7 +438,7 @@
         products(l, ko, kp);
       }
       for (int k = nstep; k < np; k++)
-        if ((live >> k) & 1) acc.add(f, fixed[k][li], ps[k]);
+        if ((live >> k) & 1) acc.add_table(f, fixed[k][li], ps[k]);
       li++;
     }
   }
@@ -445,7 +459,7 @@
         products(l, ko, kp);
       }
       for (int k = nstep; k < np; k++)
-        if ((live >> k) & 1) acc.add(f, fixed[k][li + e], ps[k]);
+        if ((live >> k) & 1) acc.add_table(f, fixed[k][li + e], ps[k]);
     }
   }
   acc.flush(f);
diff --git a/groth_sahai_rs_amd/csrc/gs_params_bls12_381.h b/groth_sahai_rs_amd/csrc/gs_params_bls12_381.h
--- a/groth_sahai_rs_amd/csrc/gs_params_bls12_381.h
+++ b/groth_sahai_rs_amd/csrc/gs_params_bls12_381.h
@@ -8,6 +8,10 @@
 #endif
 #endif
 namespace gs {
+#ifndef GS_CONST_KINDS
+#define GS_CONST_KINDS
+enum ConstKind : int { CK_ZERO, CK_ONE, CK_MINUS_ONE, CK_U, CK_MINUS_U, CK_REAL, CK_IMAG, CK_DIAG_MINUS, CK_DIAG_PLUS, CK_GENERAL };
+#endif
 struct Bls12_381 {
   static constexpr int N = 12;
   static constexpr int NR = 8;
@@ -59,8 +63,11 @@
   GS_DEVCONST static constexpr int32_t B1_28[14] = {220197600,100663296,705639,53975880,29903744,15237699,14523006,109305080,113405195,77983426,72836668,4925937,157807592,89577};
   GS_DEVCONST static constexpr int32_t B2X3_28[2][14] = {{123765578,35651586,136334786,161938349,152085800,245018794,63598036,85652624,190361624,75247962,95864366,68039792,140732600,55706},{123765578,35651586,136334786,161938349,152085800,245018794,63598036,85652624,190361624,75247962,95864366,68039792,140732600,55706}};
   GS_DEVCONST static constexpr int32_t FROB1_28[6][2][14] = {{{55049400,226492416,176409,13493970,208802528,138027152,3630751,228652862,162569026,19495856,85318031,1231484,106560762,22394},{0,0,0,0,0,0,0,0,0,0,0,0,0,0}},{{166836792,248851249,51584792,154304858,56352319,130327775,208630885,40286156,44881151,212744589,37992072,174141729,120403823,7230},{101576819,18535630,15524001,114125243,46678124,38454832,49790061,215062879,30045829,135042025,157548474,67662736,180158992,99282}},{{0,0,0,0,0,0,0,0,0,0,0,0,0,0},{37886809,200165479,30609410,74842500,80498822,209116160,179210523,180816594,266565572,239503032,99423592,150315392,2841631,53668}},{{54406951,53093802,41722322,203293854,205484154,5622420,33622907,62470036,224036522,173297123,89563204,163999141,59688213,52899},{54406951,53093802,41722322,203293854,205484154,5622420,33622907,62470036,224036522,173297123,89563204,163999141,59688213,52899}},{{92936209,158222439,30785820,88336470,20865894,78707857,182841275,141034000,160699143,258998889,184741623,151546876,109402393,76062},{0,0,0,0,0,0,0,0,0,0,0,0,0,0}},{{221243743,33509595,93307115,89163256,261836474,135950195,242253792,102756192,482217,117606257,127555277,69705414,180092037,60129},{47169868,233877284,242237134,179266844,109629425,32832411,16167154,152592843,74444763,230180357,67985269,172099051,120470778,46383}}};
+  static constexpr ConstKind FROB1_KIND[6] = {CK_ONE, CK_DIAG_MINUS, CK_IMAG, CK_DIAG_PLUS, CK_REAL, CK_DIAG_MINUS};
   GS_DEVCONST static constexpr int32_t FROB2_28[6][2][14] = {{{55049400,226492416,176409,13493970,208802528,138027152,3630751,228652862,162569026,19495856,85318031,1231484,106560762,22394},{0,0,0,0,0,0,0,0,0,0,0,0,0,0}},{{230526802,67221400,36499383,193587601,22531621,228101903,79210422,74532441,76796864,108283581,96116954,91489073,29285728,52845},{0,0,0,0,0,0,0,0,0,0,0,0,0,0}},{{175477402,109164440,36322973,180093631,82164549,90074750,75579671,114315035,182663293,88787724,10798923,90257589,191160422,30450},{0,0,0,0,0,0,0,0,0,0,0,0,0,0}},{{213364211,40894463,66932384,254936131,162663371,30755454,254790195,26696173,180793410,59855301,110222516,240572981,194002053,84118},{0,0,0,0,0,0,0,0,0,0,0,0,0,0}},{{37886809,200165479,30609410,74842500,80498822,209116160,179210523,180816594,266565572,239503032,99423592,150315392,2841631,53668},{0,0,0,0,0,0,0,0,0,0,0,0,0,0}},{{92936209,158222439,30785820,88336470,20865894,78707857,182841275,141034000,160699143,258998889,184741623,151546876,109402393,76062},{0,0,0,0,0,0,0,0,0,0,0,0,0,0}}};
+  static constexpr ConstKind FROB2_KIND[6] = {CK_ONE, CK_REAL, CK_REAL, CK_MINUS_ONE, CK_REAL, CK_REAL};
   GS_DEVCONST static constexpr int32_t FROB3_28[6][2][14] = {{{55049400,226492416,176409,13493970,208802528,138027152,3630751,228652862,162569026,19495856,85318031,1231484,106560762,22394},{0,0,0,0,0,0,0,0,0,0,0,0,0,0}},{{214006660,214293077,25386471,65136247,165981745,163160186,224798039,192878999,119325914,174489490,105977342,77805324,240874602,53613},{54406951,53093802,41722322,203293854,205484154,5622420,33622907,62470036,224036522,173297123,89563204,163999141,59688213,52899}},{{0,0,0,0,0,0,0,0,0,0,0,0,0,0},{55049400,226492416,176409,13493970,208802528,138027152,3630751,228652862,162569026,19495856,85318031,1231484,106560762,22394}},{{214006660,214293077,25386471,65136247,165981745,163160186,224798039,192878999,119325914,174489490,105977342,77805324,240874602,53613},{214006660,214293077,25386471,65136247,165981745,163160186,224798039,192878999,119325914,174489490,105977342,77805324,240874602,53613}},{{213364211,40894463,66932384,254936131,162663371,30755454,254790195,26696173,180793410,59855301,110222516,240572981,194002053,84118},{0,0,0,0,0,0,0,0,0,0,0,0,0,0}},{{54406951,53093802,41722322,203293854,205484154,5622420,33622907,62470036,224036522,173297123,89563204,163999141,59688213,52899},{214006660,214293077,25386471,65136247,165981745,163160186,224798039,192878999,119325914,174489490,105977342,77805324,240874602,53613}}};
+  static constexpr ConstKind FROB3_KIND[6] = {CK_ONE, CK_DIAG_MINUS, CK_U, CK_DIAG_PLUS, CK_MINUS_ONE, CK_DIAG_MINUS};
   static constexpr bool HAS_ENDO = true;
   GS_DEVCONST static constexpr uint32_t LAMBDA[4] = {0xffffffffu,0x00000000u,0x0001a402u,0xac45a401u};
   GS_DEVCONST static constexpr int32_t BETA_28[14] = {37886809,200165479,30609410,74842500,80498822,209116160,179210523,180816594,266565572,239503032,99423592,150315392,2841631,53668};
@@ -71,5 +78,11 @@
   GS_DEVCONST static constexpr int32_t PSI2_Y_28[14] = {213364211,40894463,66932384,254936131,162663371,30755454,254790195,26696173,180793410,59855301,110222516,240572981,194002053,84118};
   GS_DEVCONST static constexpr int32_t PSI3_X_28[2][14] = {{0,0,0,0,0,0,0,0,0,0,0,0,0,0},{213364211,40894463,66932384,254936131,162663371,30755454,254790195,26696173,180793410,59855301,110222516,240572981,194002053,84118}};
   GS_DEVCONST static constexpr int32_t PSI3_Y_28[2][14] = {{54406951,53093802,41722322,203293854,205484154,5622420,33622907,62470036,224036522,173297123,89563204,163999141,59688213,52899},{214006660,214293077,25386471,65136247,165981745,163160186,224798039,192878999,119325914,174489490,105977342,77805324,240874602,53613}};
+  static constexpr ConstKind PSI_X_KIND = CK_IMAG;
+  static constexpr ConstKind PSI_Y_KIND = CK_DIAG_MINUS;
+  static constexpr ConstKind PSI2_X_KIND = CK_REAL;
+  static constexpr ConstKind PSI2_Y_KIND = CK_MINUS_ONE;
+  static constexpr ConstKind PSI3_X_KIND = CK_MINUS_U;
+  static constexpr ConstKind PSI3_Y_KIND = CK_DIAG_MINUS;
 };
 }
diff --git a/groth_sahai_rs_amd/csrc/gs_params_bn254.h b/groth_sahai_rs_amd/csrc/gs_params_bn254.h
--- a/groth_sahai_rs_amd/csrc/gs_params_bn254.h
+++ b/groth_sahai_rs_amd/csrc/gs_params_bn254.h
@@ -8,6 +8,10 @@
 #endif
 #endif
 namespace gs {
+#ifndef GS_CONST_KINDS
+#define GS_CONST_KINDS
+enum ConstKind : int { CK_ZERO, CK_ONE, CK_MINUS_ONE, CK_U, CK_MINUS_U, CK_REAL, CK_IMAG, CK_DIAG_MINUS, CK_DIAG_PLUS, CK_GENERAL };
+#endif
 struct Bn254 {
   static constexpr int N = 8;
   static constexpr int NR = 8;
@@ -59,8 +63,11 @@
   GS_DEVCONST static constexpr int32_t B1_28[10] = {237643970,66076281,4763334,95705986,212998900,51414362,165563156,173069787,94428921,1};
   GS_DEVCONST static constexpr int32_t B2X3_28[2][10] = {{26193553,141495253,171894769,119854809,59732186,15832100,50815341,105003228,207479422,1},{169324798,167537351,100430710,187905931,14409804,219438325,8297159,254292003,222129707,2}};
   GS_DEVCONST static constexpr int32_t FROB1_28[6][2][10] = {{{168693142,111503912,91066263,31901995,249956604,17138120,144666204,147168414,120954792,0},{0,0,0,0,0,0,0,0,0,0}},{{133812001,148983001,115022330,46996794,168023309,175683240,100797293,104742705,245863714,2},{209518029,201944753,158778186,246160477,210649201,171526389,209979198,53258301,211906895,1}},{{140912976,227821077,257547131,43198697,4610002,129533238,192242920,264698265,118551830,2},{181583081,26829790,145239802,134208534,183985030,63805091,202956448,46570285,87740487,1}},{{83059826,204664921,41965564,76289372,115534858,28421534,226234731,215327779,360179,1},{194284916,163115080,49151338,194679599,222240089,141486694,99351608,123507005,258529708,2}},{{208317434,262351505,119736315,220162787,142173683,256650118,190801998,887777,20243402,2},{212065600,159522258,90307450,196404121,152942189,255877235,2933919,102716968,126783104,1}},{{236217877,184571513,20657105,262931563,12266425,58945376,245120179,17071039,39035204,2},{133272975,216598130,9045820,148217946,34804272,136589691,85149247,39083786,3724050,3}}};
+  static constexpr ConstKind FROB1_KIND[6] = {CK_ONE, CK_GENERAL, CK_GENERAL, CK_GENERAL, CK_GENERAL, CK_GENERAL};
   GS_DEVCONST static constexpr int32_t FROB2_28[6][2][10] = {{{168693142,111503912,91066263,31901995,249956604,17138120,144666204,147168414,120954792,0},{0,0,0,0,0,0,0,0,0,0}},{{56972283,105669712,228356411,10331154,254790175,259527765,85027812,197267587,247015697,2},{0,0,0,0,0,0,0,0,0,0}},{{156714597,262601255,137290147,246864615,4833570,242389645,208797064,50099172,126060905,2},{0,0,0,0,0,0,0,0,0,0}},{{242151345,191059780,207420836,79842651,158830213,174233164,18407913,88964452,154054346,2},{0,0,0,0,0,0,0,0,0,0}},{{85436748,196893981,70130688,101413492,153996642,200278975,78046304,38865279,27993441,0},{0,0,0,0,0,0,0,0,0,0}},{{254129890,39962437,161196952,133315487,135517790,217417096,222712508,186033693,148948233,0},{0,0,0,0,0,0,0,0,0,0}}};
+  static constexpr ConstKind FROB2_KIND[6] = {CK_ONE, CK_REAL, CK_REAL, CK_MINUS_ONE, CK_REAL, CK_REAL};
   GS_DEVCONST static constexpr int32_t FROB3_28[6][2][10] = {{{168693142,111503912,91066263,31901995,249956604,17138120,144666204,147168414,120954792,0},{0,0,0,0,0,0,0,0,0,0}},{{108585996,163715322,218319775,231133125,123814385,214601971,191797595,34346809,50823778,1},{96123710,168468400,191581498,95021741,156797909,110407292,197124267,71121725,146317535,2}},{{61390692,566658,101912546,190896821,252781826,172357921,109691706,102543529,75923538,0},{108446554,28537652,196884390,157548044,92417415,71878819,229727544,94151635,21874737,1}},{{59349205,97898772,256521535,35455274,24816503,162949751,205274842,20805086,6213503,2},{216559571,139448612,249335761,185500503,186546727,49884590,63722509,112625861,16479430,0}},{{89510400,196146886,188816392,12978662,192731260,152969732,227371785,121455318,225948398,2},{169967077,207684762,231786589,189991190,180115521,168398853,147329430,222040410,252340873,2}},{{28985521,261494431,138392687,227950732,71822300,127002716,154818457,149123811,144316937,1},{145156726,198296246,124114604,33294981,84601829,13823162,170288652,195619255,221755845,0}}};
+  static constexpr ConstKind FROB3_KIND[6] = {CK_ONE, CK_GENERAL, CK_GENERAL, CK_GENERAL, CK_GENERAL, CK_GENERAL};
   static constexpr bool HAS_ENDO = true;
   GS_DEVCONST static constexpr int32_t BETA_28[10] = {156714597,262601255,137290147,246864615,4833570,242389645,208797064,50099172,126060905,2};
   static constexpr int GLV1_SUBBITS = 127;
diff --git a/groth_sahai_rs_amd/csrc/gs_tower.cuh b/groth_sahai_rs_amd/csrc/gs_tower.cuh
--- a/groth_sahai_rs_amd/csrc/gs_tower.cuh
+++ b/groth_sahai_rs_amd/csrc/gs_tower.cuh
@@ -105,6 +105,112 @@
 }
 
 template <class C> GS_HD Fq<C> mul_l2(const Fq<C>& a, const Fq<C>& b) { return mul(a, b); }
+
+#ifndef GS_CONST_KINDS
+#define GS_CONST_KINDS
+enum ConstKind : int { CK_ZERO, CK_ONE, CK_MINUS_ONE, CK_U, CK_MINUS_U, CK_REAL, CK_IMAG, CK_DIAG_MINUS, CK_DIAG_PLUS, CK_GENERAL };
+#endif
+template <class C> GS_HD Fq<C> fq_const28(const int32_t* c) {
+  Fq<C> r;
+#pragma unroll
+  for (int i = 0; i < C::L; i++) r.v[i] = c[i];
+  return r;
+}
+template <class C> constexpr bool const_limbs_zero(const int32_t* a) {
+  for (int i = 0; i < C::L; i++)
+    if (a[i] != 0) return false;
+  return true;
+}
+template <class C> constexpr bool const_limbs_eq(const int32_t* a, const int32_t* b) {
+  for (int i = 0; i < C::L; i++)
+    if (a[i] != b[i]) return false;
+  return true;
+}
+template <class C> constexpr bool const_limbs_sum_p(const int32_t* a, const int32_t* b) {
+  int64_t cy = 0;
+  for (int i = 0; i < C::L; i++) {
+    const int64_t t = (int64_t)a[i] + b[i] + cy;
+    if (i < C::L - 1) {
+      if ((t & M28) != C::P28[i]) return false;
+      cy = t >> 28;
+    } else if (t != C::P28[i])
+      return false;
+  }
+  return true;
+}
+template <class C> constexpr bool const_kind_ok(ConstKind k, const int32_t* c0, const int32_t* c1) {
+  switch (k) {
+    case CK_ZERO: return const_limbs_zero<C>(c0) && const_limbs_zero<C>(c1);
+    case CK_ONE: return const_limbs_eq<C>(c0, C::ONE28) && const_limbs_zero<C>(c1);
+    case CK_MINUS_ONE: return const_limbs_sum_p<C>(c0, C::ONE28) && const_limbs_zero<C>(c1);
+    case CK_U: return const_limbs_zero<C>(c0) && const_limbs_eq<C>(c1, C::ONE28);
+    case CK_MINUS_U: return const_limbs_zero<C>(c0) && const_limbs_sum_p<C>(c1, C::ONE28);
+    case CK_REAL: return const_limbs_zero<C>(c1);
+    case CK_IMAG: return const_limbs_zero<C>(c0);
+    case CK_DIAG_MINUS: return const_limbs_sum_p<C>(c0, c1);
+    case CK_DIAG_PLUS: return const_limbs_eq<C>(c0, c1);
+    default: return true;
+  }
+}
+template <class C> constexpr bool const_kind_ok_fq(ConstKind k, const int32_t* c) {
+  return k == CK_ONE ? const_limbs_eq<C>(c, C::ONE28) : k == CK_MINUS_ONE ? const_limbs_sum_p<C>(c, C::ONE28) : k == CK_REAL;
+}
+template <class C> constexpr bool frob_kinds_ok() {
+  for (int k = 0; k < 6; k++)
+    if (!const_kind_ok<C>(C::FROB1_KIND[k], C::FROB1_28[k][0], C::FROB1_28[k][1]) ||
+        !const_kind_ok<C>(C::FROB2_KIND[k], C::FROB2_28[k][0], C::FROB2_28[k][1]) ||
+        !const_kind_ok<C>(C::FROB3_KIND[k], C::FROB3_28[k][0], C::FROB3_28[k][1]))
+      return false;
+  return true;
+}
+#if defined(GS_CONST_GENERAL)
+constexpr bool CONST_KINDS_ON = false;
+#else
+constexpr bool CONST_KINDS_ON = true;
+#endif
+template <class C, ConstKind K, bool CONJ> GS_HD Fp2<C> mul_const(const Fp2<C>& x, const int32_t (*c)[C::L]) {
+  constexpr ConstKind KK = CONST_KINDS_ON ? K : CK_GENERAL;
+  const Fq<C>& a = x.c0;
+  const Fq<C> b = CONJ ? neg(x.c1) : x.c1, nb = CONJ ? x.c1 : neg(x.c1);
+  if constexpr (KK == CK_ZERO) {
+    return {fq_zero<C>(), fq_zero<C>()};
+  } else if constexpr (KK == CK_ONE) {
+    return {a, b};
+  } else if constexpr (KK == CK_MINUS_ONE) {
+    return {neg(a), nb};
+  } else if constexpr (KK == CK_U) {
+    return {nb, a};
+  } else if constexpr (KK == CK_MINUS_U) {
+    return {b, neg(a)};
+  } else if constexpr (KK == CK_REAL) {
+    const Fq<C> k = fq_const28<C>(c[0]);
+    return {mul(a, k), mul(b, k)};
+  } else if constexpr (KK == CK_IMAG) {
+    const Fq<C> k = fq_const28<C>(c[1]);
+    return {mul(nb, k), mul(a, k)};
+  } else if constexpr (KK == CK_DIAG_MINUS) {
+    const Fq<C> k = fq_const28<C>(c[0]);
+    return {mul_l2(add(a, b), k), mul_l2(sub(b, a), k)};
+  } else if constexpr (KK == CK_DIAG_PLUS) {
+    const Fq<C> k = fq_const28<C>(c[0]);
+    return {mul_l2(sub(a, b), k), mul_l2(add(a, b), k)};
+  } else {
+    Fp2<C> k;
+    k.c0 = fq_const28<C>(c[0]);
+    k.c1 = fq_const28<C>(c[1]);
+    return mul(Fp2<C>{a, b}, k);
+  }
+}
+template <class C, ConstKind K> GS_HD Fp2<C> mul_const_fq(const Fp2<C>& x, const int32_t* c) {
+  static_assert(K == CK_ONE || K == CK_MINUS_ONE || K == CK_REAL, "an Fq constant");
+  if constexpr (CONST_KINDS_ON && K == CK_ONE)
+    return x;
+  else if constexpr (CONST_KINDS_ON && K == CK_MINUS_ONE)
+    return neg(x);
+  else
+    return mul_fp(x, fq_const28<C>(c));
+}
+template <ConstKind K> constexpr bool const_is_minus_one() { return CONST_KINDS_ON && K == CK_MINUS_ONE; }
 template <class C> GS_HD Fq<C> sqr_l2(const Fq<C>& a) { return sqr(a); }
 
 template <class F> GS_HD F zero_of();
@@ -258,6 +364,34 @@
   }
   return r;
 }
+template <class C, int J, int K> GS_HD Fp2<C> frob_mul(const Fp2<C>& x) {
+  static_assert(frob_kinds_ok<C>(), "FROBj_KIND does not describe FROBj_28: regenerate the parameter headers");
+  if constexpr (J == 1)
+    return mul_const<C, C::FROB1_KIND[K], true>(x, C::FROB1_28[K]);
+  else if constexpr (J == 2)
+    return mul_const<C, C::FROB2_KIND[K], false>(x, C::FROB2_28[K]);
+  else
+    return mul_const<C, C::FROB3_KIND[K], true>(x, C::FROB3_28[K]);
+}
+template <class C, int J> GS_HD void f12_frob_j(Fp12<C>& r, const Fp12<C>& a) {
+  const Fp2<C> x0 = a.c0.c0;
+  r.c0.c0 = (J & 1) ? conj(x0) : x0;
+  r.c0.c1 = frob_mul<C, J, 2>(a.c0.c1);
+  r.c0.c2 = frob_mul<C, J, 4>(a.c0.c2);
+  r.c1.c0 = frob_mul<C, J, 1>(a.c1.c0);
+  r.c1.c1 = frob_mul<C, J, 3>(a.c1.c1);
+  r.c1.c2 = frob_mul<C, J, 5>(a.c1.c2);
+}
+#if !defined(GS_CONST_GENERAL)
+template <class C> GS_HD_NOINLINE void f12_frob(Fp12<C>& r, const Fp12<C>& a, int j) {
+  if (j == 1)
+    f12_frob_j<C, 1>(r, a);
+  else if (j == 2)
+    f12_frob_j<C, 2>(r, a);
+  else
+    f12_frob_j<C, 3>(r, a);
+}
+#else
 template <class C> GS_HD_NOINLINE void f12_frob(Fp12<C>& r, const Fp12<C>& a, int j) {
   bool cj = (j & 1);
   Fp2<C> x;
@@ -274,6 +408,7 @@
   x = cj ? conj(a.c1.c2) : a.c1.c2;
   r.c1.c2 = mul(x, frob_coeff<C>(j, 5));
 }
+#endif
 
 template <class C>
 GS_ML void f12_mul_by_014(Fp12<C>& f, const Fp2<C>& l0, const Fp2<C>& l1, const Fp2<C>& l4) {
diff --git a/groth_sahai_rs_amd/csrc/gs_wire.cuh b/groth_sahai_rs_amd/csrc/gs_wire.cuh
--- a/groth_sahai_rs_amd/csrc/gs_wire.cuh
+++ b/groth_sahai_rs_amd/csrc/gs_wire.cuh
@@ -230,8 +230,7 @@
     uint32_t xa[2] = {C::XABS_LIMBS[0], C::XABS_LIMBS[1]};
     jac_mul_bits(j, q, xa, 64);
     Aff<Fp2<C>> e = q;
-    endo_apply<C>(e, 1);
-    e.y = neg(e.y);
+    endo_apply<C>(e, 1, true);
     return jac_eq_aff(j, e);
   }
 }
```

Result: no change. 243,700 proofs+verifies/s (median of 6 runs) (+0.6%).
